# colmap/pycolmap

Hardware: AMD Instinct MI355X
Metric: descriptor-pair distances/sec (exhaustive SIFT match: dot + top-2 + ratio + cross-check) (higher is better)
Workload: dtype u8 descriptors, int8 MFMA / int32 accumulate; 1 GPU; 500 images x 4096 descriptors, exhaustive match + ratio test + cross-check (BASELINE.json configs[1] at N=1); pairs_total=124750, pairs_per_rank=124750, kernel=auto, matches_rank0=1865611

## Files before the change

### include/amc.h

```cpp
#ifndef AMC_H_
#define AMC_H_

#include <stddef.h>
#include <stdint.h>

#ifdef __cplusplus
extern "C" {
#endif

#define AMC_ABI_VERSION 5
#define AMC_DESC_DIM 128

enum {
    AMC_OK = 0,
    AMC_E_INVALID = -1,
    AMC_E_HIP = -2,
    AMC_E_NOMEM = -3,
    AMC_E_STATE = -4
};

enum { AMC_KERNEL_AUTO = 0, AMC_KERNEL_MFMA = 1, AMC_KERNEL_DOT4 = 2 };

typedef struct amc_ctx amc_ctx;

// ... 43 lines not shown

typedef struct amc_gathered_tables {
    size_t npairs;
    const uint64_t* offsets;
    const uint32_t* matches;
    const uint32_t* matches_device;
    uint64_t num_matches;
    uint64_t rows_sent, rows_received;
    int32_t world_size, rank;
    double sizes_ms, meta_ms, rows_ms, reorder_ms, download_ms, total_ms;
    void* _priv;
} amc_gathered_tables;

int amc_allgather_match_tables(amc_ctx* ctx, amc_comm* comm, const uint64_t* pair_index, size_t npairs_local,
                               const uint64_t* offsets, const uint32_t* matches, int download,
                               amc_gathered_tables* out);
void amc_gathered_tables_free(amc_gathered_tables* t);

typedef struct amc_gathered_records {
    size_t npairs;
    size_t record_bytes;
    const void* records;
    const void* records_device;
    uint64_t bytes_sent, bytes_received;
    int32_t world_size, rank;
    double total_ms;
    void* _priv;
} amc_gathered_records;
int amc_allgather_pair_records(amc_ctx* ctx, amc_comm* comm, const uint64_t* pair_index, size_t npairs_local,
                               const void* records, size_t record_bytes, int download, amc_gathered_records* out);
void amc_gathered_records_free(amc_gathered_records* r);
int amc_allgather_inlier_tables(amc_ctx* ctx, amc_comm* comm, const uint64_t* pair_index, size_t npairs_local,
                                int download, amc_gathered_tables* out);

int amc_ctx_reserve_slots(amc_ctx* ctx, uint32_t num_slots);
int amc_ctx_grow_slots(amc_ctx* ctx, uint32_t num_slots);

int amc_upload_descriptors(amc_ctx* ctx, uint32_t slot, const uint8_t* host_desc, uint32_t rows);

int amc_upload_descriptors_device(amc_ctx* ctx, uint32_t slot, const void* dev_desc,
                                  uint32_t rows);

int amc_match_pairs(amc_ctx* ctx, const uint32_t* slot1, const uint32_t* slot2, size_t npairs,
                    const amc_match_opts* opts, amc_match_result* out);
void amc_match_result_free(amc_match_result* r);

void amc_match_opts_default(amc_match_opts* opts);

int amc_get_acos_lut(amc_ctx* ctx, float* out);


typedef struct amc_ransac_opts {
    double max_error;
    double min_inlier_ratio;
    double confidence;
    double dyn_num_trials_multiplier;
    int64_t min_num_trials;
    int64_t max_num_trials;
} amc_ransac_opts;

typedef struct amc_tvg_opts {
    int32_t min_num_inliers;
    int32_t detect_watermark;
    int32_t multiple_ignore_watermark;
    int32_t force_H_use;
    int32_t compute_relative_pose;
    int32_t multiple_models;
    double min_E_F_inlier_ratio;
    double max_H_inlier_ratio;
    double watermark_min_inlier_ratio;
    double watermark_border_size;
    amc_ransac_opts ransac;
} amc_tvg_opts;

enum {
    AMC_TVG_UNDEFINED = 0, AMC_TVG_DEGENERATE = 1, AMC_TVG_CALIBRATED = 2, AMC_TVG_UNCALIBRATED = 3,
    AMC_TVG_PLANAR = 4, AMC_TVG_PANORAMIC = 5, AMC_TVG_PLANAR_OR_PANORAMIC = 6, AMC_TVG_WATERMARK = 7,
    AMC_TVG_MULTIPLE = 8
};

enum {
    AMC_CAM_SIMPLE_PINHOLE = 0,
    AMC_CAM_PINHOLE = 1,
    AMC_CAM_SIMPLE_RADIAL = 2,
    AMC_CAM_RADIAL = 3,
    AMC_CAM_OPENCV = 4,
    AMC_CAM_OPENCV_FISHEYE = 5,
    AMC_CAM_FULL_OPENCV = 6,
    AMC_CAM_FOV = 7,
    AMC_CAM_SIMPLE_RADIAL_FISHEYE = 8,
    AMC_CAM_RADIAL_FISHEYE = 9,
    AMC_CAM_THIN_PRISM_FISHEYE = 10
};

typedef struct amc_tvg {
    int32_t config;
    int32_t num_inliers;
    double E[9], F[9], H[9];
    int64_t num_trials[4];
    int64_t model_inliers[3];
} amc_tvg;

typedef struct amc_pose {
    int32_t ok;
    int32_t config;
    double qvec[4];
    double tvec[3];
    double R[9];
    double tri_angle;
    uint32_t num_points3D;
    uint32_t pad_;
} amc_pose;

typedef struct amc_verify_result {
    size_t npairs;
    amc_tvg* tvg;
    uint8_t* inlier_mask;
    double device_ms;
    double kernel_ms;
    uint32_t kernel_launches;
    amc_pose* pose;
    double pose_kernel_ms;
    uint64_t work[12];
    void* _priv;
} amc_verify_result;

void amc_tvg_opts_default(amc_tvg_opts* opts);

int amc_upload_keypoints(amc_ctx* ctx, uint32_t slot, const float* xy, uint32_t rows,
                         uint32_t stride_floats);

int amc_upload_points_f64(amc_ctx* ctx, uint32_t slot, const double* xy, uint32_t rows);

int amc_upload_camera(amc_ctx* ctx, uint32_t slot, int32_t model_id, uint64_t width,
                      uint64_t height, const double* params, int32_t num_params,
                      int32_t has_prior_focal_length);

int amc_cam_from_img(amc_ctx* ctx, int32_t model_id, const double* params, int32_t num_params,
                     const double* xy, size_t n, double* uv);
int amc_img_from_cam(amc_ctx* ctx, int32_t model_id, const double* params, int32_t num_params,
                     const double* uv, size_t n, double* xy);

int amc_verify_pairs(amc_ctx* ctx, const uint32_t* slot1, const uint32_t* slot2, size_t npairs,
                     const uint64_t* match_offsets, const uint32_t* matches,
                     const amc_tvg_opts* opts, uint32_t seed, amc_verify_result* out);
void amc_verify_result_free(amc_verify_result* r);

int amc_match_verify_pairs(amc_ctx* ctx, const uint32_t* slot1, const uint32_t* slot2, size_t npairs,
                           const amc_match_opts* match_opts, const amc_tvg_opts* tvg_opts, uint32_t seed,
                           amc_match_result* match_out, amc_verify_result* verify_out);

int amc_ctx_last_timeline(amc_ctx* ctx, double out_ms[8]);

int amc_pose_pairs(amc_ctx* ctx, const uint32_t* slot1, const uint32_t* slot2, size_t npairs,
                   const uint64_t* match_offsets, const uint32_t* inlier_matches, const amc_tvg* geoms,
                   amc_pose* out);

int amc_match_guided_pairs(amc_ctx* ctx, const uint32_t* slot1, const uint32_t* slot2, size_t npairs,
                           const amc_tvg* geoms, double max_error, const amc_match_opts* opts,
                           amc_match_result* out);

enum { AMC_RANSAC_F = 0, AMC_RANSAC_H = 1, AMC_RANSAC_E = 2 };
typedef struct amc_ransac_report {
    int32_t success;
    int32_t num_inliers;
    int64_t num_trials;
    double model[9];
} amc_ransac_report;
typedef struct amc_ransac_result {
    size_t npairs;
    amc_ransac_report* reports;
    uint8_t* inlier_mask;
    double device_ms;
    void* _priv;
} amc_ransac_result;
int amc_ransac_pairs(amc_ctx* ctx, int kind, const uint32_t* slot1, const uint32_t* slot2, size_t npairs,
                     const uint64_t* match_offsets, const uint32_t* matches,
                     const amc_ransac_opts* opts, uint32_t seed, amc_ransac_result* out);
void amc_ransac_result_free(amc_ransac_result* r);

int amc_squared_sampson_error(amc_ctx* ctx, const double* points1, const double* points2, size_t n,
                              const double E[9], double* out);

int amc_homography_decomposition(amc_ctx* ctx, const double H[9], const double K1[9], const double K2[9],
                                 const double* points1, const double* points2, size_t n, double R[9], double t[3],
                                 double normal[3], double* points3D, uint64_t* num_points3D);

#ifdef __cplusplus
}
#endif
#endif
```

### pycolmap_amd/_capi.py

```python
from __future__ import annotations

import ctypes as C
from pathlib import Path

import numpy as np

_PKG = Path(__file__).resolve().parent
LIB_PATH = _PKG / "libamc.so"

AMC_OK = 0
AMC_E_INVALID, AMC_E_HIP, AMC_E_NOMEM, AMC_E_STATE = -1, -2, -3, -4
KERNEL_AUTO, KERNEL_MFMA, KERNEL_DOT4 = 0, 1, 2
KERNELS = {"auto": KERNEL_AUTO, "mfma": KERNEL_MFMA, "dot4": KERNEL_DOT4}

EXPORTED_SYMBOLS = [
    "amc_last_error", "amc_abi_version", "amc_device_count", "amc_ctx_create", "amc_ctx_destroy",
    "amc_ctx_set_stream", "amc_ctx_reserve_slots", "amc_upload_descriptors",
    "amc_upload_descriptors_device", "amc_match_pairs", "amc_match_result_free",
    "amc_match_opts_default", "amc_get_acos_lut",
    "amc_tvg_opts_default", "amc_upload_keypoints", "amc_upload_camera", "amc_verify_pairs",
    "amc_verify_result_free", "amc_upload_points_f64", "amc_ransac_pairs", "amc_ransac_result_free",
    "amc_squared_sampson_error", "amc_match_guided_pairs", "amc_ctx_grow_slots", "amc_pose_pairs",
    "amc_cam_from_img", "amc_match_verify_pairs", "amc_ctx_trim", "amc_ctx_resident_matches",
    "amc_homography_decomposition", "amc_img_from_cam",
# ... 991 lines not shown
class UndistortOpts(C.Structure):
    _fields_ = [("blank_pixels", C.c_double), ("min_scale", C.c_double), ("max_scale", C.c_double),
                ("max_image_size", C.c_int32), ("_pad", C.c_int32), ("roi_min_x", C.c_double), ("roi_min_y", C.c_double),
                ("roi_max_x", C.c_double), ("roi_max_y", C.c_double)]


class UndistortCam(C.Structure):
    _fields_ = [("model", C.c_int32), ("_pad", C.c_int32), ("width", C.c_uint64), ("height", C.c_uint64),
                ("params", C.c_double * 12)]


class UndistortImage(C.Structure):
    _fields_ = [("src", C.c_void_p), ("src_stride", C.c_uint64), ("channels", C.c_int32), ("_pad", C.c_int32),
                ("src_camera", UndistortCam), ("dst_camera", UndistortCam), ("dst", C.c_void_p)]


class UndistortResult(C.Structure):
    _fields_ = [("device_ms", C.c_double), ("kernel_ms", C.c_double), ("num_batches", C.c_uint32),
                ("num_resized", C.c_uint32)]


CAMERA_MODEL_IDS = {"SIMPLE_PINHOLE": 0, "PINHOLE": 1, "SIMPLE_RADIAL": 2, "RADIAL": 3, "OPENCV": 4, "OPENCV_FISHEYE": 5,
                    "FULL_OPENCV": 6, "FOV": 7, "SIMPLE_RADIAL_FISHEYE": 8, "RADIAL_FISHEYE": 9, "THIN_PRISM_FISHEYE": 10}
CAMERA_NUM_PARAMS = [3, 4, 4, 5, 8, 8, 12, 5, 4, 5, 12]


def _undistort_cam(camera) -> UndistortCam:
    model, width, height, params = camera
    mid = CAMERA_MODEL_IDS[model] if isinstance(model, str) else int(model)
    p = [float(v) for v in params]
    if 0 <= mid < len(CAMERA_NUM_PARAMS) and len(p) != CAMERA_NUM_PARAMS[mid]:
        raise ValueError(f"camera model {model} takes {CAMERA_NUM_PARAMS[mid]} parameters, got {len(p)}")
    c = UndistortCam()
    c.model, c.width, c.height = mid, int(width), int(height)
    for i, v in enumerate(p[:12]):
        c.params[i] = v
    return c


def _undistort_cam_tuple(c: UndistortCam):
    n = CAMERA_NUM_PARAMS[c.model]
    return (c.model, int(c.width), int(c.height), np.array(c.params[:n], dtype=np.float64))


def undistort_options(**kw) -> UndistortOpts:
    o = UndistortOpts()
    load().amc_undistort_opts_default(C.byref(o))
    for k, v in kw.items():
        if k.startswith("_") or k not in dict(UndistortOpts._fields_):
            raise ValueError(f"undistort options: unknown option {k!r}")
        setattr(o, k, v)
    return o


def undistort_camera(camera, **opts):
    out = UndistortCam()
    _check(load().amc_undistort_camera(C.byref(undistort_options(**opts)), C.byref(_undistort_cam(camera)), C.byref(out)))
    return _undistort_cam_tuple(out)


def undistort_points(camera, undistorted, points) -> np.ndarray:
    xy = np.ascontiguousarray(points, dtype=np.float64).reshape(-1, 2)
    out = np.empty_like(xy)
    _check(load().amc_undistort_points(C.byref(_undistort_cam(camera)), C.byref(_undistort_cam(undistorted)), xy.shape[0],
                                       xy.ctypes.data_as(C.c_void_p), out.ctypes.data_as(C.c_void_p)))
    return out


class RansacOpts(C.Structure):
    _fields_ = [("max_error", C.c_double), ("min_inlier_ratio", C.c_double),
                ("confidence", C.c_double), ("dyn_num_trials_multiplier", C.c_double),
                ("min_num_trials", C.c_int64), ("max_num_trials", C.c_int64)]


class TvgOpts(C.Structure):
    _fields_ = [("min_num_inliers", C.c_int32), ("detect_watermark", C.c_int32),
                ("multiple_ignore_watermark", C.c_int32), ("force_H_use", C.c_int32),
                ("compute_relative_pose", C.c_int32), ("multiple_models", C.c_int32),
                ("min_E_F_inlier_ratio", C.c_double), ("max_H_inlier_ratio", C.c_double),
                ("watermark_min_inlier_ratio", C.c_double), ("watermark_border_size", C.c_double),
                ("ransac", RansacOpts)]


class Tvg(C.Structure):
    _fields_ = [("config", C.c_int32), ("num_inliers", C.c_int32), ("E", C.c_double * 9),
                ("F", C.c_double * 9), ("H", C.c_double * 9), ("num_trials", C.c_int64 * 4),
                ("model_inliers", C.c_int64 * 3)]


class Pose(C.Structure):
    _fields_ = [("ok", C.c_int32), ("config", C.c_int32), ("qvec", C.c_double * 4), ("tvec", C.c_double * 3),
                ("R", C.c_double * 9), ("tri_angle", C.c_double), ("num_points3D", C.c_uint32),
                ("pad_", C.c_uint32)]


class VerifyResult(C.Structure):
    _fields_ = [("npairs", C.c_size_t), ("tvg", C.POINTER(Tvg)), ("inlier_mask", C.POINTER(C.c_uint8)),
                ("device_ms", C.c_double), ("kernel_ms", C.c_double), ("kernel_launches", C.c_uint32),
                ("pose", C.POINTER(Pose)), ("pose_kernel_ms", C.c_double), ("work", C.c_uint64 * 12),
                ("_priv", C.c_void_p)]


class RansacReport(C.Structure):
    _fields_ = [("success", C.c_int32), ("num_inliers", C.c_int32), ("num_trials", C.c_int64),
                ("model", C.c_double * 9)]


class RansacResult(C.Structure):
    _fields_ = [("npairs", C.c_size_t), ("reports", C.POINTER(RansacReport)),
                ("inlier_mask", C.POINTER(C.c_uint8)), ("device_ms", C.c_double), ("_priv", C.c_void_p)]


RANSAC_DTYPE = np.dtype([("success", np.int32), ("num_inliers", np.int32), ("num_trials", np.int64),
                         ("model", np.float64, (3, 3))])
POSE_DTYPE = np.dtype([("ok", np.int32), ("config", np.int32), ("qvec", np.float64, (4,)),
                       ("tvec", np.float64, (3,)), ("R", np.float64, (3, 3)), ("tri_angle", np.float64),
                       ("num_points3D", np.uint32), ("pad_", np.uint32)])
TVG_DTYPE = np.dtype([("config", np.int32), ("num_inliers", np.int32), ("E", np.float64, (3, 3)),
                      ("F", np.float64, (3, 3)), ("H", np.float64, (3, 3)),
                      ("num_trials", np.int64, (4,)), ("model_inliers", np.int64, (3,))])
CAMERA_MODELS = {"SIMPLE_PINHOLE": 0, "PINHOLE": 1, "SIMPLE_RADIAL": 2, "RADIAL": 3, "OPENCV": 4, "OPENCV_FISHEYE": 5,
                 "FULL_OPENCV": 6, "FOV": 7, "SIMPLE_RADIAL_FISHEYE": 8, "RADIAL_FISHEYE": 9,
                 "THIN_PRISM_FISHEYE": 10}
CONFIG_NAMES = ["UNDEFINED", "DEGENERATE", "CALIBRATED", "UNCALIBRATED", "PLANAR", "PANORAMIC",
                "PLANAR_OR_PANORAMIC", "WATERMARK", "MULTIPLE"]

_lib = None


def load() -> C.CDLL:
    global _lib
    if _lib is not None:
        return _lib
    import os
    path = Path(os.environ.get("AMC_LIB_PATH", LIB_PATH))
    if not path.exists():
        raise ImportError(
            f"{path} not found — run `python -m pycolmap_amd.build` (hipcc, gfx950). "
            "pycolmap_amd has no CPU fallback.")
    lib = C.CDLL(str(path))
    lib.amc_last_error.restype = C.c_char_p
    lib.amc_abi_version.restype = C.c_int
    lib.amc_device_count.restype = C.c_int
    lib.amc_ctx_create.argtypes = [C.c_int, C.POINTER(C.c_void_p)]
    lib.amc_ctx_destroy.argtypes = [C.c_void_p]
    lib.amc_ctx_destroy.restype = None
    lib.amc_ctx_set_stream.argtypes = [C.c_void_p, C.c_void_p]
    lib.amc_ctx_trim.argtypes = [C.c_void_p]
    lib.amc_ctx_trim.restype = C.c_int
    lib.amc_ctx_resident_matches.argtypes = [C.c_void_p, C.c_void_p, C.c_void_p]
    lib.amc_ctx_resident_matches.restype = C.c_int
    lib.amc_upload_matches.argtypes = [C.c_void_p, C.c_void_p, C.c_uint64]
    lib.amc_upload_matches.restype = C.c_int
    if hasattr(lib, "amc_ctx_last_timeline"):
        lib.amc_ctx_last_timeline.argtypes = [C.c_void_p, C.c_void_p]
    lib.amc_ctx_reserve_slots.argtypes = [C.c_void_p, C.c_uint32]
    lib.amc_ctx_grow_slots.argtypes = [C.c_void_p, C.c_uint32]
    lib.amc_upload_descriptors.argtypes = [C.c_void_p, C.c_uint32, C.c_void_p, C.c_uint32]
    lib.amc_upload_descriptors_device.argtypes = [C.c_void_p, C.c_uint32, C.c_void_p, C.c_uint32]
    lib.amc_match_pairs.argtypes = [C.c_void_p, C.c_void_p, C.c_void_p, C.c_size_t,
                                    C.POINTER(MatchOpts), C.POINTER(MatchResult)]
    lib.amc_match_result_free.argtypes = [C.POINTER(MatchResult)]
    lib.amc_match_result_free.restype = None
    lib.amc_match_opts_default.argtypes = [C.POINTER(MatchOpts)]
    if hasattr(lib, "amc_sift_extract"):
        lib.amc_sift_opts_default.argtypes = [C.POINTER(SiftOpts)]
        lib.amc_sift_opts_default.restype = None
        lib.amc_sift_extract.argtypes = [C.c_void_p, C.POINTER(SiftImage), C.c_size_t, C.POINTER(SiftOpts),
                                         C.POINTER(SiftResult)]
        lib.amc_sift_extract.restype = C.c_int
        lib.amc_sift_result_free.argtypes = [C.POINTER(SiftResult)]
        lib.amc_sift_result_free.restype = None
    lib.amc_match_opts_default.restype = None
    if hasattr(lib, "amc_estimate_absolute_poses"):
        lib.amc_estimate_absolute_poses.argtypes = ([C.c_void_p, C.c_void_p, C.c_size_t] + [C.c_void_p] * 4 +
                                                    [C.POINTER(AbsPoseOpts), C.POINTER(AbsPoseRefineOpts), C.c_int,
                                                     C.POINTER(AbsPoseResult)])
        lib.amc_estimate_absolute_poses.restype = C.c_int
        lib.amc_refine_absolute_poses.argtypes = ([C.c_void_p, C.c_void_p, C.c_size_t] + [C.c_void_p] * 7 +
                                                  [C.POINTER(AbsPoseRefineOpts), C.c_int, C.POINTER(AbsPoseResult)])
        lib.amc_refine_absolute_poses.restype = C.c_int
        lib.amc_abspose_result_free.argtypes = [C.POINTER(AbsPoseResult)]
        lib.amc_abspose_result_free.restype = None
    if hasattr(lib, "amc_estimate_rig_absolute_poses"):
        lib.amc_estimate_rig_absolute_poses.argtypes = ([C.c_void_p, C.c_void_p, C.c_size_t] + [C.c_void_p] * 7 +
                                                        [C.POINTER(RansacOpts), C.POINTER(AbsPoseRefineOpts), C.c_int,
                                                         C.POINTER(RigPoseResult)])
        lib.amc_estimate_rig_absolute_poses.restype = C.c_int
        lib.amc_rigpose_result_free.argtypes = [C.POINTER(RigPoseResult)]
        lib.amc_rigpose_result_free.restype = None
    if hasattr(lib, "amc_bundle_adjust"):
        lib.amc_ba_opts_default.argtypes = [C.POINTER(BaOpts)]
        lib.amc_ba_opts_default.restype = None
        lib.amc_bundle_adjust.argtypes = [C.c_void_p, C.POINTER(BaProblem), C.POINTER(BaOpts), C.POINTER(BaResult)]
        lib.amc_bundle_adjust.restype = C.c_int
    if hasattr(lib, "amc_bundle_adjust_masked"):
        lib.amc_bundle_adjust_masked.argtypes = [C.c_void_p, C.POINTER(BaProblem), C.c_void_p, C.POINTER(BaOpts),
                                                 C.POINTER(BaResult)]
        lib.amc_bundle_adjust_masked.restype = C.c_int
    if hasattr(lib, "amc_filter_points3d"):
        lib.amc_filter_opts_default.argtypes = [C.POINTER(FilterOpts)]
        lib.amc_filter_opts_default.restype = None
        lib.amc_filter_points3d.argtypes = [C.c_void_p, C.POINTER(FilterProblem), C.POINTER(FilterOpts),
                                            C.POINTER(FilterResult)]
        lib.amc_filter_points3d.restype = C.c_int
        lib.amc_filter_result_free.argtypes = [C.POINTER(FilterResult)]
        lib.amc_filter_result_free.restype = None
    if hasattr(lib, "amc_triangulate_observations"):
        lib.amc_triobs_opts_default.argtypes = [C.POINTER(TriobsOpts)]
        lib.amc_triobs_opts_default.restype = None
        lib.amc_triangulate_observations.argtypes = [C.c_void_p, C.POINTER(TriobsProblem), C.POINTER(TriobsOpts),
                                                     C.POINTER(TriobsResult)]
        lib.amc_triangulate_observations.restype = C.c_int
        lib.amc_triobs_result_free.argtypes = [C.POINTER(TriobsResult)]
        lib.amc_triobs_result_free.restype = None
    if hasattr(lib, "amc_complete_tracks"):
        lib.amc_complete_opts_default.argtypes = [C.POINTER(CompleteOpts)]
        lib.amc_complete_opts_default.restype = None
        lib.amc_complete_tracks.argtypes = [C.c_void_p, C.POINTER(CompleteProblem), C.POINTER(CompleteOpts),
                                            C.POINTER(CompleteResult)]
        lib.amc_complete_tracks.restype = C.c_int
        lib.amc_complete_result_free.argtypes = [C.POINTER(CompleteResult)]
        lib.amc_complete_result_free.restype = None
    if hasattr(lib, "amc_merge_tracks"):
        lib.amc_merge_opts_default.argtypes = [C.POINTER(MergeOpts)]
        lib.amc_merge_opts_default.restype = None
        lib.amc_merge_tracks.argtypes = [C.c_void_p, C.POINTER(MergeProblem), C.POINTER(MergeOpts), C.POINTER(MergeResult)]
        lib.amc_merge_tracks.restype = C.c_int
        lib.amc_merge_result_free.argtypes = [C.POINTER(MergeResult)]
        lib.amc_merge_result_free.restype = None
    if hasattr(lib, "amc_retriangulate_pairs"):
        lib.amc_retri_opts_default.argtypes = [C.POINTER(RetriOpts)]
        lib.amc_retri_opts_default.restype = None
        lib.amc_retriangulate_pairs.argtypes = [C.c_void_p, C.POINTER(RetriProblem), C.POINTER(RetriOpts), C.POINTER(RetriResult)]
        lib.amc_retriangulate_pairs.restype = C.c_int
        lib.amc_retri_result_free.argtypes = [C.POINTER(RetriResult)]
        lib.amc_retri_result_free.restype = None
    if hasattr(lib, "amc_image_visibility"):
        lib.amc_image_visibility.argtypes = [C.c_void_p, C.POINTER(VisibilityProblem), C.POINTER(VisibilityResult)]
        lib.amc_image_visibility.restype = C.c_int
        lib.amc_visibility_result_free.argtypes = [C.POINTER(VisibilityResult)]
        lib.amc_visibility_result_free.restype = None
        lib.amc_pair_angle_opts_default.argtypes = [C.POINTER(PairAngleOpts)]
        lib.amc_pair_angle_opts_default.restype = None
        lib.amc_shared_point_angles.argtypes = [C.c_void_p, C.POINTER(PairAngleProblem), C.POINTER(PairAngleOpts),
                                                C.POINTER(PairAngleResult)]
        lib.amc_shared_point_angles.restype = C.c_int
        lib.amc_pair_angle_result_free.argtypes = [C.POINTER(PairAngleResult)]
        lib.amc_pair_angle_result_free.restype = None
    if hasattr(lib, "amc_patch_match"):
        lib.amc_patch_match_opts_default.argtypes = [C.POINTER(PatchMatchOpts)]
        lib.amc_patch_match_opts_default.restype = None
        lib.amc_patch_match.argtypes = [C.c_void_p, C.POINTER(PatchMatchOpts), C.POINTER(PatchMatchProblem), C.POINTER(PatchMatchResult)]
        lib.amc_patch_match.restype = C.c_int
        lib.amc_patch_match_result_free.argtypes = [C.POINTER(PatchMatchResult)]
        lib.amc_patch_match_result_free.restype = None
    if hasattr(lib, "amc_fuse_depth_maps"):
        lib.amc_fusion_opts_default.argtypes = [C.POINTER(FusionOpts)]
        lib.amc_fusion_opts_default.restype = None
        lib.amc_fuse_depth_maps.argtypes = [C.c_void_p, C.POINTER(FusionOpts), C.POINTER(FusionProblem), C.POINTER(FusionResult)]
        lib.amc_fuse_depth_maps.restype = C.c_int
        lib.amc_fusion_result_free.argtypes = [C.POINTER(FusionResult)]
        lib.amc_fusion_result_free.restype = None
    if hasattr(lib, "amc_triangulate_pairs"):
        lib.amc_pair_tri_opts_default.argtypes = [C.POINTER(PairTriOpts)]
        lib.amc_pair_tri_opts_default.restype = None
        lib.amc_triangulate_pairs.argtypes = [C.c_void_p, C.POINTER(PairTriProblem), C.POINTER(PairTriOpts), C.POINTER(PairTriResult)]
        lib.amc_triangulate_pairs.restype = C.c_int
        lib.amc_pair_tri_result_free.argtypes = [C.POINTER(PairTriResult)]
        lib.amc_pair_tri_result_free.restype = None
    if hasattr(lib, "amc_triangulate_tracks"):
        lib.amc_tri_opts_default.argtypes = [C.POINTER(TriOpts)]
        lib.amc_tri_opts_default.restype = None
        lib.amc_triangulate_tracks.argtypes = [C.c_void_p, C.c_void_p, C.c_size_t, C.c_void_p, C.c_size_t, C.c_void_p,
                                               C.c_void_p, C.POINTER(TriOpts), C.POINTER(TriResult)]
        lib.amc_triangulate_tracks.restype = C.c_int
        lib.amc_tri_result_free.argtypes = [C.POINTER(TriResult)]
        lib.amc_tri_result_free.restype = None
    if hasattr(lib, "amc_undistort_images"):
        lib.amc_undistort_opts_default.argtypes = [C.POINTER(UndistortOpts)]
        lib.amc_undistort_opts_default.restype = None
        lib.amc_undistort_camera.argtypes = [C.POINTER(UndistortOpts), C.POINTER(UndistortCam), C.POINTER(UndistortCam)]
        lib.amc_undistort_camera.restype = C.c_int
        lib.amc_undistort_points.argtypes = [C.POINTER(UndistortCam), C.POINTER(UndistortCam), C.c_size_t, C.c_void_p,
                                             C.c_void_p]
        lib.amc_undistort_points.restype = C.c_int
        lib.amc_undistort_images.argtypes = [C.c_void_p, C.c_size_t, C.c_void_p, C.POINTER(UndistortResult)]
        lib.amc_undistort_images.restype = C.c_int
    lib.amc_get_acos_lut.argtypes = [C.c_void_p, C.c_void_p]
    lib.amc_tvg_opts_default.argtypes = [C.POINTER(TvgOpts)]
    lib.amc_tvg_opts_default.restype = None
    lib.amc_upload_keypoints.argtypes = [C.c_void_p, C.c_uint32, C.c_void_p, C.c_uint32, C.c_uint32]
    lib.amc_upload_camera.argtypes = [C.c_void_p, C.c_uint32, C.c_int32, C.c_uint64, C.c_uint64,
                                      C.c_void_p, C.c_int32, C.c_int32]
    lib.amc_verify_pairs.argtypes = [C.c_void_p, C.c_void_p, C.c_void_p, C.c_size_t, C.c_void_p,
                                     C.c_void_p, C.POINTER(TvgOpts), C.c_uint32, C.POINTER(VerifyResult)]
    lib.amc_verify_result_free.argtypes = [C.POINTER(VerifyResult)]
    lib.amc_verify_result_free.restype = None
    lib.amc_match_guided_pairs.argtypes = [C.c_void_p, C.c_void_p, C.c_void_p, C.c_size_t, C.c_void_p, C.c_double,
                                           C.POINTER(MatchOpts), C.POINTER(MatchResult)]
    lib.amc_upload_points_f64.argtypes = [C.c_void_p, C.c_uint32, C.c_void_p, C.c_uint32]
    lib.amc_ransac_pairs.argtypes = [C.c_void_p, C.c_int, C.c_void_p, C.c_void_p, C.c_size_t, C.c_void_p,
                                     C.c_void_p, C.POINTER(RansacOpts), C.c_uint32, C.POINTER(RansacResult)]
    lib.amc_ransac_result_free.argtypes = [C.POINTER(RansacResult)]
    lib.amc_ransac_result_free.restype = None
    lib.amc_cam_from_img.argtypes = [C.c_void_p, C.c_int32, C.c_void_p, C.c_int32, C.c_void_p, C.c_size_t, C.c_void_p]
# ... 51 lines not shown
    return n


def comm_unique_id() -> bytes:
    buf = C.create_string_buffer(COMM_ID_BYTES)
    _check(load().amc_comm_unique_id(buf))
    return buf.raw


class Comm:

    def __init__(self, ctx: "Context", world_size: int, rank: int, unique_id: bytes):
        if len(unique_id) != COMM_ID_BYTES:
            raise ValueError(f"unique_id must be {COMM_ID_BYTES} bytes")
        self._lib, self._ctx = ctx._lib, ctx
        self.world_size, self.rank = int(world_size), int(rank)
        h = C.c_void_p()
        _check(self._lib.amc_comm_create(ctx._h, int(world_size), int(rank), unique_id, C.byref(h)))
        self._h = h

    def close(self) -> None:
        if getattr(self, "_h", None) and getattr(self._ctx, "_h", None):
            self._lib.amc_comm_destroy(self._h)
        self._h = None

    def __del__(self):
        try:
            self.close()
        except Exception:
            pass

    def _tables_out(self, res, download):
        try:
            g_off = np.ctypeslib.as_array(res.offsets, shape=(int(res.npairs) + 1,)).copy()
            total = int(res.num_matches)
            g_m = None
            if download:
                g_m = (np.ctypeslib.as_array(res.matches, shape=(total, 2)).copy() if total
                       else np.zeros((0, 2), dtype=np.uint32))
            stats = {k: float(getattr(res, k)) for k in ("sizes_ms", "meta_ms", "rows_ms", "reorder_ms", "download_ms", "total_ms")}
            stats.update(num_matches=total, rows_sent=int(res.rows_sent), rows_received=int(res.rows_received),
                         world_size=int(res.world_size), rank=int(res.rank), device_ptr=int(res.matches_device or 0),
                         gather_path="C ABI: ncclAllGather (sizes) + grouped ncclSend/ncclRecv (records, rows) from device memory")
        finally:
            self._lib.amc_gathered_tables_free(C.byref(res))
        return g_off, g_m, stats

    def allgather_match_tables(self, pair_index, offsets, matches=None, download: bool = True):
        off = np.ascontiguousarray(offsets, dtype=np.uint64).reshape(-1)
        n = off.size - 1
        idx = None if pair_index is None else np.ascontiguousarray(pair_index, dtype=np.uint64)
        m = None if matches is None else np.ascontiguousarray(matches, dtype=np.uint32).reshape(-1, 2)
        local = None
        if n < 0:
            local = "offsets must have npairs + 1 entries"
        elif idx is not None and idx.shape != (n,):
            local = "one global position per local pair"
        elif m is not None and m.shape[0] != int(off[-1]) - int(off[0]):
            local = "offsets and matches disagree (%d rows for offsets[-1] = %d)" % (m.shape[0], int(off[-1]))
        if local is not None:
            off, n, idx, m = np.array([1, 0], dtype=np.uint64), 1, None, np.zeros((1, 2), dtype=np.uint32)
        res = GatheredTables()
        rc = self._lib.amc_allgather_match_tables(
            self._ctx._h, self._h, None if idx is None else idx.ctypes.data_as(C.c_void_p), n,
            off.ctypes.data_as(C.c_void_p), None if m is None else m.ctypes.data_as(C.c_void_p), 1 if download else 0,
            C.byref(res))
        if local is not None:
            raise AmcError(rc if rc != AMC_OK else AMC_E_INVALID, "amc_allgather_match_tables: " + local)
        _check(rc)
        return self._tables_out(res, download)

    def allgather_pair_records(self, pair_index, records=None, download: bool = True, dtype=None):
        idx = None if pair_index is None else np.ascontiguousarray(pair_index, dtype=np.uint64).reshape(-1)
        rec = None if records is None else np.ascontiguousarray(records).reshape(-1)
        rdt = TVG_DTYPE if rec is None else rec.dtype
        if dtype is not None:
            rdt = np.dtype(dtype)
        n = len(rec) if rec is not None else (len(idx) if idx is not None else 0)
        width = rdt.itemsize
        if rec is not None and idx is not None and len(idx) != n:
            width, bad = 4, "one global position per local record"
        else:
            bad = None
        res = GatheredRecords()
        rc = self._lib.amc_allgather_pair_records(
            self._ctx._h, self._h, None if idx is None else idx.ctypes.data_as(C.c_void_p), n,
            None if rec is None else rec.ctypes.data_as(C.c_void_p), width, 1 if download else 0, C.byref(res))
        if bad is not None:
            raise AmcError(rc if rc != AMC_OK else AMC_E_INVALID, "amc_allgather_pair_records: " + bad)
        _check(rc)
        try:
            total = int(res.npairs)
            out = None
            if download:
                out = (np.frombuffer(C.string_at(res.records, total * width), dtype=rdt).copy() if total
                       else np.zeros(0, dtype=rdt))
            stats = dict(npairs=total, record_bytes=int(res.record_bytes), bytes_sent=int(res.bytes_sent),
                         bytes_received=int(res.bytes_received), world_size=int(res.world_size), rank=int(res.rank),
                         total_ms=float(res.total_ms), device_ptr=int(res.records_device or 0))
        finally:
            self._lib.amc_gathered_records_free(C.byref(res))
        return out, stats

    def allgather_inlier_tables(self, pair_index, npairs_local: int | None = None, download: bool = True):
        idx = None if pair_index is None else np.ascontiguousarray(pair_index, dtype=np.uint64).reshape(-1)
        n = len(idx) if idx is not None else int(npairs_local or 0)
        res = GatheredTables()
        _check(self._lib.amc_allgather_inlier_tables(self._ctx._h, self._h, None if idx is None else idx.ctypes.data_as(C.c_void_p),
                                                     n, 1 if download else 0, C.byref(res)))
        return self._tables_out(res, download)


class Context:

    def comm_create(self, world_size: int, rank: int, unique_id: bytes) -> Comm:
        import weakref
        comm = Comm(self, world_size, rank, unique_id)
        self.__dict__.setdefault("_comms", []).append(weakref.ref(comm))
        return comm

    def __init__(self, device_id: int = 0):
        self._lib = load()
        h = C.c_void_p()
        _check(self._lib.amc_ctx_create(device_id, C.byref(h)))
        self._h = h
        self.device_id = device_id
        self.resident_generation = 0

    def close(self) -> None:
        self.resident_generation = getattr(self, "resident_generation", 0) + 1
        for ref in self.__dict__.pop("_comms", []):
            comm = ref()
            if comm is not None:
                comm.close()
        if getattr(self, "_h", None):
            self._lib.amc_ctx_destroy(self._h)
            self._h = None

    def __del__(self):
        try:
            self.close()
        except Exception:
            pass

    def __enter__(self):
        return self

    def __exit__(self, *exc):
        self.close()

    def set_stream(self, hip_stream: int | None) -> None:
        _check(self._lib.amc_ctx_set_stream(self._h, C.c_void_p(hip_stream or 0)))

    def last_timeline(self) -> dict:
        buf = (C.c_double * 8)()
        _check(self._lib.amc_ctx_last_timeline(self._h, buf))
        return dict(verify_setup_done=buf[0], match_returned=buf[1], verify_launched=buf[2], verify_results_on_host=buf[3],
                    call_returned=buf[4], batch_handover_host_ms_hidden=buf[5])

    def resident_matches(self):
        ptr, n = C.c_void_p(), C.c_uint64()
        _check(self._lib.amc_ctx_resident_matches(self._h, C.byref(ptr), C.byref(n)))
        return int(ptr.value or 0), int(n.value)

    def upload_matches(self, matches) -> int:
        m = np.ascontiguousarray(matches, dtype=np.uint32).reshape(-1, 2)
        self.resident_generation += 1
        _check(self._lib.amc_upload_matches(self._h, m.ctypes.data_as(C.c_void_p), C.c_uint64(m.shape[0])))
        return int(m.shape[0])

    def resident_view_valid(self, generation: int) -> bool:
        return generation == self.resident_generation and bool(getattr(self, "_h", None))

    def resident_matches_tensor(self, device_index: int = 0, copy: bool = False):
        import torch
        ptr, n = self.resident_matches()
        if n == 0:
            return torch.zeros((0, 2), dtype=torch.int32, device=torch.device("cuda", device_index))
        if copy:
            return self.resident_matches_tensor(device_index, copy=False).clone()

        class _View:
            __cuda_array_interface__ = {"shape": (n, 2), "typestr": "<i4", "data": (ptr, False), "version": 3, "strides": None}
        return torch.as_tensor(_View(), device=torch.device("cuda", device_index))

    def trim(self) -> None:
        self.resident_generation += 1
        _check(self._lib.amc_ctx_trim(self._h))

    def reserve_slots(self, n: int) -> None:
        _check(self._lib.amc_ctx_reserve_slots(self._h, n))

    def grow_slots(self, n: int) -> None:
        _check(self._lib.amc_ctx_grow_slots(self._h, n))

    def upload_descriptors(self, slot: int, desc: np.ndarray) -> None:
        d = np.ascontiguousarray(desc, dtype=np.uint8)
        if d.size and (d.ndim != 2 or d.shape[1] != 128):
            raise ValueError(f"descriptors must be N x 128 uint8, got {d.shape}")
        rows = d.shape[0] if d.ndim == 2 else 0
        _check(self._lib.amc_upload_descriptors(self._h, slot, d.ctypes.data_as(C.c_void_p), rows))

    def upload_descriptors_device(self, slot: int, dev_ptr: int, rows: int) -> None:
        _check(self._lib.amc_upload_descriptors_device(self._h, slot, C.c_void_p(dev_ptr), rows))

    def sift_extract(self, images, **opts):
        single = isinstance(images, np.ndarray)
        imgs = [im if isinstance(im, np.ndarray) and im.ndim == 2 and im.strides[1] == 1 and im.strides[0] >= im.shape[1]
                else np.ascontiguousarray(im) for im in ([images] if single else images)]
        for im in imgs:
            if im.dtype != np.uint8 or im.ndim != 2:
                raise ValueError(f"sift_extract: images must be 2-D uint8, got {im.dtype} {im.shape}")
        o = SiftOpts()
        self._lib.amc_sift_opts_default(C.byref(o))
        for k, v in opts.items():
            if k == "normalization" and isinstance(v, str):
                v = SIFT_NORMALIZATIONS[v]
            if k not in dict(SiftOpts._fields_):
                raise ValueError(f"sift_extract: unknown option {k!r}")
            setattr(o, k, type(getattr(o, k))(v) if not isinstance(v, bool) else int(v))
        arr = (SiftImage * max(1, len(imgs)))()
        for i, im in enumerate(imgs):
            arr[i] = SiftImage(im.ctypes.data, im.shape[1], im.shape[0], im.strides[0])
        res = SiftResult()
        _check(self._lib.amc_sift_extract(self._h, arr, len(imgs), C.byref(o), C.byref(res)))
        try:
            off = np.ctypeslib.as_array(res.offsets, (len(imgs) + 1,)).copy()
            n = int(off[-1])
            kp = np.ctypeslib.as_array(res.keypoints, (max(n, 1), 4))[:n].copy()
            desc = np.ctypeslib.as_array(res.descriptors, (max(n, 1), 128))[:n].copy()
            stats = {"device_ms": res.device_ms, "stage_ms": dict(zip(SIFT_STAGES, list(res.stage_ms)))}
        finally:
            self._lib.amc_sift_result_free(C.byref(res))
        out = [(kp[off[i]:off[i + 1]], desc[off[i]:off[i + 1]]) for i in range(len(imgs))]
        return (out[0] if single else out), stats

    def estimate_absolute_poses(self, offsets, camera_models, camera_params, points2D, points3D, estimation=None,
                                refinement=None, return_covariance=False):
        off, models, prm, p2, p3 = abspose_inputs(offsets, camera_models, camera_params, points2D, points3D)
        eo, ro = abspose_options(estimation, refinement)
        res = AbsPoseResult()
        ptr = lambda a: a.ctypes.data_as(C.c_void_p)
        _check(self._lib.amc_estimate_absolute_poses(self._h, ptr(off), off.size - 1, ptr(models), ptr(prm), ptr(p2),
                                                      ptr(p3), C.byref(eo), C.byref(ro), int(bool(return_covariance)),
                                                      C.byref(res)))
        return self._abspose_out(res, off.size - 1, int(off[-1]), return_covariance)

    def refine_absolute_poses(self, offsets, camera_models, camera_params, points2D, points3D, qvec, tvec, inlier_mask,
                              refinement=None, return_covariance=False):
        off, models, prm, p2, p3 = abspose_inputs(offsets, camera_models, camera_params, points2D, points3D)
        nq, n = off.size - 1, int(off[-1])
        q = np.ascontiguousarray(qvec, dtype=np.float64).reshape(-1, 4)
        t = np.ascontiguousarray(tvec, dtype=np.float64).reshape(-1, 3)
        m = np.ascontiguousarray(inlier_mask, dtype=bool).reshape(-1).astype(np.uint8)
        if q.shape[0] != nq or t.shape[0] != nq or m.size != n:
            raise ValueError(f"refine_absolute_poses: {nq} queries and {n} correspondences by offsets, {q.shape[0]} "
                             f"rotations, {t.shape[0]} translations, {m.size} mask entries")
        _, ro = abspose_options(None, refinement)
        res = AbsPoseResult()
        ptr = lambda a: a.ctypes.data_as(C.c_void_p)
        _check(self._lib.amc_refine_absolute_poses(self._h, ptr(off), nq, ptr(models), ptr(prm), ptr(p2), ptr(p3),
                                                    ptr(q), ptr(t), ptr(m), C.byref(ro), int(bool(return_covariance)),
                                                    C.byref(res)))
        return self._abspose_out(res, nq, n, return_covariance)

    def _abspose_out(self, res, nq, n, cov):
        try:
            a = lambda p, shape: np.ctypeslib.as_array(p, (max(shape[0], 1),) + shape[1:])[:shape[0]].copy()
            out = {"success": a(res.success, (nq,)).astype(bool), "qvec": a(res.qvec, (nq, 4)),
                   "tvec": a(res.tvec, (nq, 3)), "num_inliers": a(res.num_inliers, (nq,)),
                   "num_trials": a(res.num_trials, (nq,)), "focal_factor": a(res.focal_factor, (nq,)),
                   "inlier_mask": a(res.inlier_mask, (n,)).astype(bool), "device_ms": res.device_ms,
                   "kernel_ms": res.kernel_ms, "num_batches": int(res.num_batches)}
            if cov:
                out["covariance"] = a(res.covariance, (nq, 36)).reshape(nq, 6, 6)
        finally:
            self._lib.amc_abspose_result_free(C.byref(res))
        return out

    def bundle_adjust(self, camera_models, camera_params, camera_const, image_cameras, qvec, tvec, pose_const, xyz,
                      obs_image, obs_point, obs_xy, options=None, point_const=None):
        models, prm, cc, icam, q, t, pc, X, oi, op, xy = ba_inputs(camera_models, camera_params, camera_const,
                                                                   image_cameras, qvec, tvec, pose_const, xyz,
                                                                   obs_image, obs_point, obs_xy)
        o = ba_options(options)
        ptr = lambda a: a.ctypes.data_as(C.c_void_p)
        pb = BaProblem(models.size, ptr(models), ptr(prm), ptr(cc), icam.size, ptr(icam), ptr(q), ptr(t), ptr(pc),
                       X.shape[0], ptr(X), oi.size, ptr(oi), ptr(op), ptr(xy))
        res = BaResult()
        if point_const is None:
            _check(self._lib.amc_bundle_adjust(self._h, C.byref(pb), C.byref(o), C.byref(res)))
        else:
            mask = np.ascontiguousarray(np.asarray(point_const).reshape(-1) != 0, dtype=np.uint8)
            if mask.size != X.shape[0]:
                raise ValueError(f"bundle adjustment: {X.shape[0]} points, {mask.size} point_const flags")
            _check(self._lib.amc_bundle_adjust_masked(self._h, C.byref(pb), ptr(mask), C.byref(o), C.byref(res)))
        out = {k: getattr(res, k) for k, _ in BaResult._fields_}
        out["termination"] = BA_TERMINATIONS[res.termination]
        out.update(camera_params=prm, qvec=q, tvec=t, xyz=X)
        return out

    def filter_points3d(self, camera_models, camera_params, image_cameras, qvec, tvec, xyz, track_offsets, obs_image,
                        obs_xy, selected=None, max_reproj_error=4.0, min_tri_angle=1.5, errors_only=False):
        models, prm, icam, q, t, X, off, oi, xy, sel = filter_inputs(camera_models, camera_params, image_cameras, qvec,
                                                                     tvec, xyz, track_offsets, obs_image, obs_xy,
                                                                     selected)
# ... 563 lines not shown
```

### pycolmap_amd/csrc/amc_api.hip

```cpp
#include <algorithm>
#include <chrono>
#include <cmath>
#include <cstdarg>
#include <cstdio>
#include <cstring>
#include <new>
#include <string>
#include <thread>
#include <vector>

#include "amc_ctx.h"
#include "camera_math.h"

using namespace amc;

namespace {
thread_local std::string g_err;
}

namespace amc {
int api_fail(int code, const char* fmt, ...) {
    char buf[512];
    va_list ap;
    va_start(ap, fmt);
    vsnprintf(buf, sizeof buf, fmt, ap);
    va_end(ap);
    g_err = buf;
    return code;
}
CtxView ctx_view(amc_ctx* c) {
    return CtxView{c->device, c->stream, c->resident_matches ? c->d_keep.p : nullptr, c->resident_matches};
}
VerifyResident verify_resident(amc_ctx* c) { return c->vres; }
}

extern "C" {

const char* amc_last_error(void) { return g_err.c_str(); }
int amc_abi_version(void) { return AMC_ABI_VERSION; }

int amc_device_count(void) {
    int n = 0;
    hipError_t e = hipGetDeviceCount(&n);
    if (e != hipSuccess) {
        if (e == hipErrorNoDevice) return 0;
        return api_fail(AMC_E_HIP, "hipGetDeviceCount: %s", hipGetErrorString(e));
    }
    return n;
}

void amc_match_opts_default(amc_match_opts* o) {
    if (!o) return;
    o->max_ratio = 0.8;
    o->max_distance = 0.7;
    o->cross_check = 1;
    o->kernel = AMC_KERNEL_AUTO;
}

int amc_ctx_create(int device_id, amc_ctx** out) {
    if (!out) return api_fail(AMC_E_INVALID, "amc_ctx_create: out is NULL");
    *out = nullptr;
    int n = 0;
    HIPCHK(hipGetDeviceCount(&n));
    if (device_id < 0 || device_id >= n)
        return api_fail(AMC_E_INVALID, "amc_ctx_create: device %d out of range (%d devices)",
                        device_id, n);
    HIPCHK(hipSetDevice(device_id));
    hipDeviceProp_t prop;
    HIPCHK(hipGetDeviceProperties(&prop, device_id));
    if (std::strncmp(prop.gcnArchName, "gfx950", 6) != 0)
        return api_fail(AMC_E_HIP, "amc_ctx_create: device %d is %s; this library is gfx950-only",
                        device_id, prop.gcnArchName);
    amc_ctx* c = new (std::nothrow) amc_ctx();
    if (!c) return api_fail(AMC_E_NOMEM, "amc_ctx_create: out of host memory");
    c->device = device_id;
    hipError_t e = hipStreamCreateWithFlags(&c->own_stream, hipStreamNonBlocking);
    if (e != hipSuccess) {
        delete c;
        return api_fail(AMC_E_HIP, "hipStreamCreate: %s", hipGetErrorString(e));
    }
    c->stream = c->own_stream;
    e = hipStreamCreateWithFlags(&c->copy_stream, hipStreamNonBlocking);
    if (e != hipSuccess) {
        (void)hipStreamDestroy(c->own_stream);
        delete c;
        return api_fail(AMC_E_HIP, "hipStreamCreate: %s", hipGetErrorString(e));
    }
    bool ev_ok = true;
    for (auto& ev : c->cev) ev_ok &= hipEventCreateWithFlags(&ev, hipEventDisableTiming) == hipSuccess;
    {
        int lo = 0, hi = 0;
        (void)hipDeviceGetStreamPriorityRange(&lo, &hi);
        if (hipStreamCreateWithPriority(&c->aux_stream, hipStreamNonBlocking, lo) != hipSuccess) c->aux_stream = nullptr;
        for (auto& ev : c->aev) ev_ok &= hipEventCreateWithFlags(&ev, hipEventDisableTiming) == hipSuccess;
    }
    if (hipStreamCreateWithFlags(&c->vstream, hipStreamNonBlocking) != hipSuccess) c->vstream = nullptr;
    ev_ok &= hipEventCreateWithFlags(&c->vev_setup, hipEventDisableTiming) == hipSuccess;
    ev_ok &= hipEventCreateWithFlags(&c->vev_matches, hipEventDisableTiming) == hipSuccess;
    for (auto& ev : c->ev) ev_ok &= hipEventCreate(&ev) == hipSuccess;
    for (auto& set : c->bev)
        for (auto& ev : set) ev_ok &= hipEventCreate(&ev) == hipSuccess;
    if (!ev_ok) {
        amc_ctx_destroy(c);
        return api_fail(AMC_E_HIP, "amc_ctx_create: hipEventCreate failed");
    }
    c->h_lut.resize(kAcosLutSize);
    const float kDistNorm = 1.0f / (512.0f * 512.0f);
    for (int d = 0; d < kAcosLutSize; ++d)
        c->h_lut[d] = acosf(std::fmin(kDistNorm * (float)d, 1.0f));
    if (hipMalloc(reinterpret_cast<void**>(&c->d_lut), kAcosLutSize * sizeof(float)) !=
            hipSuccess ||
        hipMalloc(reinterpret_cast<void**>(&c->d_scalars), 16 * sizeof(uint32_t)) !=
            hipSuccess ||
        hipMalloc(reinterpret_cast<void**>(&c->d_vscalars), kVScalarWords * sizeof(uint32_t)) != hipSuccess ||
        hipMemcpy(c->d_lut, c->h_lut.data(), kAcosLutSize * sizeof(float),
                  hipMemcpyHostToDevice) != hipSuccess ||
        c->h_scalars.ensure(16) != hipSuccess) {
        amc_ctx_destroy(c);
        return api_fail(AMC_E_HIP, "amc_ctx_create: device allocation failed");
    }
    *out = c;
    return AMC_OK;
}

void amc_ctx_destroy(amc_ctx* c) {
    if (!c) return;
    (void)hipSetDevice(c->device);
    const bool dprof = env_flag("AMC_DESTROY_PROFILE");
    auto tp0 = std::chrono::steady_clock::now();
    auto dlap = [&](const char* what) {
        if (!dprof) return;
        const auto now = std::chrono::steady_clock::now();
        std::fprintf(stderr, "[amc destroy] %s %.1f ms\n", what, std::chrono::duration<double, std::milli>(now - tp0).count());
        tp0 = now;
    };
    (void)hipDeviceSynchronize();
    dlap("sync");
    c->slots.clear();
    c->arena.release_all();
    dlap("slots");
    c->d_imgs.release();
    c->d_grids.release();
    if (c->d_lut) (void)hipFree(c->d_lut);
    if (c->d_accept) (void)hipFree(c->d_accept);
    if (c->d_scalars) (void)hipFree(c->d_scalars);
    c->ms.release_all();
    c->d_keep.release(); c->d_csr.release();
    dlap("match device buffers");
    c->h_csr[0].release(); c->h_csr[1].release();
    c->h_tout.release(); c->h_tmask.release();
    for (int k = 0; k < 2; ++k) {
        c->h_pairs[k].release(); c->h_work[k].release(); c->h_order[k].release(); c->h_order2[k].release();
        c->h_grp[k].release(); c->h_grp2[k].release();
        c->h_pair_off[k].release(); c->h_pair_cnt[k].release(); c->h_matches[k].release();
        c->h_bscalars[k].release();
    }
    c->h_scalars.release();
    dlap("pinned host buffers");
    c->d_timgs.release(); c->d_tmatches.release();
    c->d_estate.release(); c->d_stream.release(); c->d_wmcut.release();
    c->d_tout.release();
    c->vslices.clear();
    c->h_timgs.release(); c->h_tp.release(); c->h_moff.release();
    if (c->d_vscalars) (void)hipFree(c->d_vscalars);
    c->d_tvg_packed.release(); c->d_mask_packed.release(); c->d_moff.release(); c->d_tp_all.release(); c->d_worksum.release();
    c->d_ppairs.release(); c->d_pmatches.release(); c->d_pcos.release(); c->d_pout.release();
    c->h_ppairs.release(); c->h_pout.release();
    dlap("verify device buffers");
    for (auto& ev : c->ev)
        if (ev) (void)hipEventDestroy(ev);
    for (auto& set : c->bev)
        for (auto& ev : set)
            if (ev) (void)hipEventDestroy(ev);
    for (auto& ev : c->cev)
        if (ev) (void)hipEventDestroy(ev);
    if (c->copy_stream) (void)hipStreamDestroy(c->copy_stream);
    if (c->aux_stream) (void)hipStreamDestroy(c->aux_stream);
    for (auto& ev : c->aev)
        if (ev) (void)hipEventDestroy(ev);
    if (c->vstream) (void)hipStreamDestroy(c->vstream);
    if (c->vev_setup) (void)hipEventDestroy(c->vev_setup);
    if (c->vev_matches) (void)hipEventDestroy(c->vev_matches);
    if (c->own_stream) (void)hipStreamDestroy(c->own_stream);
    dlap("events and streams");
    delete c;
    dlap("delete (pools)");
}

int amc_ctx_set_stream(amc_ctx* c, void* hip_stream) {
    if (!c) return api_fail(AMC_E_INVALID, "amc_ctx_set_stream: ctx is NULL");
    c->stream = hip_stream ? reinterpret_cast<hipStream_t>(hip_stream) : c->own_stream;
    return AMC_OK;
}

int amc_ctx_trim(amc_ctx* c) {
    if (!c) return api_fail(AMC_E_INVALID, "amc_ctx_trim: NULL ctx");
    HIPCHK(hipSetDevice(c->device));
    HIPCHK(hipStreamSynchronize(c->stream));
    if (c->copy_stream) HIPCHK(hipStreamSynchronize(c->copy_stream));
    c->result_pool->trim();
    c->d_keep.release(); c->d_csr.release();
    c->resident_matches = 0;
    c->vres = amc::VerifyResident{};
    c->ms.release_large();
    if (c->d_stream.cap * sizeof(uint32_t) > ((size_t)16 << 20)) {
        c->d_stream.release();
        c->stream_len = 0;
    }
    if (c->aux_stream) HIPCHK(hipStreamSynchronize(c->aux_stream));
    if (c->vstream) HIPCHK(hipStreamSynchronize(c->vstream));
    for (auto& sl : c->vslices)
        if (sl) sl->release();
    c->h_tp.release(); c->h_moff.release(); c->h_ppairs.release(); c->h_pout.release();
    c->d_estate.release();
    c->d_tout.release(); c->d_tmatches.release(); c->d_pmatches.release(); c->d_pcos.release();
    c->d_tvg_packed.release(); c->d_mask_packed.release(); c->d_moff.release(); c->d_tp_all.release();
    c->verify_pool->trim();
    c->arena.release_idle_slabs();
    c->h_tout.release(); c->h_tmask.release();
    for (int k = 0; k < 2; ++k) {
        c->h_matches[k].release();
        c->h_csr[k].release();
    }
    return AMC_OK;
}

int amc_ctx_resident_matches(amc_ctx* c, const uint32_t** dev_matches, uint64_t* num_matches) {
    if (!c || !dev_matches || !num_matches) return api_fail(AMC_E_INVALID, "amc_ctx_resident_matches: NULL argument");
    *dev_matches = c->resident_matches ? c->d_keep.p : nullptr;
    *num_matches = c->resident_matches;
    return AMC_OK;
}

int amc_upload_matches(amc_ctx* c, const uint32_t* matches, uint64_t num_matches) {
    if (!c) return api_fail(AMC_E_INVALID, "amc_upload_matches: ctx is NULL");
    if (num_matches > 0 && !matches) return api_fail(AMC_E_INVALID, "amc_upload_matches: NULL rows");
    HIPCHK(hipSetDevice(c->device));
    HIPCHK(hipStreamSynchronize(c->stream));
    c->resident_matches = 0;
    c->vres = amc::VerifyResident{};
    if (num_matches == 0) return AMC_OK;
    HIPCHK(c->d_keep.ensure((size_t)(2 * num_matches)));
    HIPCHK(hipMemcpyAsync(c->d_keep.p, matches, (size_t)(2 * num_matches) * sizeof(uint32_t), hipMemcpyHostToDevice, c->stream));
    HIPCHK(hipStreamSynchronize(c->stream));
    c->resident_matches = num_matches;
    return AMC_OK;
}

int amc_ctx_reserve_slots(amc_ctx* c, uint32_t num_slots) {
    if (!c) return api_fail(AMC_E_INVALID, "amc_ctx_reserve_slots: ctx is NULL");
    HIPCHK(hipSetDevice(c->device));
    HIPCHK(hipStreamSynchronize(c->stream));
    c->slots.assign(num_slots, Slot());
    c->arena.release_all();
    c->table_dirty = true;
    return AMC_OK;
}

int amc_ctx_grow_slots(amc_ctx* c, uint32_t num_slots) {
    if (!c) return api_fail(AMC_E_INVALID, "amc_ctx_grow_slots: ctx is NULL");
    if (num_slots < c->slots.size())
        return api_fail(AMC_E_INVALID, "amc_ctx_grow_slots: %u < current %zu slots (use amc_ctx_reserve_slots to reset)",
                        num_slots, c->slots.size());
    c->slots.resize(num_slots);
    c->table_dirty = true;
    return AMC_OK;
}

static int upload_common(amc_ctx* c, uint32_t slot, const void* src, uint32_t rows,
                         hipMemcpyKind kind) {
    if (!c) return api_fail(AMC_E_INVALID, "upload_descriptors: ctx is NULL");
    if (slot >= c->slots.size())
        return api_fail(AMC_E_INVALID, "upload_descriptors: slot %u >= reserved %zu", slot,
                        c->slots.size());
    if (rows > 0 && !src) return api_fail(AMC_E_INVALID, "upload_descriptors: NULL data, rows=%u", rows);
    if (rows > (1u << 30)) return api_fail(AMC_E_INVALID, "upload_descriptors: rows=%u too large", rows);
    HIPCHK(hipSetDevice(c->device));
    Slot& s = c->slots[slot];
    if (s.base) {
        HIPCHK(hipStreamSynchronize(c->stream));
        c->arena.free(s.base);
        s.base = nullptr;
    }
    c->table_dirty = true;
    s.valid = true;
    s.dev.rows = rows;
    s.dev.rows_pad = round_up(rows, kRowPad);
    s.maxsq = 0;
    if (rows == 0) return AMC_OK;
    const size_t rp = s.dev.rows_pad;
    const size_t bytes = rp * kDim * 2 + rp * sizeof(int32_t);
    hipError_t e = c->arena.alloc(&s.base, bytes);
    if (e != hipSuccess) {
        s.valid = false;
        s.dev = ImageDev{};
        return api_fail(AMC_E_NOMEM, "upload_descriptors: hipMalloc(%zu): %s", bytes,
                        hipGetErrorString(e));
    }
    uint8_t* raw = static_cast<uint8_t*>(s.base);
    uint8_t* prep = raw + rp * kDim;
    int32_t* rs = reinterpret_cast<int32_t*>(prep + rp * kDim);
    s.dev.raw = raw;
    s.dev.prep = prep;
    s.dev.rs128 = rs;
    HIPCHK(hipMemcpyAsync(raw, src, (size_t)rows * kDim, kind, c->stream));
    if (rp > rows)
        HIPCHK(memset_async(raw + (size_t)rows * kDim, 0, (rp - rows) * kDim, c->stream));
    HIPCHK(memset_async(c->d_scalars + 2, 0, sizeof(uint32_t), c->stream));
    HIPCHK(launch_prep(raw, prep, rs, s.dev.rows_pad, c->d_scalars + 2, c->stream));
    HIPCHK(hipMemcpyAsync(c->h_scalars.p + 2, c->d_scalars + 2, sizeof(uint32_t),
                          hipMemcpyDeviceToHost, c->stream));
    HIPCHK(hipStreamSynchronize(c->stream));
    s.maxsq = c->h_scalars.p[2];
    return AMC_OK;
}

int amc_upload_descriptors(amc_ctx* c, uint32_t slot, const uint8_t* host_desc, uint32_t rows) {
    return upload_common(c, slot, host_desc, rows, hipMemcpyHostToDevice);
}
int amc_upload_descriptors_device(amc_ctx* c, uint32_t slot, const void* dev_desc,
                                  uint32_t rows) {
    return upload_common(c, slot, dev_desc, rows, hipMemcpyDeviceToDevice);
}

int amc_get_acos_lut(amc_ctx* c, float* out) {
    if (!c || !out) return api_fail(AMC_E_INVALID, "amc_get_acos_lut: NULL argument");
    HIPCHK(hipSetDevice(c->device));
    HIPCHK(hipMemcpy(out, c->d_lut, kAcosLutSize * sizeof(float), hipMemcpyDeviceToHost));
    return AMC_OK;
}

void amc_tvg_opts_default(amc_tvg_opts* o) {
    if (!o) return;
    o->min_num_inliers = 15;
    o->detect_watermark = 1;
    o->multiple_ignore_watermark = 1;
    o->force_H_use = 0;
    o->compute_relative_pose = 0;
    o->multiple_models = 0;
    o->min_E_F_inlier_ratio = 0.95;
    o->max_H_inlier_ratio = 0.8;
    o->watermark_min_inlier_ratio = 0.7;
    o->watermark_border_size = 0.1;
    o->ransac.max_error = 4.0;
    o->ransac.min_inlier_ratio = 0.25;
    o->ransac.confidence = 0.999;
    o->ransac.dyn_num_trials_multiplier = 3.0;
    o->ransac.min_num_trials = 100;
    o->ransac.max_num_trials = 10000;
}

static int build_keypoint_grid(amc_ctx* c, Slot& s, const float* xy, uint32_t rows) {
    guided::GridGeom gg;
    std::vector<uint32_t> sidx, start;
    if (!guided::build_grid(xy, rows, gg, sidx, start)) return AMC_OK;
    GridDev g{};
    g.x0 = gg.x0; g.y0 = gg.y0; g.cw = gg.cw; g.ch = gg.ch; g.inv_cw = gg.inv_cw; g.inv_ch = gg.inv_ch;
    g.bx1 = gg.bx1; g.by1 = gg.by1;
    g.n = rows;
    std::vector<float> sxy((size_t)rows * 2);
    for (uint32_t k = 0; k < rows; ++k) {
        sxy[2 * (size_t)k] = xy[2 * (size_t)sidx[k]];
        sxy[2 * (size_t)k + 1] = xy[2 * (size_t)sidx[k] + 1];
    }
    const size_t b_xy = sxy.size() * sizeof(float), b_idx = sidx.size() * sizeof(uint32_t), b_st = start.size() * sizeof(uint32_t);
    hipError_t e = c->arena.alloc(&s.grid_base, b_xy + b_idx + b_st);
    if (e != hipSuccess) return api_fail(AMC_E_NOMEM, "amc_upload_keypoints: hipMalloc (grid): %s", hipGetErrorString(e));
    char* base = static_cast<char*>(s.grid_base);
    HIPCHK(hipMemcpy(base, sxy.data(), b_xy, hipMemcpyHostToDevice));
    HIPCHK(hipMemcpy(base + b_xy, sidx.data(), b_idx, hipMemcpyHostToDevice));
    HIPCHK(hipMemcpy(base + b_xy + b_idx, start.data(), b_st, hipMemcpyHostToDevice));
    g.sxy = reinterpret_cast<const float*>(base);
    g.sidx = reinterpret_cast<const uint32_t*>(base + b_xy);
    g.cell_start = reinterpret_cast<const uint32_t*>(base + b_xy + b_idx);
    s.grid = g;
    return AMC_OK;
// ... 238 lines not shown
```

### pycolmap_amd/csrc/amc_ctx.h

```cpp
#pragma once

#include <functional>
#include <map>
#include <memory>
#include <mutex>
#include <vector>

#include "amc_internal.h"
#include "slot_arena.h"
#include "scan_accept.h"

namespace amc {

inline uint32_t round_up(uint32_t x, uint32_t m) { return (x + m - 1) / m * m; }

struct Slot {
    void* base = nullptr;
    ImageDev dev{};
    uint32_t maxsq = 0;
    bool valid = false;
    float* kp = nullptr;
    double* kp64 = nullptr;
    double* kpn = nullptr;
    bool kpn_valid = false;
    uint32_t kp_rows = 0;
    bool has_kp = false, has_cam = false;
    CameraDev cam{};
    void* grid_base = nullptr;
    GridDev grid{};
};

struct HipRaw {
    static int alloc(void** p, size_t bytes) { return (int)hipMalloc(p, bytes); }
    static void free(void* p) { (void)hipFree(p); }
    static void clear_error() { (void)hipGetLastError(); }
};
struct SlotArena : amc::SlotArenaT<HipRaw> {
    template <class T>
    hipError_t alloc(T** out, size_t bytes) {
        return (hipError_t)amc::SlotArenaT<HipRaw>::alloc(out, bytes);
    }
};

struct PinnedPool {
    static constexpr size_t kMaxIdleBytes = (size_t)3 << 29;
    std::mutex mu;
    std::vector<PinBuf<uint32_t>> idle;
    PinBuf<uint32_t> acquire(size_t want = 0) {
        std::lock_guard<std::mutex> lock(mu);
        if (idle.empty()) return PinBuf<uint32_t>();
        auto better = [&](const PinBuf<uint32_t>& a, const PinBuf<uint32_t>& b) {
            const bool fa = a.cap >= want, fb = b.cap >= want;
            if (want && fa != fb) return fa;
            if (want && fa) return a.cap < b.cap;
            return a.cap > b.cap;
        };
        size_t best = 0;
        for (size_t i = 1; i < idle.size(); ++i)
            if (better(idle[i], idle[best])) best = i;
        PinBuf<uint32_t> b = std::move(idle[best]);
        idle.erase(idle.begin() + best);
        return b;
    }
    void give_back(PinBuf<uint32_t> b) {
        if (!b.p) return;
        std::lock_guard<std::mutex> lock(mu);
        idle.push_back(std::move(b));
        auto total = [&] {
            size_t t = 0;
            for (auto& x : idle) t += x.cap * sizeof(uint32_t);
            return t;
        };
        while (!idle.empty() && (idle.size() > 3 || total() > kMaxIdleBytes)) {
            size_t small = 0;
            for (size_t i = 1; i < idle.size(); ++i)
                if (idle[i].cap < idle[small].cap) small = i;
            idle.erase(idle.begin() + small);
        }
    }
    void trim() {
        std::lock_guard<std::mutex> lock(mu);
        idle.clear();
    }
};

struct VerifyClassSlot {
    PinBuf<TvgPair> h_pairs, h_pairs_e;
    DevBuf<TvgPair> pairs, pairs_e;
    DevBuf<double> ws, ws_e;
    DevBuf<uint8_t> maskws;
    void release() { pairs.release(); pairs_e.release(); ws.release(); ws_e.release(); maskws.release(); h_pairs.release(); h_pairs_e.release(); }
};
struct VerifySliceBufs {
    PinBuf<uint32_t> h_tabs;
    DevBuf<uint32_t> tabs;
    DevBuf<uint8_t> outmask, emask;
    VerifyClassSlot cls[4];
    hipEvent_t ev[4] = {nullptr, nullptr, nullptr, nullptr};
    hipEvent_t ev_e_done = nullptr, ev_aux_done = nullptr;
    bool aux_pending = false;
    void release() {
        tabs.release(); outmask.release(); emask.release(); h_tabs.release();
        for (auto& k : cls) k.release();
    }
    ~VerifySliceBufs() {
        for (auto& e : ev)
            if (e) (void)hipEventDestroy(e);
        if (ev_e_done) (void)hipEventDestroy(ev_e_done);
        if (ev_aux_done) (void)hipEventDestroy(ev_aux_done);
    }
};
constexpr size_t kVScalarWords = 128;
constexpr size_t kMaxStreamWords = (size_t)1 << 28;

struct TrialTabKey {
    uint32_t M;
    double confidence, multiplier;
    bool operator<(const TrialTabKey& o) const {
        if (M != o.M) return M < o.M;
        if (confidence != o.confidence) return confidence < o.confidence;
        return multiplier < o.multiplier;
    }
};
constexpr size_t kTrialTabCacheWords = size_t(64) << 20;

}

using namespace amc;

struct amc_ctx {
    int device = 0;
    hipStream_t own_stream = nullptr;
    hipStream_t stream = nullptr;
    hipStream_t copy_stream = nullptr;
    hipEvent_t cev[2] = {nullptr, nullptr};
    hipStream_t aux_stream = nullptr;
    hipEvent_t aev[2] = {nullptr, nullptr};
    std::vector<Slot> slots;
    bool table_dirty = true;
    DevBuf<ImageDev> d_imgs;
    DevBuf<GridDev> d_grids;
    float* d_lut = nullptr;
    std::vector<float> h_lut;
    ScanAccept* d_accept = nullptr;
    ScanAccept h_accept{};
    float accept_ratio = 0.f, accept_distance = 0.f;
    bool accept_valid = false;
    uint32_t* d_scalars = nullptr;
    struct MatchScratch {
        DevBuf<PairDev> d_pairs;
        DevBuf<Dot4Work> d_work;
        DevBuf<uint32_t> d_order, d_order2;
        DevBuf<uint32_t> d_grp, d_grp2, d_seg_base, d_grp_segs, d_grp_item_base;
        DevBuf<SegDesc> d_segs;
        DevBuf<Top2> d_rowbuf, d_colbuf;
        DevBuf<uint32_t> d_accmask;
        DevBuf<GuidedDev> d_guided;
        DevBuf<uint32_t> d_pair_off, d_pair_cnt, d_matches, d_cand_cnt, d_candbuf;
        DevBuf<uint32_t> d_live, d_live_fwd, d_live_all, d_live_rev, d_live_scan;
        void release_all() {
            d_pairs.release(); d_work.release(); d_order.release(); d_order2.release();
            d_grp.release(); d_grp2.release(); d_seg_base.release(); d_grp_segs.release();
            d_grp_item_base.release(); d_segs.release();
            d_rowbuf.release(); d_colbuf.release(); d_accmask.release(); d_guided.release();
            d_pair_off.release(); d_pair_cnt.release(); d_matches.release();
            d_cand_cnt.release(); d_candbuf.release();
            d_live.release(); d_live_fwd.release(); d_live_all.release(); d_live_rev.release();
            d_live_scan.release();
        }
        void release_large() {
            d_rowbuf.release(); d_colbuf.release(); d_accmask.release(); d_matches.release(); d_candbuf.release();
            d_segs.release(); d_seg_base.release();
        }
    };
    MatchScratch ms;
    DevBuf<uint32_t> d_keep;
    DevBuf<uint64_t> d_csr;
    uint64_t resident_matches = 0;
    PinBuf<uint64_t> h_csr[2];
    std::shared_ptr<PinnedPool> result_pool = std::make_shared<PinnedPool>();
    SlotArena arena;
    PinBuf<PairDev> h_pairs[2];
    PinBuf<Dot4Work> h_work[2];
    PinBuf<uint32_t> h_order[2], h_order2[2], h_pair_off[2], h_pair_cnt[2], h_matches[2], h_bscalars[2];
    PinBuf<uint32_t> h_grp[2], h_grp2[2];
    PinBuf<uint32_t> h_scalars;
    hipEvent_t ev[6] = {nullptr, nullptr, nullptr, nullptr, nullptr, nullptr};
    hipEvent_t bev[2][5] = {{nullptr, nullptr, nullptr, nullptr, nullptr},
                            {nullptr, nullptr, nullptr, nullptr, nullptr}};
    DevBuf<TvgImage> d_timgs;
    DevBuf<uint32_t> d_tmatches;
    DevBuf<TvgEState> d_estate;
    std::vector<std::unique_ptr<VerifySliceBufs>> vslices;
    hipStream_t vstream = nullptr;
    hipEvent_t vev_setup = nullptr, vev_matches = nullptr;
    uint32_t* d_vscalars = nullptr;
    std::vector<double> wm_cut_cache;
    double wm_cut_conf = 0.0, wm_cut_mult = 0.0;
    bool wm_cut_on_device = false;
    PinBuf<TvgImage> h_timgs;
    std::vector<TvgImage> timgs_on_device;
    PinBuf<TvgPair> h_tp;
    PinBuf<uint64_t> h_moff;
    DevBuf<uint32_t> d_stream;
    uint32_t stream_seed = 0;
    size_t stream_len = 0;
    DevBuf<double> d_wmcut;
    DevBuf<TvgOut> d_tout;
    DevBuf<amc_tvg> d_tvg_packed;
    DevBuf<uint8_t> d_mask_packed;
    DevBuf<uint64_t> d_moff;
    DevBuf<TvgPair> d_tp_all;
    DevBuf<unsigned long long> d_worksum;
    amc::VerifyResident vres;
    double timeline[8] = {0, 0, 0, 0, 0, 0, 0, 0};
    double last_hook_ms = 0.0;
    std::shared_ptr<PinnedPool> verify_pool = std::make_shared<PinnedPool>();
    PinBuf<TvgOut> h_tout;
    PinBuf<uint8_t> h_tmask;
    std::map<TrialTabKey, std::vector<uint32_t>> trial_tabs;
    size_t trial_tab_words = 0;
    DevBuf<PosePair> d_ppairs;
    DevBuf<uint32_t> d_pmatches;
    DevBuf<double> d_pcos;
    DevBuf<PoseOut> d_pout;
    PinBuf<PosePair> h_ppairs;
    PinBuf<PoseOut> h_pout;
};

namespace amc {

using BatchHook = std::function<int(size_t begin, size_t end, const uint64_t* offsets, const uint64_t* keep_off)>;
int match_impl(amc_ctx* c, const uint32_t* slot1, const uint32_t* slot2, size_t npairs, const amc_match_opts* opts_in,
               const amc_tvg* geoms, double max_error, amc_match_result* out, std::vector<uint64_t>* keep_off = nullptr,
               const BatchHook* batch_hook = nullptr);

int ensure_normalized(amc_ctx* c, uint32_t slot);
void fill_tvg_images(const amc_ctx* c, std::vector<TvgImage>& timgs);

}
```

### pycolmap_amd/csrc/amc_internal.h

```cpp
#pragma once

#include <hip/hip_runtime.h>
#include <stdint.h>

#include <algorithm>
#include <cstdlib>
#include <type_traits>
#include <vector>

#include "../../include/amc.h"
#include "guided_region.h"

namespace amc {

constexpr int kDim = AMC_DESC_DIM;
constexpr int kRowPad = 256;
constexpr int kAcosLutSize = 262145;

__host__ __device__ __forceinline__ constexpr uint32_t arena_swizzle(uint32_t row) {
    return ((row >> 1) & 1u) | (((row >> 5) & 3u) << 1);
}

struct ImageDev {
    const uint8_t* raw;
// ... 172 lines not shown
};

inline hipError_t create_events(hipEvent_t* ev, int n, const unsigned* flags = nullptr) {
    for (int i = 0; i < n; ++i) {
        const hipError_t e = hipEventCreateWithFlags(&ev[i], flags ? flags[i] : hipEventDefault);
        if (e != hipSuccess) {
            for (int j = 0; j < i; ++j) (void)hipEventDestroy(ev[j]);
            std::fill(ev, ev + n, nullptr);
            return e;
        }
    }
    return hipSuccess;
}

class StreamTimer {
  public:
    explicit StreamTimer(hipStream_t s) : s_(s), made_(create_events(ab_, 2)) {}
    StreamTimer(const StreamTimer&) = delete;
    StreamTimer& operator=(const StreamTimer&) = delete;
    ~StreamTimer() {
        for (hipEvent_t e : ab_)
            if (e) (void)hipEventDestroy(e);
        for (hipEvent_t e : spans_) (void)hipEventDestroy(e);
    }

    hipError_t start() { return made_ != hipSuccess ? made_ : hipEventRecord(ab_[0], s_); }
    hipError_t stop(double& ms) {
        hipError_t e = hipEventRecord(ab_[1], s_);
        if (e == hipSuccess) e = hipEventSynchronize(ab_[1]);
        return e == hipSuccess ? add_elapsed(ab_[0], ab_[1], ms) : e;
    }
    hipError_t span_begin() {
        hipEvent_t two[2];
        if (const hipError_t e = create_events(two, 2)) return e;
        spans_.insert(spans_.end(), two, two + 2);
        return hipEventRecord(two[0], s_);
    }
    hipError_t span_end() { return hipEventRecord(spans_.back(), s_); }
    hipError_t spans(double& ms) const {
        for (size_t i = 0; i + 1 < spans_.size(); i += 2)
            if (const hipError_t e = add_elapsed(spans_[i], spans_[i + 1], ms)) return e;
        return hipSuccess;
    }

  private:
    static hipError_t add_elapsed(hipEvent_t a, hipEvent_t b, double& ms) {
        float f = 0.f;
        const hipError_t e = hipEventElapsedTime(&f, a, b);
        if (e == hipSuccess) ms += f;
        return e;
    }
    hipStream_t s_;
    hipEvent_t ab_[2] = {nullptr, nullptr};
    hipError_t made_;
    std::vector<hipEvent_t> spans_;
};

struct Batches {
    std::vector<size_t> start{0};
    uint64_t most_items = 0, most_elems = 0;
    size_t count() const { return start.size() - 1; }
};
inline Batches split_batches(const uint64_t* offsets, size_t n, uint64_t max_items, uint64_t max_elems,
                             uint64_t factor = 1) {
    Batches b;
    for (size_t i = 0; i < n;) {
        size_t j = i + 1;
        while (j < n && j - i < max_items && (offsets[j + 1] - offsets[i]) * factor <= max_elems) ++j;
        b.most_items = std::max<uint64_t>(b.most_items, j - i);
        b.most_elems = std::max<uint64_t>(b.most_elems, offsets[j] - offsets[i]);
        b.start.push_back(j);
        i = j;
    }
    return b;
}

struct CtxView {
    int device;
    hipStream_t stream;
    const uint32_t* resident;
    uint64_t resident_rows;
};
CtxView ctx_view(amc_ctx* c);
struct TvgPair;
struct VerifyResident {
    size_t npairs = 0;
    uint64_t total = 0;
    const amc_tvg* tvg = nullptr;
    const uint8_t* mask = nullptr;
    const uint64_t* moff = nullptr;
    const TvgPair* tp = nullptr;
    const uint32_t* matches = nullptr;
};
VerifyResident verify_resident(amc_ctx* c);

hipError_t memset_async(void* p, int value, size_t bytes, hipStream_t s);
hipError_t memcpy_async(void* dst, const void* src, size_t bytes, hipMemcpyKind kind, hipStream_t s);

hipError_t launch_prep(const uint8_t* raw, uint8_t* prep, int32_t* rs128, uint32_t rows_pad,
                 uint32_t* maxsq_out, hipStream_t s);

hipError_t launch_match_dot4(const ImageDev* imgs, const PairDev* pairs, const Dot4Work* work,
                       uint32_t nwork, Top2* rowbuf, Top2* colbuf, const GuidedDev* guided, hipStream_t s);
hipError_t launch_match_guided_grid(const ImageDev* imgs, const GridDev* grids, const PairDev* pairs, const Dot4Work* work,
                              uint32_t nwork, Top2* rowbuf, Top2* colbuf, const GuidedDev* guided, hipStream_t s);

constexpr int kSegRows = 128;
constexpr int kSegsPerItem = 4;
struct alignas(64) SegDesc {
    const uint8_t* xprep;
    const int32_t* xrs;
    Top2* out;
    const uint32_t* list;
    const uint8_t* yprep;
    const int32_t* yrs;
    uint32_t cnt;
    uint32_t accword;
    uint32_t yrows;
    uint32_t pad_;
};
__device__ __forceinline__ bool one_way_accepts(const Top2 t, const float* __restrict__ lut,
                                                float max_ratio, float max_distance) {
    if (t.best_v == 0u) return false;
    const float a_best = lut[min(t.best_v, 262144u)];
    if (a_best > max_distance) return false;
    const float a_second = lut[min(t.second_v, 262144u)];
    if (a_best >= max_ratio * a_second) return false;
    return true;
}

hipError_t launch_build_segments(int mode, const ImageDev* imgs, const PairDev* pairs, const uint32_t* order,
                           const uint32_t* grp_start, uint32_t ngroups, const uint32_t* cand_cnt,
                           const uint32_t* candbuf, Top2* outbuf, uint32_t* seg_base, uint32_t* grp_segs,
                           uint32_t* grp_item_base, SegDesc* segs, uint32_t* nitems_dev, hipStream_t s);
struct ScanAccept;
struct CopyJob {
    const void* src = nullptr;
    void* dst = nullptr;
    unsigned long long n16 = 0;
    uint32_t parts = 0, pad_ = 0;
};
hipError_t launch_match_mfma(int mode, const SegDesc* segs, const uint32_t* nitems_dev, uint32_t max_items,
                       uint32_t* queue_head, uint32_t* accmask, const ScanAccept* accept_dev, hipStream_t s,
                       const CopyJob& job = CopyJob(), uint32_t* copy_head = nullptr);

size_t live_scratch_words(size_t npairs);
hipError_t launch_live_pairs(const ImageDev* imgs, const PairDev* pairs, uint32_t npairs, const uint32_t* accmask,
                             const uint32_t* order, uint32_t norder, uint32_t* live, uint32_t* live_fwd,
                             uint32_t* live_all, uint32_t* nlive, uint32_t* cand_cnt, uint32_t* pair_cnt,
                             uint32_t* pair_off, uint32_t* scratch, hipStream_t s);
hipError_t launch_compact_order(const uint32_t* order, uint32_t norder, uint32_t npairs, const uint32_t* key, uint32_t* list,
                                uint32_t* nlist, uint32_t* scratch, hipStream_t s);

hipError_t launch_resolve_index(int side, const ImageDev* imgs, const PairDev* pairs,
                          Top2* table, uint32_t* accmask, const float* acos_lut, FinalizeParams fp,
                          const uint32_t* cand_cnt, const uint32_t* candbuf, uint32_t* err_count,
                          bool grouped, const uint32_t* order, const uint32_t* nlist, uint32_t max_list, hipStream_t s);
uint32_t resolve_grouped_max_rows();
constexpr uint32_t kSelectMaxCols = 1u << 20;

hipError_t launch_select_candidates(const ImageDev* imgs, const PairDev* pairs, uint32_t npairs, uint32_t max_cols,
                              const Top2* rowbuf, const uint32_t* accmask, const float* acos_lut,
                              FinalizeParams fp, uint32_t* cand_cnt, uint32_t* candbuf, const uint32_t* list,
                              const uint32_t* nlist, hipStream_t s);

hipError_t launch_finalize(const ImageDev* imgs, const PairDev* pairs, uint32_t npairs, const uint32_t* list,
                     const uint32_t* nlist, const Top2* rowbuf, const Top2* colbuf, uint32_t* accmask,
                     const float* acos_lut, FinalizeParams fp, uint32_t* cursor, uint32_t capacity,
                     uint32_t* pair_off, uint32_t* pair_cnt, uint32_t* matches, hipStream_t s);

hipError_t launch_host_copy(void* dst_pinned, const void* src_dev, size_t bytes, hipStream_t s);
hipError_t launch_reorder_matches(const uint32_t* src_off, const uint32_t* cnt, const uint64_t* dst_off, uint32_t npairs,
                            const uint32_t* src, uint32_t* dst, hipStream_t s);

struct CameraDev {
    int32_t model_id;
    int32_t has_prior;
    uint64_t width, height;
    double params[12];
};
struct TvgImage {
    const float* kp;
    const double* kp64;
    const double* kpn;
    uint32_t rows;
    uint32_t pad;
    CameraDev cam;
};
hipError_t launch_undistort(const float* kp, const double* kp64, uint32_t rows, const CameraDev& cam, double* kpn,
                            hipStream_t s);
hipError_t launch_project(const double* uv, uint32_t n, const CameraDev& cam, double* xy, hipStream_t s);
struct TvgPair {
    uint32_t slot1, slot2;
    uint64_t match_off;
    uint64_t mask_off;
    uint32_t M;
    uint32_t tab_off[3];
    uint32_t orig;
};
struct PosePair {
    uint32_t slot1, slot2;
    uint64_t match_off;
    uint64_t mask_off;
    uint64_t ws_off;
    uint32_t M;
    int32_t config;
    double E[9], H[9];
};
struct alignas(128) PoseOut {
    int32_t ok;
    int32_t t_is_zero;
    uint32_t num_points3D;
    uint32_t pad;
    double R[9], t[3], q[4], cmed[2];
};
hipError_t launch_pose(const TvgImage* imgs, const PosePair* pairs, uint32_t npairs, const uint32_t* matches,
                       const uint8_t* mask, double* cosine_ws, PoseOut* out, hipStream_t s);

struct alignas(128) TvgOut {
    amc_tvg g;
    unsigned long long prof[8];
    unsigned long long work[12];
};
struct TvgParams {
    int32_t min_num_inliers, detect_watermark, force_H_use, min_num_trials;
    int32_t max_trials[4];
    double min_E_F_inlier_ratio, max_H_inlier_ratio, watermark_min_inlier_ratio,
        watermark_border_size, max_error;
    int32_t force_slow_sampler;
    int32_t no_fast_count;
    int32_t no_fast32;
    int32_t mode;
    uint32_t* bad_index_count;
    const double* wm_cut;
    const uint32_t* stream;
    uint32_t stream_len;
    uint32_t* stream_err;
};
struct alignas(64) TvgEState {
    double model[9];
    double sum;
    int32_t cnt, success, num_trials;
    uint32_t soff;
};
void tvg_diag_report();
void tvg_diag_report_e();
size_t tvg_ws_doubles_host(uint32_t mcap);
size_t tvg_ws_doubles_e_host(uint32_t mcap);
size_t tvg_ws_mask_bytes_host(uint32_t mcap);
constexpr int kTvgEWavesPerSimd = 2;
constexpr int kTvgFhWavesPerSimd = 4;
size_t tvg_lds_bytes(uint32_t mcap, int waves);
size_t tvg_lds_bytes_e(uint32_t mcap, int waves);
hipError_t launch_pack_verify(const TvgOut* out, const TvgPair* tp, uint32_t npairs, const uint8_t* mask_src,
                              const uint64_t* moff, amc_tvg* tvg_dst, uint8_t* mask_dst, unsigned long long* work,
                              int32_t trivial_below, hipStream_t s);
hipError_t launch_homography_decomposition(const double* in27, const double* p1, const double* p2, uint32_t n, double* out16,
                                           double* points3D, hipStream_t s);
hipError_t launch_sampson(const double* p1, const double* p2, size_t n, const double* E9, double* out,
                          hipStream_t s);
hipError_t launch_tvg_e(const TvgImage* imgs, const TvgPair* pairs, uint32_t npairs, const uint32_t* matches,
                        const uint32_t* trial_tabs, const TvgParams& P, double* ws, uint32_t mcap, uint32_t num_waves,
                        int waves_per_block, uint32_t* queue_head, TvgEState* estate, uint8_t* emask, TvgOut* out,
                        uint8_t* out_mask, hipStream_t s);
hipError_t launch_tvg_fh(const TvgImage* imgs, const TvgPair* pairs, uint32_t npairs, const uint32_t* matches,
                         const uint32_t* trial_tabs, const TvgParams& P, double* ws, uint8_t* mask_ws, uint32_t mcap,
                         uint32_t num_waves, int waves_per_block, uint32_t* queue_head, const TvgEState* estate,
                         const uint8_t* emask, TvgOut* out, uint8_t* out_mask, hipStream_t s);

size_t tvg_big_lds_bytes(int waves);
size_t tvg_big_lds_bytes_e(int waves);
size_t tvg_big_idx_doubles_host(uint32_t mcap);
hipError_t launch_tvg_e_big(const TvgImage* imgs, const TvgPair* pairs, uint32_t npairs, const uint32_t* matches,
                            const uint32_t* trial_tabs, const TvgParams& P, double* ws, uint32_t mcap, uint32_t num_waves,
                            int waves_per_block, uint32_t* queue_head, TvgEState* estate, uint8_t* emask, TvgOut* out,
                            uint8_t* out_mask, hipStream_t s);
hipError_t launch_tvg_fh_big(const TvgImage* imgs, const TvgPair* pairs, uint32_t npairs, const uint32_t* matches,
                             const uint32_t* trial_tabs, const TvgParams& P, double* ws, uint8_t* mask_ws, uint32_t mcap,
                             uint32_t num_waves, int waves_per_block, uint32_t* queue_head, const TvgEState* estate,
                             const uint8_t* emask, TvgOut* out, uint8_t* out_mask, hipStream_t s);

}
```

### pycolmap_amd/csrc/amc_match.hip

```cpp
#include <algorithm>
#include <chrono>
#include <cstdio>
#include <cstdlib>
#include <cstring>
#include <limits>
#include <memory>
#include <new>
#include <vector>

#include "amc_ctx.h"

using namespace amc;

namespace {

struct ResultPriv {
    std::vector<uint64_t> offsets;
    PinBuf<uint32_t> matches;
    std::shared_ptr<PinnedPool> pool;
    ~ResultPriv() {
        if (pool) pool->give_back(std::move(matches));
    }
};

constexpr size_t kMaxTop2Entries = (size_t)256 << 20;
constexpr size_t kMaxMatchCap = (size_t)256 << 20;

}

static void guided_grid_setup(GuidedDev& g, const GridDev& g1, const GridDev& g2, bool dense_only) {
    g.grid_ok = 0;
    g.bound[0] = g.bound[1] = 0.0;
    for (int k = 0; k < 9; ++k) g.minv[k] = 0.0;
    if (dense_only || g1.n == 0 || g2.n == 0) return;
    const float box1[4] = {g1.x0, g1.y0, g1.bx1, g1.by1}, box2[4] = {g2.x0, g2.y0, g2.bx1, g2.by1};
    g.grid_ok = guided::guided_pair_setup(g.kind, g.m, g.max_residual, box1, box2, g.bound, g.minv) ? 1 : 0;
}

int amc::match_impl(amc_ctx* c, const uint32_t* slot1, const uint32_t* slot2, size_t npairs,
                    const amc_match_opts* opts_in, const amc_tvg* geoms, double max_error,
                    amc_match_result* out, std::vector<uint64_t>* keep_off, const BatchHook* batch_hook) {
    if (!c || !out) return api_fail(AMC_E_INVALID, "amc_match_pairs: NULL ctx/out");
    std::memset(out, 0, sizeof *out);
    if (npairs > 0 && (!slot1 || !slot2))
        return api_fail(AMC_E_INVALID, "amc_match_pairs: NULL pair arrays");
    const bool prof = env_flag("AMC_MATCH_PROFILE");
    const bool guided_dense_only = env_flag("AMC_GUIDED_DENSE");
    const bool accept_trivial = env_flag("AMC_SCAN_ACCEPT_TRIVIAL");
    const bool resolve_ungrouped = env_flag("AMC_RESOLVE_UNGROUPED");
    const size_t batch_entries = (size_t)env_int("AMC_MATCH_BATCH_ENTRIES", 0, 0, (long long)kMaxTop2Entries);
    const char* const d2h_env = std::getenv("AMC_D2H");
    const size_t fuse_min_bytes = (size_t)env_int("AMC_D2H_FUSE_MIN_BYTES", 1 << 20, 0, std::numeric_limits<long long>::max());
    const int hook_split_mode = (int)env_int("AMC_HOOK_SPLIT", 1, 0, 2);
    const auto wall0 = std::chrono::steady_clock::now();
    double t_prepare = 0.0, t_collect = 0.0, t_enqueue = 0.0, t_scatter = 0.0;
    auto since = [](std::chrono::steady_clock::time_point t) {
        return std::chrono::duration<double, std::milli>(std::chrono::steady_clock::now() - t).count();
    };
    amc_match_opts o;
    if (opts_in) o = *opts_in; else amc_match_opts_default(&o);
    if (o.kernel != AMC_KERNEL_AUTO && o.kernel != AMC_KERNEL_MFMA && o.kernel != AMC_KERNEL_DOT4)
        return api_fail(AMC_E_INVALID, "amc_match_pairs: unknown kernel %d", o.kernel);
    uint64_t rows_total = 0;
    for (size_t i = 0; i < npairs; ++i) {
        if (slot1[i] >= c->slots.size() || slot2[i] >= c->slots.size())
            return api_fail(AMC_E_INVALID, "amc_match_pairs: pair %zu references slot out of range", i);
        if (!c->slots[slot1[i]].valid || !c->slots[slot2[i]].valid)
            return api_fail(AMC_E_STATE, "amc_match_pairs: pair %zu references a slot with no "
                            "descriptors uploaded", i);
        rows_total += c->slots[slot1[i]].dev.rows_pad;
    }
    std::vector<GuidedDev> h_guided;
    if (geoms) {
        h_guided.resize(npairs);
        for (size_t i = 0; i < npairs; ++i) {
            const int cfg = geoms[i].config;
            GuidedDev& g = h_guided[i];
            g.kind = (cfg == AMC_TVG_CALIBRATED || cfg == AMC_TVG_UNCALIBRATED) ? kGuidedF
                     : (cfg == AMC_TVG_PLANAR || cfg == AMC_TVG_PANORAMIC || cfg == AMC_TVG_PLANAR_OR_PANORAMIC)
                         ? kGuidedH : kGuidedNone;
            if (g.kind == kGuidedNone)
                return api_fail(AMC_E_INVALID, "amc_match_guided_pairs: pair %zu: configuration %d has no guided "
                                "matching (COLMAP keeps the inlier matches it has)", i, cfg);
            const double* m = g.kind == kGuidedF ? geoms[i].F : geoms[i].H;
            for (int k = 0; k < 9; ++k) g.m[k] = (float)m[k];
            g.max_residual = (float)(max_error * max_error);
            const Slot& a = c->slots[slot1[i]];
            const Slot& b = c->slots[slot2[i]];
            if (!a.kp || !b.kp || a.kp_rows < a.dev.rows || b.kp_rows < b.dev.rows)
                return api_fail(AMC_E_STATE, "amc_match_guided_pairs: pair %zu: float32 keypoints (one per descriptor) "
                                "must be uploaded for both images", i);
            guided_grid_setup(g, a.grid, b.grid, guided_dense_only);
        }
    }
    HIPCHK(hipSetDevice(c->device));
    hipStream_t st = c->stream;

    if (c->table_dirty) {
        HIPCHK(c->d_imgs.ensure(c->slots.size()));
        std::vector<ImageDev> t(c->slots.size());
        for (size_t i = 0; i < t.size(); ++i) t[i] = c->slots[i].dev;
        if (!t.empty())
            HIPCHK(hipMemcpy(c->d_imgs.p, t.data(), t.size() * sizeof(ImageDev),
                             hipMemcpyHostToDevice));
        HIPCHK(c->d_grids.ensure(c->slots.size()));
        std::vector<GridDev> gt(c->slots.size());
        for (size_t i = 0; i < gt.size(); ++i) gt[i] = c->slots[i].grid;
        if (!gt.empty())
            HIPCHK(hipMemcpy(c->d_grids.p, gt.data(), gt.size() * sizeof(GridDev), hipMemcpyHostToDevice));
        c->table_dirty = false;
    }

    const float max_ratio_f = (float)o.max_ratio;
    FinalizeParams fp;
    fp.max_ratio = max_ratio_f;
    fp.max_distance = (float)o.max_distance;
    fp.cross_check = o.cross_check ? 1 : 0;
    fp.reserved = 0;

    if (!c->accept_valid || std::memcmp(&c->accept_ratio, &fp.max_ratio, sizeof(float)) != 0 ||
        std::memcmp(&c->accept_distance, &fp.max_distance, sizeof(float)) != 0) {
        c->h_accept = build_scan_accept(c->h_lut.data(), (uint32_t)c->h_lut.size(), fp.max_ratio, fp.max_distance);
        if (accept_trivial) c->h_accept.trivial = 1;
        if (!c->d_accept) HIPCHK(hipMalloc(reinterpret_cast<void**>(&c->d_accept), sizeof(ScanAccept)));
        HIPCHK(hipStreamSynchronize(st));
        HIPCHK(hipMemcpy(c->d_accept, &c->h_accept, sizeof(ScanAccept), hipMemcpyHostToDevice));
        c->accept_ratio = fp.max_ratio;
        c->accept_distance = fp.max_distance;
        c->accept_valid = true;
    }
    HIPCHK(hipEventRecord(c->ev[0], st));
    ResultPriv* priv = new (std::nothrow) ResultPriv();
    if (!priv) return api_fail(AMC_E_NOMEM, "amc_match_pairs: out of host memory");
    priv->offsets.assign(npairs + 1, 0);
    priv->pool = c->result_pool;
    priv->matches = c->result_pool->acquire();
    size_t keep_used = 0;
    c->resident_matches = 0;
    c->vres = amc::VerifyResident{};
    if (keep_off) keep_off->assign(npairs, 0);

    const size_t mfma_max_cols = kSelectMaxCols;

    uint64_t num_dist = 0, n_mfma = 0, n_dot4 = 0, n_grid = 0;
    double kernel_ms = 0.0, cross_ms = 0.0;
    uint32_t kernel_launches = 0;

    int rc = AMC_OK;
    auto hc = [&](hipError_t e, const char* what) {
        if (e != hipSuccess && rc == AMC_OK)
            rc = api_fail(AMC_E_HIP, "amc_match_pairs: %s: %s", what, hipGetErrorString(e));
        return e == hipSuccess;
    };
    const size_t max_entries = batch_entries ? batch_entries : kMaxTop2Entries;

    struct Batch {
        size_t begin = 0, end = 0, nb = 0, top_rows = 0, top_cols = 0, cap = 0;
        size_t row_off = 0, nwork = 0, nord = 0, nwork_grid = 0;
        uint32_t max_cols = 0;
        size_t ngrp = 0, ngrp2 = 0, seg_cap = 0;
        int set = 0;
        uint32_t total = 0;
        bool grouped_resolve = true;
    };
    uint64_t rows_carved = 0, rows_collected = 0;
    const int d2h_mode = !d2h_env ? 0 : (std::strcmp(d2h_env, "memcpy") == 0 ? 2 : (std::strcmp(d2h_env, "stream") == 0 ? 1 : 0));
    struct PendingCopy {
        void* dst = nullptr;
        const void* src = nullptr;
        size_t bytes = 0;
        int set = -1;
    } pending;
    constexpr uint32_t kCopyParts = 64 / kSegsPerItem;
    auto sync_batch_streams = [&](const char* what) { return hc(hipStreamSynchronize(st), what); };
    const bool hook_split = batch_hook && hook_split_mode != 0;
    const size_t hook_split_min_pairs = hook_split_mode == 2 ? 2 : 4096;
    auto carve = [&](size_t begin, int set) {
        Batch b;
        b.begin = b.end = begin;
        b.set = set;
        size_t limit = max_entries;
        const uint64_t rows_left = rows_total - rows_carved;
        if (begin > 0 && rows_left <= max_entries && rows_left > max_entries / 4)
            limit = (size_t)(rows_left - max_entries / 4);
        if (begin == 0 && hook_split && rows_total <= max_entries && npairs >= hook_split_min_pairs)
            limit = (size_t)(rows_total * 6 / 10);
        while (b.end < npairs) {
            const Slot& x = c->slots[slot1[b.end]];
            const Slot& y = c->slots[slot2[b.end]];
            const size_t nr = x.dev.rows_pad, nc = y.dev.rows_pad;
            const size_t mc = o.cross_check ? std::min(x.dev.rows, y.dev.rows) : x.dev.rows;
            if (b.end > b.begin && (b.top_rows + nr > limit || b.top_cols + nc > max_entries ||
                                    b.cap + mc > kMaxMatchCap || b.end - b.begin >= (1u << 24)))
                break;
            b.top_rows += nr; b.top_cols += nc; b.cap += mc; ++b.end;
        }
        b.nb = b.end - b.begin;
        rows_carved += b.top_rows;
        return b;
    };
    auto build_reverse_order = [&](Batch& b) {
        const int k = b.set;
        const size_t nord = b.nord;
        if (!nord || !o.cross_check) return;
        const PairDev* hp = c->h_pairs[k].p;
        const size_t nslots = c->slots.size();
        std::vector<uint32_t> cnt(nslots + 1), tmp(nord);
        auto by_slot = [&](const uint32_t* src, uint32_t* dst, bool key_is_slot2) {
            std::fill(cnt.begin(), cnt.end(), 0u);
            for (size_t q = 0; q < nord; ++q) ++cnt[(key_is_slot2 ? hp[src[q]].slot2 : hp[src[q]].slot1) + 1];
            for (size_t v = 0; v < nslots; ++v) cnt[v + 1] += cnt[v];
            for (size_t q = 0; q < nord; ++q) dst[cnt[key_is_slot2 ? hp[src[q]].slot2 : hp[src[q]].slot1]++] = src[q];
        };
        uint32_t* ord2 = c->h_order2[k].p;
        by_slot(c->h_order[k].p, tmp.data(), true);
        by_slot(tmp.data(), ord2, false);
        size_t ngrp2 = 0;
        for (size_t q = 0; q < nord; ++q)
            if (q == 0 || hp[ord2[q]].slot1 != hp[ord2[q - 1]].slot1) c->h_grp2[k].p[ngrp2++] = (uint32_t)q;
        c->h_grp2[k].p[ngrp2] = (uint32_t)nord;
    };
    auto prepare = [&](Batch& b, bool defer_reverse) {
        const int k = b.set;
        const size_t nb = b.nb, begin = b.begin;
        if (!hc(c->h_pairs[k].ensure(nb), "pinned pairs") || !hc(c->h_order[k].ensure(nb), "pinned order") ||
            !hc(c->h_order2[k].ensure(nb), "pinned order2") || !hc(c->h_pair_off[k].ensure(nb), "pinned pair_off") ||
            !hc(c->h_pair_cnt[k].ensure(nb), "pinned pair_cnt") || !hc(c->h_bscalars[k].ensure(16), "pinned scalars"))
            return false;
        std::vector<uint8_t> want_mfma(nb, 0);
        for (size_t i = 0; i < nb; ++i) {
            const Slot& x = c->slots[slot1[begin + i]];
            const Slot& y = c->slots[slot2[begin + i]];
            const bool nonempty = x.dev.rows > 0 && y.dev.rows > 0;
            want_mfma[i] = nonempty && o.kernel != AMC_KERNEL_DOT4 && !geoms &&
                           (!o.cross_check || y.dev.rows_pad <= mfma_max_cols);
        }
        PairDev* hp = c->h_pairs[k].p;
        size_t row_off = 0, col_off = 0, nwork = 0, nord = 0, nimg1 = 0;
        std::vector<uint8_t> seen1(c->slots.size(), 0);
        b.grouped_resolve = !resolve_ungrouped;
        for (size_t i = 0; i < nb; ++i) {
            const Slot& x = c->slots[slot1[begin + i]];
            const Slot& y = c->slots[slot2[begin + i]];
            const bool nonempty = x.dev.rows > 0 && y.dev.rows > 0;
            if (o.kernel == AMC_KERNEL_MFMA && nonempty && !want_mfma[i]) {
                rc = api_fail(AMC_E_INVALID,
                              "amc_match_pairs: kernel=MFMA forced but pair %zu is not eligible "
                              "(rows_pad=%u, cols_pad=%u > %zu)", begin + i, x.dev.rows_pad,
                              y.dev.rows_pad, mfma_max_cols);
                return false;
            }
            PairDev& pd = hp[i];
            pd.slot1 = slot1[begin + i];
            pd.slot2 = slot2[begin + i];
            pd.mode = want_mfma[i] ? 1u : 0u;
            pd.pad = 0;
            pd.row_off = row_off;
            pd.col_off = col_off;
            row_off += x.dev.rows_pad;
            col_off += y.dev.rows_pad;
            num_dist += (uint64_t)x.dev.rows * y.dev.rows;
            if (!nonempty) continue;
            if (want_mfma[i]) {
                c->h_order[k].p[nord++] = (uint32_t)i;
                if (!seen1[pd.slot1]) { seen1[pd.slot1] = 1; ++nimg1; }
                ++n_mfma;
                b.max_cols = std::max(b.max_cols, y.dev.rows);
                if (std::max(x.dev.rows_pad, y.dev.rows_pad) > resolve_grouped_max_rows()) b.grouped_resolve = false;
            } else {
                nwork += (x.dev.rows + 63) / 64;
                if (o.cross_check) nwork += (y.dev.rows + 63) / 64;
                if (geoms && h_guided[begin + i].grid_ok) ++n_grid; else ++n_dot4;
            }
        }
        if (nord) {
            const size_t nslots = c->slots.size();
            std::vector<uint32_t> cnt(nslots + 1), tmp(nord);
            auto by_slot = [&](const uint32_t* src, uint32_t* dst, bool key_is_slot2) {
                std::fill(cnt.begin(), cnt.end(), 0u);
                for (size_t q = 0; q < nord; ++q) ++cnt[(key_is_slot2 ? hp[src[q]].slot2 : hp[src[q]].slot1) + 1];
                for (size_t v = 0; v < nslots; ++v) cnt[v + 1] += cnt[v];
                for (size_t q = 0; q < nord; ++q) dst[cnt[key_is_slot2 ? hp[src[q]].slot2 : hp[src[q]].slot1]++] = src[q];
            };
            uint32_t* ord = c->h_order[k].p;
            by_slot(ord, tmp.data(), false);
            by_slot(tmp.data(), ord, true);
        }
        b.ngrp = b.ngrp2 = 0;
        b.seg_cap = 0;
        if (nord) {
            if (!hc(c->h_grp[k].ensure(nord + 1), "pinned group cuts") ||
                (o.cross_check && !hc(c->h_grp2[k].ensure(nord + 1), "pinned group cuts")))
                return false;
            size_t seg1 = 0, seg2 = 0;
            for (size_t q = 0; q < nord; ++q) {
                const PairDev& pq = hp[c->h_order[k].p[q]];
                if (q == 0 || pq.slot2 != hp[c->h_order[k].p[q - 1]].slot2) c->h_grp[k].p[b.ngrp++] = (uint32_t)q;
                seg1 += (c->slots[pq.slot1].dev.rows + kSegRows - 1) / kSegRows;
                seg2 += (c->slots[pq.slot2].dev.rows + kSegRows - 1) / kSegRows;
            }
            c->h_grp[k].p[b.ngrp] = (uint32_t)nord;
            if (o.cross_check) b.ngrp2 = nimg1;
            b.seg_cap = std::max(seg1 + kSegsPerItem * b.ngrp, o.cross_check ? seg2 + kSegsPerItem * b.ngrp2 : 0);
        }
        b.nwork_grid = 0;
        if (nwork) {
            if (!hc(c->h_work[k].ensure(nwork), "pinned work")) return false;
            size_t w = 0;
            for (int pass = geoms ? 0 : 1; pass < 2; ++pass) {
                for (size_t i = 0; i < nb; ++i) {
                    if (hp[i].mode) continue;
                    if (geoms && (h_guided[begin + i].grid_ok != 0) != (pass == 0)) continue;
                    const Slot& x = c->slots[slot1[begin + i]];
                    const Slot& y = c->slots[slot2[begin + i]];
                    if (x.dev.rows == 0 || y.dev.rows == 0) continue;
                    for (uint32_t rb = 0; rb < (x.dev.rows + 63) / 64; ++rb)
                        c->h_work[k].p[w++] = Dot4Work{(uint32_t)i, 0u, rb};
                    if (o.cross_check)
                        for (uint32_t rb = 0; rb < (y.dev.rows + 63) / 64; ++rb)
                            c->h_work[k].p[w++] = Dot4Work{(uint32_t)i, 1u, rb};
                }
                if (pass == 0) b.nwork_grid = w;
            }
        }
        b.row_off = row_off;
        b.nwork = nwork;
        b.nord = nord;
        if (!defer_reverse) build_reverse_order(b);
        return true;
    };
    auto enqueue_scan = [&](Batch& b) {
        const int k = b.set;
        amc_ctx::MatchScratch& S = c->ms;
        const size_t nb = b.nb, nord = b.nord, nwork = b.nwork;
        const bool grow = S.d_pairs.cap < nb || S.d_order.cap < nb || S.d_order2.cap < nb ||
                          S.d_rowbuf.cap < b.top_rows || S.d_colbuf.cap < b.top_cols ||
                          S.d_accmask.cap < b.top_rows / 32 + 8 || S.d_pair_off.cap < nb || S.d_pair_cnt.cap < nb ||
                          S.d_matches.cap < 2 * b.cap || S.d_cand_cnt.cap < nb || S.d_candbuf.cap < b.top_cols ||
                          S.d_live.cap < nb || S.d_live_fwd.cap < nb || S.d_live_all.cap < nb || S.d_live_rev.cap < nb ||
                          S.d_live_scan.cap < live_scratch_words(nb) ||
                          S.d_work.cap < nwork || (geoms && S.d_guided.cap < nb) || S.d_segs.cap < b.seg_cap ||
                          S.d_seg_base.cap < nord || S.d_grp.cap < b.ngrp + 1 || S.d_grp2.cap < b.ngrp2 + 1 ||
                          S.d_grp_segs.cap < std::max(b.ngrp, b.ngrp2) || S.d_grp_item_base.cap < std::max(b.ngrp, b.ngrp2);
        if (grow && !sync_batch_streams("sync before growing device scratch")) return false;
        if (!hc(S.d_pairs.ensure(nb), "dev pairs") || !hc(S.d_order.ensure(nb), "dev order") ||
            !hc(S.d_order2.ensure(nb), "dev order2") ||
            !hc(S.d_rowbuf.ensure(b.top_rows), "row top2") || !hc(S.d_colbuf.ensure(b.top_cols), "col top2") ||
            !hc(S.d_accmask.ensure(b.top_rows / 32 + 8), "accept mask") ||
            !hc(S.d_pair_off.ensure(nb), "pair_off") || !hc(S.d_pair_cnt.ensure(nb), "pair_cnt") ||
            !hc(S.d_matches.ensure(2 * b.cap), "dev matches") ||
            !hc(S.d_cand_cnt.ensure(nb), "cand_cnt") || !hc(S.d_candbuf.ensure(b.top_cols), "candbuf") ||
            !hc(S.d_live.ensure(nb), "live flags") || !hc(S.d_live_fwd.ensure(nb), "live list (forward)") ||
            !hc(S.d_live_all.ensure(nb), "live list") || !hc(S.d_live_rev.ensure(nb), "live list (reverse)") ||
            !hc(S.d_live_scan.ensure(live_scratch_words(nb)), "live list scratch") ||
            (nwork && !hc(S.d_work.ensure(nwork), "dev work")) || (geoms && !hc(S.d_guided.ensure(nb), "dev guided")) ||
            !hc(S.d_segs.ensure(b.seg_cap), "segment descriptors") || !hc(S.d_seg_base.ensure(nord), "segment bases") ||
            !hc(S.d_grp.ensure(b.ngrp + 1), "group cuts") || !hc(S.d_grp2.ensure(b.ngrp2 + 1), "group cuts") ||
            !hc(S.d_grp_segs.ensure(std::max(b.ngrp, b.ngrp2)), "group segments") ||
            !hc(S.d_grp_item_base.ensure(std::max(b.ngrp, b.ngrp2)), "group items"))
            return false;
        bool okq = hc(hipMemcpyAsync(S.d_pairs.p, c->h_pairs[k].p, nb * sizeof(PairDev),
                                     hipMemcpyHostToDevice, st), "H2D pairs") &&
                   hc(memset_async(c->d_scalars, 0, 2 * sizeof(uint32_t), st), "memset cursor") &&
                   hc(memset_async(c->d_scalars + 3, 0, sizeof(uint32_t), st), "memset errcount");
        if (okq && nord)
            okq = hc(hipMemcpyAsync(S.d_order.p, c->h_order[k].p, nord * sizeof(uint32_t),
                                    hipMemcpyHostToDevice, st), "H2D order") &&
                  hc(hipMemcpyAsync(S.d_grp.p, c->h_grp[k].p, (b.ngrp + 1) * sizeof(uint32_t),
                                    hipMemcpyHostToDevice, st), "H2D group cuts") &&
                  hc(memset_async(S.d_accmask.p, 0, (b.row_off / 32 + 8) * sizeof(uint32_t), st), "memset accmask");
        if (okq && nwork)
            okq = hc(hipMemcpyAsync(S.d_work.p, c->h_work[k].p, nwork * sizeof(Dot4Work),
                                    hipMemcpyHostToDevice, st), "H2D work");
        if (okq && geoms)
            okq = hc(hipMemcpyAsync(S.d_guided.p, h_guided.data() + b.begin, nb * sizeof(GuidedDev),
                                    hipMemcpyHostToDevice, st), "H2D guided");
        if (!okq) return false;
        if (nord &&
            !hc(launch_build_segments(0, c->d_imgs.p, S.d_pairs.p, S.d_order.p, S.d_grp.p, (uint32_t)b.ngrp,
                                      S.d_cand_cnt.p, S.d_candbuf.p, S.d_rowbuf.p, S.d_seg_base.p, S.d_grp_segs.p,
                                      S.d_grp_item_base.p, S.d_segs.p, c->d_scalars + 5, st), "segment packing"))
            return false;
        if (!hc(hipEventRecord(c->bev[k][0], st), "event record")) return false;
        if (nord) {
            CopyJob job;
            const uintptr_t ps = reinterpret_cast<uintptr_t>(pending.src), pd = reinterpret_cast<uintptr_t>(pending.dst);
            const bool take = pending.set >= 0 && d2h_mode == 0 && b.seg_cap > 0 && pending.bytes >= fuse_min_bytes &&
                              (ps & 15) == (pd & 15);
            int done_set = -1;
            if (take) {
                const size_t head = (ps & 15) ? 16 - (ps & 15) : 0, n16 = (pending.bytes - head) / 16;
                const size_t tail = pending.bytes - head - n16 * 16;
                if (head && !hc(memcpy_async(pending.dst, pending.src, head, hipMemcpyDeviceToHost, st), "D2H matches (head)"))
                    return false;
                if (tail && !hc(memcpy_async(static_cast<char*>(pending.dst) + head + n16 * 16,
                                             static_cast<const char*>(pending.src) + head + n16 * 16, tail,
                                             hipMemcpyDeviceToHost, st), "D2H matches (tail)"))
                    return false;
                job.src = static_cast<const char*>(pending.src) + head;
                job.dst = static_cast<char*>(pending.dst) + head;
                job.n16 = n16;
                job.parts = kCopyParts;
                done_set = pending.set;
                pending.set = -1;
            }
            if (!hc(launch_match_mfma(0, S.d_segs.p, c->d_scalars + 5, (uint32_t)std::min<size_t>(b.seg_cap, 0xFFFFFFFFu),
                                      c->d_scalars + 1, S.d_accmask.p, c->d_accept, st, job, c->d_scalars + 7), "forward scan"))
                return false;
            if (done_set >= 0 && !hc(hipEventRecord(c->bev[done_set][4], st), "event record")) return false;
        }
        if (b.nwork_grid &&
            !hc(launch_match_guided_grid(c->d_imgs.p, c->d_grids.p, S.d_pairs.p, S.d_work.p, (uint32_t)b.nwork_grid,
                                         S.d_rowbuf.p, S.d_colbuf.p, S.d_guided.p, st), "guided scan"))
            return false;
        if (nwork > b.nwork_grid &&
            !hc(launch_match_dot4(c->d_imgs.p, S.d_pairs.p, S.d_work.p + b.nwork_grid, (uint32_t)(nwork - b.nwork_grid),
                                  S.d_rowbuf.p, S.d_colbuf.p, geoms ? S.d_guided.p : nullptr, st), "dot4 scan"))
            return false;
        kernel_launches += (nord ? 1 : 0) + (b.nwork_grid ? 1 : 0) + (nwork > b.nwork_grid ? 1 : 0);
        return hc(hipEventRecord(c->bev[k][1], st), "event record");
    };
    auto enqueue_chain = [&](Batch& b) {
        const int k = b.set;
        amc_ctx::MatchScratch& S = c->ms;
        const size_t nb = b.nb, nord = b.nord;
        uint32_t* const nlive = c->d_scalars + 8;
        if (!hc(launch_live_pairs(c->d_imgs.p, S.d_pairs.p, (uint32_t)nb, S.d_accmask.p, S.d_order.p, (uint32_t)nord,
                                  S.d_live.p, S.d_live_fwd.p, S.d_live_all.p, nlive, S.d_cand_cnt.p, S.d_pair_cnt.p,
                                  S.d_pair_off.p, S.d_live_scan.p, st), "live pairs"))
            return false;
        if (nord &&
            !hc(launch_resolve_index(0, c->d_imgs.p, S.d_pairs.p, S.d_rowbuf.p, S.d_accmask.p, c->d_lut,
                                     fp, S.d_cand_cnt.p, S.d_candbuf.p, c->d_scalars + 3, b.grouped_resolve,
                                     S.d_live_fwd.p, nlive, (uint32_t)nord, st), "resolve (rows)"))
            return false;
        if (nord && o.cross_check) {
            if (!hc(launch_select_candidates(c->d_imgs.p, S.d_pairs.p, (uint32_t)nb, b.max_cols, S.d_rowbuf.p,
                                             S.d_accmask.p, c->d_lut, fp, S.d_cand_cnt.p, S.d_candbuf.p,
                                             S.d_live_all.p, nlive + 1, st),
                    "candidate selection"))
                return false;
            if (!hc(hipMemcpyAsync(S.d_order2.p, c->h_order2[k].p, nord * sizeof(uint32_t),
                                   hipMemcpyHostToDevice, st), "H2D order2") ||
                !hc(hipMemcpyAsync(S.d_grp2.p, c->h_grp2[k].p, (b.ngrp2 + 1) * sizeof(uint32_t),
                                   hipMemcpyHostToDevice, st), "H2D group cuts"))
                return false;
            if (!hc(launch_compact_order(S.d_order2.p, (uint32_t)nord, (uint32_t)nb, S.d_cand_cnt.p, S.d_live_rev.p, nlive + 2,
                                         S.d_live_scan.p, st),
                    "live pairs (reverse)") ||
                !hc(launch_build_segments(1, c->d_imgs.p, S.d_pairs.p, S.d_order2.p, S.d_grp2.p, (uint32_t)b.ngrp2,
                                          S.d_cand_cnt.p, S.d_candbuf.p, S.d_colbuf.p, S.d_seg_base.p, S.d_grp_segs.p,
                                          S.d_grp_item_base.p, S.d_segs.p, c->d_scalars + 5, st), "segment packing (reverse)") ||
                !hc(launch_match_mfma(1, S.d_segs.p, c->d_scalars + 5, (uint32_t)std::min<size_t>(b.seg_cap, 0xFFFFFFFFu),
                                      c->d_scalars + 1, S.d_accmask.p, c->d_accept, st), "reverse scan") ||
                !hc(launch_resolve_index(1, c->d_imgs.p, S.d_pairs.p, S.d_colbuf.p, S.d_accmask.p, c->d_lut,
                                         fp, S.d_cand_cnt.p, S.d_candbuf.p, c->d_scalars + 3, b.grouped_resolve,
                                         S.d_live_rev.p, nlive + 2, (uint32_t)nord, st), "resolve (columns)"))
                return false;
        }
        if (!hc(hipEventRecord(c->bev[k][2], st), "event record") ||
            !hc(launch_finalize(c->d_imgs.p, S.d_pairs.p, (uint32_t)nb, S.d_live_all.p, nlive + 1, S.d_rowbuf.p, S.d_colbuf.p,
                                S.d_accmask.p, c->d_lut, fp, c->d_scalars, (uint32_t)std::min(b.cap, (size_t)0xFFFFFFFFu),
                                S.d_pair_off.p, S.d_pair_cnt.p, S.d_matches.p, st), "finalize"))
            return false;
        return hc(hipMemcpyAsync(c->h_bscalars[k].p, c->d_scalars, 4 * sizeof(uint32_t),
                                 hipMemcpyDeviceToHost, st), "D2H cursor") &&
               hc(hipMemcpyAsync(c->h_pair_off[k].p, S.d_pair_off.p, nb * sizeof(uint32_t),
                                 hipMemcpyDeviceToHost, st), "D2H pair_off") &&
               hc(hipMemcpyAsync(c->h_pair_cnt[k].p, S.d_pair_cnt.p, nb * sizeof(uint32_t),
                                 hipMemcpyDeviceToHost, st), "D2H pair_cnt") &&
               hc(hipEventRecord(c->bev[k][3], st), "event record");
    };
    auto collect = [&](Batch& b) {
        const int k = b.set;
        amc_ctx::MatchScratch& S = c->ms;
        if (!hc(hipEventSynchronize(c->bev[k][3]), "wait for the batch")) return false;
        b.total = c->h_bscalars[k].p[0];
        if (c->h_bscalars[k].p[3] != 0) {
            rc = api_fail(AMC_E_HIP, "amc_match_pairs: internal: %u accepted rows could not be resolved "
                          "to an index (scan/recompute mismatch)", c->h_bscalars[k].p[3]);
            return false;
        }
        if (b.total > b.cap) {
            rc = api_fail(AMC_E_HIP, "amc_match_pairs: internal: %u matches exceed capacity %zu", b.total, b.cap);
            return false;
        }
        if (!hc(c->h_csr[k].ensure(b.nb), "pinned csr")) return false;
        uint64_t run = keep_used;
        for (size_t i = 0; i < b.nb; ++i) {
            c->h_csr[k].p[i] = run;
            if (keep_off) (*keep_off)[b.begin + i] = run;
            run += c->h_pair_cnt[k].p[i];
            priv->offsets[b.begin + i + 1] = run;
        }
        if (run - keep_used != b.total) {
            rc = api_fail(AMC_E_HIP, "amc_match_pairs: internal: pair counts (%llu) disagree with the cursor (%u)",
                          (unsigned long long)(run - keep_used), b.total);
            return false;
        }
        rows_collected += b.top_rows;
        if (b.total) {
            const auto tgrow = std::chrono::steady_clock::now();
            const size_t need = 2 * (keep_used + (size_t)b.total);
            size_t want = need;
            if (rows_collected > 0 && rows_collected < rows_total) {
                const double est = std::min((double)need * ((double)rows_total / (double)rows_collected) * 1.1, 4.0 * (double)need);
                want = std::max(need, (size_t)est / 2 * 2);
            }
            if (need > c->d_keep.cap) {
                DevBuf<uint32_t> bigger;
                if (bigger.ensure(std::max(want, 2 * c->d_keep.cap)) != hipSuccess) {
                    (void)hipGetLastError();
                    if (!hc(bigger.ensure(need), "resident match table")) return false;
                }
                if (keep_used &&
                    !hc(hipMemcpyAsync(bigger.p, c->d_keep.p, 2 * keep_used * sizeof(uint32_t), hipMemcpyDeviceToDevice, st),
                        "move resident match table"))
                    return false;
                if (!sync_batch_streams("sync before freeing the old resident table") ||
                    !hc(hipStreamSynchronize(c->copy_stream), "sync before freeing the old resident table"))
                    return false;
                c->d_keep = std::move(bigger);
            }
            if (need > priv->matches.cap) {
                if (!sync_batch_streams("sync before growing the result buffer") ||
                    !hc(hipStreamSynchronize(c->copy_stream), "sync before growing the result buffer"))
                    return false;
                PinBuf<uint32_t> bigger;
                if (bigger.ensure(std::max(want, 2 * priv->matches.cap)) != hipSuccess) {
                    (void)hipGetLastError();
                    if (prof) std::fprintf(stderr, "[amc match profile] pinned result: %zu words refused, asking for %zu\n", want, need);
                    if (!hc(bigger.ensure(need), "pinned result")) return false;
                }
                if (keep_used) std::memcpy(bigger.p, priv->matches.p, 2 * keep_used * sizeof(uint32_t));
                priv->matches = std::move(bigger);
            }
            if (prof && since(tgrow) > 5.0)
                std::fprintf(stderr, "[amc match profile] batch of %zu pairs: %.1f ms growing the result tables to %zu words\n", b.nb,
                             since(tgrow), priv->matches.cap);
            if (!hc(c->d_csr.ensure(b.nb), "dev csr") ||
                !hc(hipMemcpyAsync(c->d_csr.p, c->h_csr[k].p, b.nb * sizeof(uint64_t), hipMemcpyHostToDevice, st), "H2D csr"))
                return false;
            if (!hc(launch_reorder_matches(S.d_pair_off.p, S.d_pair_cnt.p, c->d_csr.p, (uint32_t)b.nb, S.d_matches.p,
                                           c->d_keep.p, st), "reorder launch"))
                return false;
            pending.dst = priv->matches.p + 2 * keep_used;
            pending.src = c->d_keep.p + 2 * keep_used;
            pending.bytes = (size_t)b.total * 2 * sizeof(uint32_t);
            pending.set = k;
            keep_used += b.total;
            return true;
        }
        return hc(hipEventRecord(c->bev[k][4], st), "event record");
    };
    double t_hook = 0.0;
    auto run_hook = [&](const Batch& b) {
        if (!batch_hook) return true;
        const auto th = std::chrono::steady_clock::now();
        const int hrc = (*batch_hook)(b.begin, b.end, priv->offsets.data(), keep_off ? keep_off->data() : nullptr);
        t_hook += since(th);
        if (hrc != AMC_OK && rc == AMC_OK) rc = hrc;
        return hrc == AMC_OK;
    };
    auto flush_copy = [&]() {
        if (pending.set < 0) return true;
        const int k = pending.set;
        pending.set = -1;
        if (!hc(hipEventRecord(c->cev[k], st), "event record") || !hc(hipStreamWaitEvent(c->copy_stream, c->cev[k], 0), "stream wait"))
            return false;
        if (d2h_mode == 2) {
            if (!hc(hipMemcpyAsync(pending.dst, pending.src, pending.bytes, hipMemcpyDeviceToHost, c->copy_stream), "D2H matches"))
                return false;
        } else {
            if (!hc(launch_host_copy(pending.dst, pending.src, pending.bytes, c->copy_stream), "D2H matches")) return false;
        }
        return hc(hipEventRecord(c->bev[k][4], c->copy_stream), "event record");
    };
    auto scatter = [&](Batch& b) {
        const int k = b.set;
        if (!hc(hipEventSynchronize(c->bev[k][4]), "wait for the matches")) return false;
        float ms = 0.f;
        if (hipEventElapsedTime(&ms, c->bev[k][0], c->bev[k][1]) == hipSuccess) kernel_ms += ms;
        if (hipEventElapsedTime(&ms, c->bev[k][1], c->bev[k][2]) == hipSuccess) cross_ms += ms;
        return true;
    };

    if (npairs > 0) {
        Batch cur = carve(0, 0);
        auto tp = std::chrono::steady_clock::now();
        bool ok = prepare(cur, true);
        t_prepare += since(tp);
        tp = std::chrono::steady_clock::now();
        ok = ok && enqueue_scan(cur);
        if (ok) build_reverse_order(cur);
        ok = ok && enqueue_chain(cur);
        t_enqueue += since(tp);
        Batch prev;
        bool have_prev = false;
        while (ok) {
            Batch next;
            const bool have_next = cur.end < npairs;
            if (have_next) {
                tp = std::chrono::steady_clock::now();
                next = carve(cur.end, cur.set ^ 1);
                ok = prepare(next, false);
                t_prepare += since(tp);
            }
            tp = std::chrono::steady_clock::now();
            if (ok && have_prev) ok = scatter(prev);
            t_scatter += since(tp);
            tp = std::chrono::steady_clock::now();
            ok = ok && collect(cur);
            t_collect += since(tp);
            tp = std::chrono::steady_clock::now();
            if (ok && have_next) ok = enqueue_scan(next) && enqueue_chain(next);
            ok = ok && flush_copy();
            t_enqueue += since(tp);
            ok = ok && run_hook(cur);
            if (!have_next) {
                tp = std::chrono::steady_clock::now();
                ok = ok && scatter(cur);
                t_scatter += since(tp);
                break;
            }
            prev = cur;
            have_prev = true;
            cur = next;
        }
        if (!ok && rc == AMC_OK) rc = api_fail(AMC_E_HIP, "amc_match_pairs: batch failed");
        if (rc != AMC_OK) {
            (void)hipStreamSynchronize(st);
            (void)hipStreamSynchronize(c->copy_stream);
        }
    }
    if (rc == AMC_OK && npairs > 0 &&
        hc(hipEventRecord(c->cev[0], c->copy_stream), "event record"))
        hc(hipStreamWaitEvent(st, c->cev[0], 0), "stream wait");
    if (rc == AMC_OK && hc(hipEventRecord(c->ev[1], st), "event record")) hc(hipEventSynchronize(c->ev[1]), "wait for the call");
    if (rc != AMC_OK) {
        delete priv;
        return rc;
    }
    float total_ms = 0.f;
    (void)hipEventElapsedTime(&total_ms, c->ev[0], c->ev[1]);

    out->npairs = npairs;
    c->resident_matches = keep_used;
    out->offsets = priv->offsets.data();
    out->matches = priv->offsets[npairs] ? priv->matches.p : nullptr;
    out->num_distances = num_dist;
    out->pairs_mfma = n_mfma;
    out->pairs_dot4 = n_dot4;
    out->pairs_guided_grid = n_grid;
    out->device_ms = total_ms;
    out->match_kernel_ms = kernel_ms;
    out->match_kernel_launches = kernel_launches;
    out->cross_kernel_ms = cross_ms;
    out->_priv = priv;
    c->last_hook_ms = t_hook;
    if (prof)
        std::fprintf(stderr, "[amc match profile] pairs=%zu wall=%.1f ms: prepare %.1f, enqueue %.1f, collect(wait+reorder+D2H enqueue) %.1f, "
                     "scatter(wait) %.1f, batch hook %.1f; device events %.1f ms (scan %.1f, cross %.1f)\n", npairs, since(wall0), t_prepare,
                     t_enqueue, t_collect, t_scatter, t_hook, (double)total_ms, kernel_ms, cross_ms);
    return AMC_OK;
}

extern "C" {

int amc_match_pairs(amc_ctx* c, const uint32_t* slot1, const uint32_t* slot2, size_t npairs,
                    const amc_match_opts* opts_in, amc_match_result* out) {
    return match_impl(c, slot1, slot2, npairs, opts_in, nullptr, 0.0, out);
}

int amc_match_guided_pairs(amc_ctx* c, const uint32_t* slot1, const uint32_t* slot2, size_t npairs,
                           const amc_tvg* geoms, double max_error, const amc_match_opts* opts_in,
                           amc_match_result* out) {
    if (npairs > 0 && !geoms) {
        if (out) std::memset(out, 0, sizeof *out);
        return api_fail(AMC_E_INVALID, "amc_match_guided_pairs: NULL geometries");
    }
    if (!(max_error >= 0.0)) {
        if (out) std::memset(out, 0, sizeof *out);
        return api_fail(AMC_E_INVALID, "amc_match_guided_pairs: max_error must be >= 0");
    }
    static const amc_tvg kNone{};
    return match_impl(c, slot1, slot2, npairs, opts_in, npairs ? geoms : &kNone, max_error, out);
}

void amc_match_result_free(amc_match_result* r) {
    if (!r) return;
    delete static_cast<ResultPriv*>(r->_priv);
    std::memset(r, 0, sizeof *r);
}

}
```

### pycolmap_amd/csrc/match_common.hip

```cpp
#include <algorithm>
#include <atomic>
#include <climits>
#include <cstdlib>

#include "amc_internal.h"

namespace amc {

__global__ __launch_bounds__(256) void prep_kernel(const uint8_t* __restrict__ raw,
                                                   uint8_t* __restrict__ prep,
                                                   int32_t* __restrict__ rs128,
                                                   uint32_t rows_pad,
                                                   uint32_t* __restrict__ maxsq_out) {
    const uint32_t gid = blockIdx.x * 256u + threadIdx.x;
    const uint32_t r = gid >> 3, q = gid & 7;
    uint32_t sum = 0, sq = 0;
    if (r < rows_pad) {
        const uint4 v = *reinterpret_cast<const uint4*>(raw + (size_t)r * kDim + q * 16);
        const uint32_t w[4] = {v.x, v.y, v.z, v.w};
#pragma unroll
        for (int i = 0; i < 4; ++i) {
            sum = __builtin_amdgcn_udot4(w[i], 0x01010101u, sum, false);
            sq = __builtin_amdgcn_udot4(w[i], w[i], sq, false);
        }
// ... 716 lines not shown
    const uint32_t per = ((max_cols + 31) / 32 + 255) / 256;
    const size_t shmem = (size_t)std::max(per, 1u) * 256 * sizeof(uint32_t);
    if (shmem > 48 * 1024) {
        const hipError_t e = hipFuncSetAttribute(reinterpret_cast<const void*>(select_candidates_kernel),
                                                 hipFuncAttributeMaxDynamicSharedMemorySize, (int)(kSelectMaxCols / 8));
        if (e != hipSuccess) return e;
    }
    hipLaunchKernelGGL(select_candidates_kernel, dim3(npairs), dim3(256), shmem, s, imgs, pairs,
                       rowbuf, accmask, acos_lut, fp, cand_cnt, candbuf, list, nlist);
    return hipGetLastError();
}

static_assert(kRowPad % 128 == 0, "live_flag_kernel reads a pair's accept words 16 bytes (128 rows) at a time");
__global__ __launch_bounds__(256) void live_flag_kernel(const ImageDev* __restrict__ imgs, const PairDev* __restrict__ pairs,
                                                        uint32_t npairs, const uint32_t* __restrict__ accmask,
                                                        uint32_t* __restrict__ live, uint32_t* __restrict__ cand_cnt,
                                                        uint32_t* __restrict__ pair_cnt, uint32_t* __restrict__ pair_off) {
    const uint32_t pi = blockIdx.x * 4 + (threadIdx.x >> 6), lane = threadIdx.x & 63;
    if (pi >= npairs) return;
    const PairDev p = pairs[pi];
    uint32_t flag;
    if (p.mode) {
        const uint4* w = reinterpret_cast<const uint4*>(accmask + (p.row_off >> 5));
        const uint32_t n16 = imgs[p.slot1].rows_pad / 128;
        uint32_t any = 0;
        for (uint32_t k = lane; k < n16; k += 64) {
            const uint4 v = w[k];
            any |= v.x | v.y | v.z | v.w;
        }
        flag = __ballot(any != 0) ? 3u : 0u;
    } else {
        flag = (imgs[p.slot1].rows != 0 && imgs[p.slot2].rows != 0) ? 1u : 0u;
    }
    if (lane == 0) {
        live[pi] = flag;
        if (flag != 3u) cand_cnt[pi] = 0;
        if (flag == 0u) {
            pair_cnt[pi] = 0;
            pair_off[pi] = 0;
        }
    }
}

constexpr uint32_t kCompactPer = 8, kCompactThreads = 256, kCompactSeg = kCompactPer * kCompactThreads;
static_assert(kCompactPer == 8, "a thread's entries are read as two uint4");
struct CompactJob {
    const uint32_t* order;
    const uint32_t* key;
    uint32_t* list;
    uint32_t* nlist;
    uint32_t* keep;
    uint32_t* segcnt;
    uint32_t n, mask, nseg;
};
static uint32_t compact_segments(uint32_t n) { return std::max(1u, (n + kCompactSeg - 1) / kCompactSeg); }
size_t live_scratch_words(size_t npairs) { return 3 * (size_t)compact_segments((uint32_t)npairs) * (kCompactThreads + 1); }
static CompactJob compact_job(const uint32_t* order, uint32_t n, const uint32_t* key, uint32_t mask, uint32_t* list,
                              uint32_t* nlist, uint32_t* scratch) {
    const uint32_t nseg = compact_segments(n);
    return CompactJob{order, key, list, nlist, scratch, scratch + (size_t)nseg * kCompactThreads, n, mask, nseg};
}
__global__ __launch_bounds__(kCompactThreads) void compact_count_kernel(CompactJob j0, CompactJob j1) {
    __shared__ uint32_t wsum[4];
    const bool first = blockIdx.x < j0.nseg;
    const CompactJob j = first ? j0 : j1;
    const uint32_t seg = first ? blockIdx.x : blockIdx.x - j0.nseg;
    const uint32_t tid = threadIdx.x, lane = tid & 63, wid = tid >> 6;
    const uint32_t i0 = seg * kCompactSeg + tid * kCompactPer;
    uint32_t keep = 0;
    if (i0 < j.n) {
        uint32_t pi[kCompactPer], kv[kCompactPer];
        if (j.order && i0 + kCompactPer <= j.n) {
            const uint4 a = *reinterpret_cast<const uint4*>(j.order + i0), b = *reinterpret_cast<const uint4*>(j.order + i0 + 4);
            pi[0] = a.x; pi[1] = a.y; pi[2] = a.z; pi[3] = a.w; pi[4] = b.x; pi[5] = b.y; pi[6] = b.z; pi[7] = b.w;
        } else {
#pragma unroll
            for (uint32_t u = 0; u < kCompactPer; ++u) {
                const uint32_t i = min(i0 + u, j.n - 1);
                pi[u] = j.order ? j.order[i] : i;
            }
        }
#pragma unroll
        for (uint32_t u = 0; u < kCompactPer; ++u) kv[u] = j.key[pi[u]];
#pragma unroll
        for (uint32_t u = 0; u < kCompactPer; ++u)
            if (i0 + u < j.n && (kv[u] & j.mask) != 0) keep |= 1u << u;
    }
    j.keep[seg * kCompactThreads + tid] = keep;
    uint32_t c = __popc(keep);
#pragma unroll
    for (int m = 1; m < 64; m <<= 1) c += __shfl_xor(c, m);
    if (lane == 0) wsum[wid] = c;
    __syncthreads();
    if (tid == 0) j.segcnt[seg] = wsum[0] + wsum[1] + wsum[2] + wsum[3];
}
__global__ __launch_bounds__(kCompactThreads) void compact_scatter_kernel(CompactJob j0, CompactJob j1) {
    __shared__ uint32_t wsum[4], psum[4];
    const bool first = blockIdx.x < j0.nseg;
    const CompactJob j = first ? j0 : j1;
    const uint32_t seg = first ? blockIdx.x : blockIdx.x - j0.nseg;
    const uint32_t tid = threadIdx.x, lane = tid & 63, wid = tid >> 6;
    const uint32_t i0 = seg * kCompactSeg + tid * kCompactPer;
    uint32_t part = 0;
    for (uint32_t k = tid; k < seg; k += kCompactThreads) part += j.segcnt[k];
    uint32_t keep = j.keep[seg * kCompactThreads + tid];
    const uint32_t c = __popc(keep);
    uint32_t inc = c;
#pragma unroll
    for (int m = 1; m < 64; m <<= 1) {
        const uint32_t o = __shfl_up(inc, m);
        if (lane >= (uint32_t)m) inc += o;
        part += __shfl_xor(part, m);
    }
    if (lane == 63) wsum[wid] = inc;
    if (lane == 0) psum[wid] = part;
    __syncthreads();
    const uint32_t base = psum[0] + psum[1] + psum[2] + psum[3];
    uint32_t wbase = 0;
    for (uint32_t k = 0; k < wid; ++k) wbase += wsum[k];
    uint32_t dst = base + wbase + inc - c;
    while (keep) {
        const uint32_t i = i0 + (uint32_t)(__ffs(keep) - 1);
        keep &= keep - 1;
        j.list[dst++] = j.order ? j.order[i] : i;
    }
    if (seg == j.nseg - 1 && tid == 0) *j.nlist = base + wsum[0] + wsum[1] + wsum[2] + wsum[3];
}
static hipError_t launch_compact(const CompactJob& a, const CompactJob* b, hipStream_t s) {
    const CompactJob second = b ? *b : a;
    const uint32_t grid = a.nseg + (b ? b->nseg : 0u);
    hipLaunchKernelGGL(compact_count_kernel, dim3(grid), dim3(kCompactThreads), 0, s, a, second);
    hipLaunchKernelGGL(compact_scatter_kernel, dim3(grid), dim3(kCompactThreads), 0, s, a, second);
    return hipGetLastError();
}

hipError_t launch_live_pairs(const ImageDev* imgs, const PairDev* pairs, uint32_t npairs, const uint32_t* accmask,
                             const uint32_t* order, uint32_t norder, uint32_t* live, uint32_t* live_fwd,
                             uint32_t* live_all, uint32_t* nlive, uint32_t* cand_cnt, uint32_t* pair_cnt,
                             uint32_t* pair_off, uint32_t* scratch, hipStream_t s) {
    if (npairs == 0) return memset_async(nlive, 0, 2 * sizeof(uint32_t), s);
    hipLaunchKernelGGL(live_flag_kernel, dim3((npairs + 3) / 4), dim3(256), 0, s, imgs, pairs, npairs, accmask, live,
                       cand_cnt, pair_cnt, pair_off);
    const size_t third = live_scratch_words(npairs) / 3;
    const CompactJob fwd = compact_job(order, norder, live, 2u, live_fwd, nlive, scratch);
    const CompactJob all = compact_job(nullptr, npairs, live, 1u, live_all, nlive + 1, scratch + third);
    return launch_compact(fwd, &all, s);
}
hipError_t launch_compact_order(const uint32_t* order, uint32_t norder, uint32_t npairs, const uint32_t* key, uint32_t* list,
                                uint32_t* nlist, uint32_t* scratch, hipStream_t s) {
    const CompactJob job = compact_job(order, norder, key, 0xFFFFFFFFu, list, nlist, scratch + 2 * (live_scratch_words(npairs) / 3));
    return launch_compact(job, nullptr, s);
}

__global__ __launch_bounds__(256) void reorder_matches_kernel(const uint32_t* __restrict__ src_off,
                                                              const uint32_t* __restrict__ cnt,
                                                              const uint64_t* __restrict__ dst_off, uint32_t npairs,
                                                              const uint2* __restrict__ src, uint2* __restrict__ dst) {
    const uint32_t p = blockIdx.x * 4 + (threadIdx.x >> 6);
    if (p >= npairs) return;
    const uint32_t n = cnt[p];
    const uint2* s = src + src_off[p];
    uint2* d = dst + dst_off[p];
    for (uint32_t i = threadIdx.x & 63; i < n; i += 64) d[i] = s[i];
}
hipError_t launch_reorder_matches(const uint32_t* src_off, const uint32_t* cnt, const uint64_t* dst_off, uint32_t npairs,
                                  const uint32_t* src, uint32_t* dst, hipStream_t s) {
    if (npairs == 0) return hipSuccess;
    hipLaunchKernelGGL(reorder_matches_kernel, dim3((npairs + 3) / 4), dim3(256), 0, s, src_off, cnt, dst_off, npairs,
                       reinterpret_cast<const uint2*>(src), reinterpret_cast<uint2*>(dst));
    return hipGetLastError();
}

constexpr int kHostCopyBlocks = 64;
__global__ __launch_bounds__(256) void host_copy_kernel(uint4* __restrict__ dst, const uint4* __restrict__ src, size_t n16,
                                                        uint2* __restrict__ dst_tail, const uint2* __restrict__ src_tail,
                                                        uint32_t tail8) {
    const size_t stride = (size_t)gridDim.x * blockDim.x;
    size_t i = (size_t)blockIdx.x * blockDim.x + threadIdx.x;
    for (; i + 3 * stride < n16; i += 4 * stride) {
        const uint4 a = src[i], b = src[i + stride], c = src[i + 2 * stride], d = src[i + 3 * stride];
        dst[i] = a; dst[i + stride] = b; dst[i + 2 * stride] = c; dst[i + 3 * stride] = d;
    }
    for (; i < n16; i += stride) dst[i] = src[i];
    if (blockIdx.x == 0 && threadIdx.x < tail8) dst_tail[threadIdx.x] = src_tail[threadIdx.x];
}
hipError_t launch_host_copy(void* dst_pinned, const void* src_dev, size_t bytes, hipStream_t s) {
    if (bytes == 0) return hipSuccess;
    const uintptr_t a = reinterpret_cast<uintptr_t>(src_dev);
    const size_t head = (a & 15) && ((reinterpret_cast<uintptr_t>(dst_pinned) & 15) == (a & 15)) ? 16 - (a & 15) : 0;
    const bool same_phase = (reinterpret_cast<uintptr_t>(dst_pinned) & 15) == (a & 15);
    if (!same_phase || bytes < ((size_t)1 << 20)) {
        return memcpy_async(dst_pinned, src_dev, bytes, hipMemcpyDeviceToHost, s);
    }
    const char* sp = static_cast<const char*>(src_dev);
    char* dp = static_cast<char*>(dst_pinned);
    if (head) {
        const hipError_t e = memcpy_async(dp, sp, head, hipMemcpyDeviceToHost, s);
        if (e != hipSuccess) return e;
    }
    const size_t body = bytes - head, n16 = body / 16, tail = body - n16 * 16;
    hipLaunchKernelGGL(host_copy_kernel, dim3(kHostCopyBlocks), dim3(256), 0, s, reinterpret_cast<uint4*>(dp + head),
                       reinterpret_cast<const uint4*>(sp + head), n16, reinterpret_cast<uint2*>(dp + head + n16 * 16),
                       reinterpret_cast<const uint2*>(sp + head + n16 * 16), (uint32_t)(tail / 8));
    return hipGetLastError();
}

hipError_t launch_finalize(const ImageDev* imgs, const PairDev* pairs, uint32_t npairs, const uint32_t* list,
                           const uint32_t* nlist, const Top2* rowbuf, const Top2* colbuf, uint32_t* accmask,
                           const float* acos_lut, FinalizeParams fp, uint32_t* cursor, uint32_t capacity,
                           uint32_t* pair_off, uint32_t* pair_cnt, uint32_t* matches, hipStream_t s) {
    if (npairs == 0) return hipSuccess;
    hipLaunchKernelGGL(finalize_kernel, dim3(npairs), dim3(kFinalizeThreads), 0, s, imgs, pairs, list, nlist,
                       rowbuf, colbuf, accmask, acos_lut, fp, cursor, capacity, pair_off, pair_cnt, matches);
    return hipGetLastError();
}

}
```

Before: 14480 billion distances/s.

## Move batch queue building to GPU and adapt batch carving to predicted match volume

```diff
diff --git a/include/amc.h b/include/amc.h
--- a/include/amc.h
+++ b/include/amc.h
@@ -219,6 +219,9 @@
 
 int amc_ctx_last_timeline(amc_ctx* ctx, double out_ms[8]);
 
+int amc_ctx_debug_match_queues(amc_ctx* ctx, uint64_t sizes[5], uint32_t* order, uint32_t* grp, uint32_t* order2,
+                               uint32_t* grp2);
+
 int amc_pose_pairs(amc_ctx* ctx, const uint32_t* slot1, const uint32_t* slot2, size_t npairs,
                    const uint64_t* match_offsets, const uint32_t* inlier_matches, const amc_tvg* geoms,
                    amc_pose* out);
diff --git a/profiles/carve/recipes/parts_summary.py b/profiles/carve/recipes/parts_summary.py
--- /dev/null
+++ b/profiles/carve/recipes/parts_summary.py
@@ -0,0 +1,23 @@
+import json, sys, os, statistics
+d, names = sys.argv[1], sys.argv[2:]
+def last_json(p):
+    for line in reversed(open(p).read().strip().split("\n")):
+        if line.strip().startswith("{"):
+            try: return json.loads(line)
+            except Exception: pass
+res = {}
+for v in names:
+    ms, scan, launches = [], [], []
+    i = 1
+    while os.path.exists(f"{d}/head_{v}{i}.json"):
+        j = last_json(f"{d}/head_{v}{i}.json"); i += 1
+        ms.append(round(j["ms_per_step"], 3)); r = j.get("roofline") or {}
+        scan.append(round(r.get("avg_kernel_ms", 0), 3)); launches.append(r.get("kernel_launches", r.get("launches")))
+    res[v] = {"ms_per_step": ms, "median": statistics.median(ms), "spread": round(max(ms) - min(ms), 3), "scan_ms_per_launch": scan,
+              "scan_median": statistics.median(scan), "launches": launches}
+base = res[names[0]]
+for v in names[1:]:
+    res[v]["gain_vs_" + names[0]] = round(base["median"] - res[v]["median"], 3)
+    res[v]["three_spreads_of_" + names[0]] = round(3 * base["spread"], 3)
+json.dump(res, open(f"{d}/summary_multi.json", "w"), indent=1)
+print(json.dumps(res, indent=1))
diff --git a/profiles/carve/recipes/threshold_inputs.py b/profiles/carve/recipes/threshold_inputs.py
--- /dev/null
+++ b/profiles/carve/recipes/threshold_inputs.py
@@ -0,0 +1,49 @@
+import json, os, sys, time
+sys.path.insert(0, os.getcwd())
+import numpy as np
+import torch
+import bench
+from pycolmap_amd import _capi, synth
+
+which = sys.argv[1]
+out = {}
+dev = torch.device("cuda:0")
+arena = bench.make_arena_torch(500, 4096, seed=0 if which == "batches" else 1, device=dev, **({} if which == "batches" else {"overlap": "all"}))
+ctx = _capi.Context(0)
+ctx.set_stream(torch.cuda.current_stream().cuda_stream)
+ctx.reserve_slots(500)
+for i in range(500):
+    ctx.upload_descriptors_device(i, arena[i].data_ptr(), 4096)
+torch.cuda.synchronize()
+s1, s2 = synth.exhaustive_pairs(500)
+if which == "batches":
+    res = {}
+    for rnd in range(2):
+        for ent in (0, 192 << 20, 128 << 20, 96 << 20, 64 << 20):
+            if ent:
+                os.environ["AMC_MATCH_BATCH_ENTRIES"] = str(ent)
+            else:
+                os.environ.pop("AMC_MATCH_BATCH_ENTRIES", None)
+            for _ in range(3):
+                w = ctx.match_pairs(s1, s2, copy=False); w = None
+            d, wall = [], []
+            for _ in range(10):
+                t0 = time.perf_counter()
+                off, m, st = ctx.match_pairs(s1, s2, copy=False)
+                wall.append(1e3 * (time.perf_counter() - t0))
+                d.append(st["device_ms"])
+                off = m = None
+            res.setdefault(str(ent), []).append({"batches": st["match_kernel_launches"], "device_ms_median": float(np.median(d)),
+                                                 "wall_ms_median": float(np.median(wall)), "scan_ms_last": st["match_kernel_ms"]})
+            print(ent, res[str(ent)][-1], flush=True)
+    out["headline"] = res
+else:
+    for _ in range(3):
+        off = m = None
+        off, m, st = ctx.match_pairs(s1, s2, copy=False)
+    off = np.asarray(off)
+    out["dense"] = {"batches": st["match_kernel_launches"], "device_ms": st["device_ms"], "matches": int(off[-1]),
+                    "bytes_after_pair": {str(p): int((off[-1] - off[p]) * 8) for p in (65536, 108366)}}
+    print(out["dense"], flush=True)
+ctx.close()
+json.dump(out, open(f"profiles/carve/threshold_{which}.json", "w"), indent=1)
diff --git a/pycolmap_amd/_capi.py b/pycolmap_amd/_capi.py
--- a/pycolmap_amd/_capi.py
+++ b/pycolmap_amd/_capi.py
@@ -1167,6 +1167,8 @@
     lib.amc_ctx_resident_matches.restype = C.c_int
     lib.amc_upload_matches.argtypes = [C.c_void_p, C.c_void_p, C.c_uint64]
     lib.amc_upload_matches.restype = C.c_int
+    if hasattr(lib, "amc_ctx_debug_match_queues"):
+        lib.amc_ctx_debug_match_queues.argtypes = [C.c_void_p] * 6
     if hasattr(lib, "amc_ctx_last_timeline"):
         lib.amc_ctx_last_timeline.argtypes = [C.c_void_p, C.c_void_p]
     lib.amc_ctx_reserve_slots.argtypes = [C.c_void_p, C.c_uint32]
@@ -1524,6 +1526,16 @@
     def set_stream(self, hip_stream: int | None) -> None:
         _check(self._lib.amc_ctx_set_stream(self._h, C.c_void_p(hip_stream or 0)))
 
+    def debug_match_queues(self) -> dict:
+        sizes = np.zeros(5, dtype=np.uint64)
+        _check(self._lib.amc_ctx_debug_match_queues(self._h, sizes.ctypes.data, None, None, None, None))
+        begin, npairs, norder, ngrp, ngrp2 = (int(v) for v in sizes)
+        order, order2 = np.zeros(norder, dtype=np.uint32), np.zeros(norder, dtype=np.uint32)
+        grp, grp2 = np.zeros(ngrp + 1, dtype=np.uint32), np.zeros(ngrp2 + 1, dtype=np.uint32)
+        _check(self._lib.amc_ctx_debug_match_queues(self._h, sizes.ctypes.data, order.ctypes.data, grp.ctypes.data,
+                                                    order2.ctypes.data, grp2.ctypes.data))
+        return dict(begin=begin, npairs=npairs, order=order, grp=grp, order2=order2, grp2=grp2)
+
     def last_timeline(self) -> dict:
         buf = (C.c_double * 8)()
         _check(self._lib.amc_ctx_last_timeline(self._h, buf))
diff --git a/pycolmap_amd/csrc/amc_api.hip b/pycolmap_amd/csrc/amc_api.hip
--- a/pycolmap_amd/csrc/amc_api.hip
+++ b/pycolmap_amd/csrc/amc_api.hip
@@ -147,12 +147,12 @@
     c->ms.release_all();
     c->d_keep.release(); c->d_csr.release();
     dlap("match device buffers");
-    c->h_csr[0].release(); c->h_csr[1].release();
     c->h_tout.release(); c->h_tmask.release();
+    for (int k = 0; k < amc_ctx::kMatchStages; ++k) {
+        c->h_pairs[k].release(); c->h_work[k].release();
+    }
     for (int k = 0; k < 2; ++k) {
-        c->h_pairs[k].release(); c->h_work[k].release(); c->h_order[k].release(); c->h_order2[k].release();
-        c->h_grp[k].release(); c->h_grp2[k].release();
-        c->h_pair_off[k].release(); c->h_pair_cnt[k].release(); c->h_matches[k].release();
+        c->h_pair_cnt[k].release(); c->h_matches[k].release();
         c->h_bscalars[k].release();
     }
     c->h_scalars.release();
@@ -218,10 +218,27 @@
     c->verify_pool->trim();
     c->arena.release_idle_slabs();
     c->h_tout.release(); c->h_tmask.release();
-    for (int k = 0; k < 2; ++k) {
-        c->h_matches[k].release();
-        c->h_csr[k].release();
-    }
+    for (int k = 0; k < 2; ++k) c->h_matches[k].release();
+    return AMC_OK;
+}
+
+int amc_ctx_debug_match_queues(amc_ctx* c, uint64_t sizes[5], uint32_t* order, uint32_t* grp, uint32_t* order2,
+                               uint32_t* grp2) {
+    if (!c || !sizes) return api_fail(AMC_E_INVALID, "amc_ctx_debug_match_queues: NULL argument");
+    const amc_ctx::LastQueues& q = c->last_queues;
+    sizes[0] = q.begin; sizes[1] = q.npairs; sizes[2] = q.norder; sizes[3] = q.ngrp; sizes[4] = q.ngrp2;
+    if (!order && !grp && !order2 && !grp2) return AMC_OK;
+    HIPCHK(hipSetDevice(c->device));
+    HIPCHK(hipStreamSynchronize(c->stream));
+    const amc_ctx::MatchScratch& S = c->ms;
+    if (q.norder > S.d_order.cap || q.ngrp + 1 > S.d_grp.cap || (order2 && q.norder > S.d_order2.cap) ||
+        (grp2 && q.ngrp2 + 1 > S.d_grp2.cap))
+        return api_fail(AMC_E_STATE, "amc_ctx_debug_match_queues: the scratch of the last match call is gone");
+    if (q.norder == 0) return AMC_OK;
+    if (order) HIPCHK(hipMemcpy(order, S.d_order.p, q.norder * sizeof(uint32_t), hipMemcpyDeviceToHost));
+    if (grp) HIPCHK(hipMemcpy(grp, S.d_grp.p, (q.ngrp + 1) * sizeof(uint32_t), hipMemcpyDeviceToHost));
+    if (order2) HIPCHK(hipMemcpy(order2, S.d_order2.p, q.norder * sizeof(uint32_t), hipMemcpyDeviceToHost));
+    if (grp2) HIPCHK(hipMemcpy(grp2, S.d_grp2.p, (q.ngrp2 + 1) * sizeof(uint32_t), hipMemcpyDeviceToHost));
     return AMC_OK;
 }
 
diff --git a/pycolmap_amd/csrc/amc_ctx.h b/pycolmap_amd/csrc/amc_ctx.h
--- a/pycolmap_amd/csrc/amc_ctx.h
+++ b/pycolmap_amd/csrc/amc_ctx.h
@@ -151,6 +151,7 @@
         DevBuf<PairDev> d_pairs;
         DevBuf<Dot4Work> d_work;
         DevBuf<uint32_t> d_order, d_order2;
+        DevBuf<uint32_t> d_queue_tmp, d_queue_tab;
         DevBuf<uint32_t> d_grp, d_grp2, d_seg_base, d_grp_segs, d_grp_item_base;
         DevBuf<SegDesc> d_segs;
         DevBuf<Top2> d_rowbuf, d_colbuf;
@@ -160,6 +161,7 @@
         DevBuf<uint32_t> d_live, d_live_fwd, d_live_all, d_live_rev, d_live_scan;
         void release_all() {
             d_pairs.release(); d_work.release(); d_order.release(); d_order2.release();
+            d_queue_tmp.release(); d_queue_tab.release();
             d_grp.release(); d_grp2.release(); d_seg_base.release(); d_grp_segs.release();
             d_grp_item_base.release(); d_segs.release();
             d_rowbuf.release(); d_colbuf.release(); d_accmask.release(); d_guided.release();
@@ -175,15 +177,18 @@
     };
     MatchScratch ms;
     DevBuf<uint32_t> d_keep;
-    DevBuf<uint64_t> d_csr;
+    DevBuf<uint32_t> d_csr;
     uint64_t resident_matches = 0;
-    PinBuf<uint64_t> h_csr[2];
     std::shared_ptr<PinnedPool> result_pool = std::make_shared<PinnedPool>();
     SlotArena arena;
-    PinBuf<PairDev> h_pairs[2];
-    PinBuf<Dot4Work> h_work[2];
-    PinBuf<uint32_t> h_order[2], h_order2[2], h_pair_off[2], h_pair_cnt[2], h_matches[2], h_bscalars[2];
-    PinBuf<uint32_t> h_grp[2], h_grp2[2];
+    static constexpr int kMatchStages = 3;
+    PinBuf<PairDev> h_pairs[kMatchStages];
+    PinBuf<Dot4Work> h_work[kMatchStages];
+    struct LastQueues {
+        size_t begin = 0, npairs = 0, norder = 0, ngrp = 0, ngrp2 = 0;
+    };
+    LastQueues last_queues;
+    PinBuf<uint32_t> h_pair_cnt[2], h_matches[2], h_bscalars[2];
     PinBuf<uint32_t> h_scalars;
     hipEvent_t ev[6] = {nullptr, nullptr, nullptr, nullptr, nullptr, nullptr};
     hipEvent_t bev[2][5] = {{nullptr, nullptr, nullptr, nullptr, nullptr},
diff --git a/pycolmap_amd/csrc/amc_internal.h b/pycolmap_amd/csrc/amc_internal.h
--- a/pycolmap_amd/csrc/amc_internal.h
+++ b/pycolmap_amd/csrc/amc_internal.h
@@ -348,6 +348,10 @@
 hipError_t launch_compact_order(const uint32_t* order, uint32_t norder, uint32_t npairs, const uint32_t* key, uint32_t* list,
                                 uint32_t* nlist, uint32_t* scratch, hipStream_t s);
 
+size_t queue_scratch_words(size_t npairs, size_t nslots);
+hipError_t launch_build_queues(const PairDev* pairs, uint32_t npairs, uint32_t norder, uint32_t nslots, uint32_t* order,
+                               uint32_t* grp, uint32_t* order2, uint32_t* grp2, uint32_t* tmp, uint32_t* tab, hipStream_t s);
+
 hipError_t launch_resolve_index(int side, const ImageDev* imgs, const PairDev* pairs,
                           Top2* table, uint32_t* accmask, const float* acos_lut, FinalizeParams fp,
                           const uint32_t* cand_cnt, const uint32_t* candbuf, uint32_t* err_count,
@@ -366,7 +370,8 @@
                      uint32_t* pair_off, uint32_t* pair_cnt, uint32_t* matches, hipStream_t s);
 
 hipError_t launch_host_copy(void* dst_pinned, const void* src_dev, size_t bytes, hipStream_t s);
-hipError_t launch_reorder_matches(const uint32_t* src_off, const uint32_t* cnt, const uint64_t* dst_off, uint32_t npairs,
+hipError_t launch_pair_csr(const uint32_t* cnt, uint32_t npairs, uint32_t* off, uint32_t* segsum, hipStream_t s);
+hipError_t launch_reorder_matches(const uint32_t* src_off, const uint32_t* cnt, const uint32_t* dst_off, uint32_t npairs,
                             const uint32_t* src, uint32_t* dst, hipStream_t s);
 
 struct CameraDev {
diff --git a/pycolmap_amd/csrc/amc_match.hip b/pycolmap_amd/csrc/amc_match.hip
--- a/pycolmap_amd/csrc/amc_match.hip
+++ b/pycolmap_amd/csrc/amc_match.hip
@@ -9,6 +9,7 @@
 #include <vector>
 
 #include "amc_ctx.h"
+#include "match_plan.h"
 
 using namespace amc;
 
@@ -61,14 +62,30 @@
     if (opts_in) o = *opts_in; else amc_match_opts_default(&o);
     if (o.kernel != AMC_KERNEL_AUTO && o.kernel != AMC_KERNEL_MFMA && o.kernel != AMC_KERNEL_DOT4)
         return api_fail(AMC_E_INVALID, "amc_match_pairs: unknown kernel %d", o.kernel);
+    struct SlotSize {
+        uint32_t rows, rows_pad, valid;
+    };
+    std::vector<SlotSize> packed_sizes;
+    if (npairs >= c->slots.size()) {
+        packed_sizes.resize(c->slots.size());
+        for (size_t k = 0; k < packed_sizes.size(); ++k)
+            packed_sizes[k] = SlotSize{c->slots[k].dev.rows, c->slots[k].dev.rows_pad, c->slots[k].valid ? 1u : 0u};
+    }
+    const SlotSize* const packed = packed_sizes.empty() ? nullptr : packed_sizes.data();
+    auto size_of = [&](uint32_t slot) {
+        if (packed) return packed[slot];
+        const Slot& t = c->slots[slot];
+        return SlotSize{t.dev.rows, t.dev.rows_pad, t.valid ? 1u : 0u};
+    };
     uint64_t rows_total = 0;
     for (size_t i = 0; i < npairs; ++i) {
         if (slot1[i] >= c->slots.size() || slot2[i] >= c->slots.size())
             return api_fail(AMC_E_INVALID, "amc_match_pairs: pair %zu references slot out of range", i);
-        if (!c->slots[slot1[i]].valid || !c->slots[slot2[i]].valid)
+        const SlotSize x = size_of(slot1[i]);
+        if (!x.valid || !size_of(slot2[i]).valid)
             return api_fail(AMC_E_STATE, "amc_match_pairs: pair %zu references a slot with no "
                             "descriptors uploaded", i);
-        rows_total += c->slots[slot1[i]].dev.rows_pad;
+        rows_total += x.rows_pad;
     }
     std::vector<GuidedDev> h_guided;
     if (geoms) {
@@ -160,10 +177,16 @@
         uint32_t max_cols = 0;
         size_t ngrp = 0, ngrp2 = 0, seg_cap = 0;
         int set = 0;
+        int stage = 0;
         uint32_t total = 0;
         bool grouped_resolve = true;
-    };
-    uint64_t rows_carved = 0, rows_collected = 0;
+        bool quarter_short = false;
+        uint64_t rows_before = 0;
+        uint64_t keep_base = 0;
+        uint64_t num_dist = 0, n_mfma = 0, n_dot4 = 0, n_grid = 0;
+    };
+    uint64_t rows_collected = 0;
+    match_plan::History collected;
     const int d2h_mode = !d2h_env ? 0 : (std::strcmp(d2h_env, "memcpy") == 0 ? 2 : (std::strcmp(d2h_env, "stream") == 0 ? 1 : 0));
     struct PendingCopy {
         void* dst = nullptr;
@@ -175,134 +198,86 @@
     auto sync_batch_streams = [&](const char* what) { return hc(hipStreamSynchronize(st), what); };
     const bool hook_split = batch_hook && hook_split_mode != 0;
     const size_t hook_split_min_pairs = hook_split_mode == 2 ? 2 : 4096;
-    auto carve = [&](size_t begin, int set) {
+    match_plan::Limits plan_limits;
+    plan_limits.max_entries = max_entries;
+    plan_limits.max_match_cap = kMaxMatchCap;
+    const uint64_t few_bytes = (uint64_t)env_int("AMC_MATCH_FEW_BYTES", batch_entries ? 0 : (long long)match_plan::kExposedCopyBytes,
+                                                 0, std::numeric_limits<long long>::max());
+    auto carve = [&](const Batch* before, int set, int stage, bool at_limits) {
         Batch b;
-        b.begin = b.end = begin;
+        b.begin = b.end = before ? before->end : 0;
         b.set = set;
-        size_t limit = max_entries;
-        const uint64_t rows_left = rows_total - rows_carved;
-        if (begin > 0 && rows_left <= max_entries && rows_left > max_entries / 4)
-            limit = (size_t)(rows_left - max_entries / 4);
-        if (begin == 0 && hook_split && rows_total <= max_entries && npairs >= hook_split_min_pairs)
-            limit = (size_t)(rows_total * 6 / 10);
-        while (b.end < npairs) {
-            const Slot& x = c->slots[slot1[b.end]];
-            const Slot& y = c->slots[slot2[b.end]];
-            const size_t nr = x.dev.rows_pad, nc = y.dev.rows_pad;
-            const size_t mc = o.cross_check ? std::min(x.dev.rows, y.dev.rows) : x.dev.rows;
-            if (b.end > b.begin && (b.top_rows + nr > limit || b.top_cols + nc > max_entries ||
-                                    b.cap + mc > kMaxMatchCap || b.end - b.begin >= (1u << 24)))
-                break;
-            b.top_rows += nr; b.top_cols += nc; b.cap += mc; ++b.end;
-        }
+        b.stage = stage;
+        b.rows_before = before ? before->rows_before + before->top_rows : 0;
+        const uint64_t first_row_limit =
+            hook_split && rows_total <= max_entries && npairs >= hook_split_min_pairs ? rows_total * 6 / 10 : 0;
+        const match_plan::Cut cut = match_plan::carve(
+            b.begin, npairs, rows_total - b.rows_before, plan_limits, collected,
+            [&](size_t i) {
+                const SlotSize x = size_of(slot1[i]), y = size_of(slot2[i]);
+                return match_plan::PairSize{x.rows_pad, y.rows_pad, o.cross_check ? std::min(x.rows, y.rows) : x.rows};
+            },
+            first_row_limit, at_limits, few_bytes);
+        b.end = cut.end;
+        b.top_rows = (size_t)cut.top_rows; b.top_cols = (size_t)cut.top_cols; b.cap = (size_t)cut.cap;
+        b.quarter_short = cut.quarter_short;
         b.nb = b.end - b.begin;
-        rows_carved += b.top_rows;
         return b;
     };
-    auto build_reverse_order = [&](Batch& b) {
-        const int k = b.set;
-        const size_t nord = b.nord;
-        if (!nord || !o.cross_check) return;
-        const PairDev* hp = c->h_pairs[k].p;
-        const size_t nslots = c->slots.size();
-        std::vector<uint32_t> cnt(nslots + 1), tmp(nord);
-        auto by_slot = [&](const uint32_t* src, uint32_t* dst, bool key_is_slot2) {
-            std::fill(cnt.begin(), cnt.end(), 0u);
-            for (size_t q = 0; q < nord; ++q) ++cnt[(key_is_slot2 ? hp[src[q]].slot2 : hp[src[q]].slot1) + 1];
-            for (size_t v = 0; v < nslots; ++v) cnt[v + 1] += cnt[v];
-            for (size_t q = 0; q < nord; ++q) dst[cnt[key_is_slot2 ? hp[src[q]].slot2 : hp[src[q]].slot1]++] = src[q];
+    auto prepare = [&](Batch& b) {
+        const int k = b.stage;
+        const size_t nb = b.nb, begin = b.begin;
+        if (!hc(c->h_pairs[k].ensure(nb), "pinned pairs") ||
+            !hc(c->h_pair_cnt[b.set].ensure(nb), "pinned pair_cnt") || !hc(c->h_bscalars[b.set].ensure(16), "pinned scalars"))
+            return false;
+        auto want_mfma = [&](const SlotSize& x, const SlotSize& y) {
+            return x.rows > 0 && y.rows > 0 && o.kernel != AMC_KERNEL_DOT4 && !geoms &&
+                   (!o.cross_check || y.rows_pad <= mfma_max_cols);
         };
-        uint32_t* ord2 = c->h_order2[k].p;
-        by_slot(c->h_order[k].p, tmp.data(), true);
-        by_slot(tmp.data(), ord2, false);
-        size_t ngrp2 = 0;
-        for (size_t q = 0; q < nord; ++q)
-            if (q == 0 || hp[ord2[q]].slot1 != hp[ord2[q - 1]].slot1) c->h_grp2[k].p[ngrp2++] = (uint32_t)q;
-        c->h_grp2[k].p[ngrp2] = (uint32_t)nord;
-    };
-    auto prepare = [&](Batch& b, bool defer_reverse) {
-        const int k = b.set;
-        const size_t nb = b.nb, begin = b.begin;
-        if (!hc(c->h_pairs[k].ensure(nb), "pinned pairs") || !hc(c->h_order[k].ensure(nb), "pinned order") ||
-            !hc(c->h_order2[k].ensure(nb), "pinned order2") || !hc(c->h_pair_off[k].ensure(nb), "pinned pair_off") ||
-            !hc(c->h_pair_cnt[k].ensure(nb), "pinned pair_cnt") || !hc(c->h_bscalars[k].ensure(16), "pinned scalars"))
-            return false;
-        std::vector<uint8_t> want_mfma(nb, 0);
-        for (size_t i = 0; i < nb; ++i) {
-            const Slot& x = c->slots[slot1[begin + i]];
-            const Slot& y = c->slots[slot2[begin + i]];
-            const bool nonempty = x.dev.rows > 0 && y.dev.rows > 0;
-            want_mfma[i] = nonempty && o.kernel != AMC_KERNEL_DOT4 && !geoms &&
-                           (!o.cross_check || y.dev.rows_pad <= mfma_max_cols);
-        }
+        const uint32_t grouped_max_rows = resolve_grouped_max_rows();
         PairDev* hp = c->h_pairs[k].p;
-        size_t row_off = 0, col_off = 0, nwork = 0, nord = 0, nimg1 = 0;
-        std::vector<uint8_t> seen1(c->slots.size(), 0);
+        size_t row_off = 0, col_off = 0, nwork = 0, nord = 0, nimg1 = 0, nimg2 = 0, seg1 = 0, seg2 = 0;
+        std::vector<uint8_t> seen1(c->slots.size(), 0), seen2(c->slots.size(), 0);
         b.grouped_resolve = !resolve_ungrouped;
         for (size_t i = 0; i < nb; ++i) {
-            const Slot& x = c->slots[slot1[begin + i]];
-            const Slot& y = c->slots[slot2[begin + i]];
-            const bool nonempty = x.dev.rows > 0 && y.dev.rows > 0;
-            if (o.kernel == AMC_KERNEL_MFMA && nonempty && !want_mfma[i]) {
+            const SlotSize x = size_of(slot1[begin + i]), y = size_of(slot2[begin + i]);
+            const bool nonempty = x.rows > 0 && y.rows > 0, mfma = want_mfma(x, y);
+            if (o.kernel == AMC_KERNEL_MFMA && nonempty && !mfma) {
                 rc = api_fail(AMC_E_INVALID,
                               "amc_match_pairs: kernel=MFMA forced but pair %zu is not eligible "
-                              "(rows_pad=%u, cols_pad=%u > %zu)", begin + i, x.dev.rows_pad,
-                              y.dev.rows_pad, mfma_max_cols);
+                              "(rows_pad=%u, cols_pad=%u > %zu)", begin + i, x.rows_pad,
+                              y.rows_pad, mfma_max_cols);
                 return false;
             }
             PairDev& pd = hp[i];
             pd.slot1 = slot1[begin + i];
             pd.slot2 = slot2[begin + i];
-            pd.mode = want_mfma[i] ? 1u : 0u;
+            pd.mode = mfma ? 1u : 0u;
             pd.pad = 0;
             pd.row_off = row_off;
             pd.col_off = col_off;
-            row_off += x.dev.rows_pad;
-            col_off += y.dev.rows_pad;
-            num_dist += (uint64_t)x.dev.rows * y.dev.rows;
+            row_off += x.rows_pad;
+            col_off += y.rows_pad;
+            b.num_dist += (uint64_t)x.rows * y.rows;
             if (!nonempty) continue;
-            if (want_mfma[i]) {
-                c->h_order[k].p[nord++] = (uint32_t)i;
+            if (mfma) {
+                ++nord;
                 if (!seen1[pd.slot1]) { seen1[pd.slot1] = 1; ++nimg1; }
-                ++n_mfma;
-                b.max_cols = std::max(b.max_cols, y.dev.rows);
-                if (std::max(x.dev.rows_pad, y.dev.rows_pad) > resolve_grouped_max_rows()) b.grouped_resolve = false;
+                if (!seen2[pd.slot2]) { seen2[pd.slot2] = 1; ++nimg2; }
+                seg1 += (x.rows + kSegRows - 1) / kSegRows;
+                seg2 += (y.rows + kSegRows - 1) / kSegRows;
+                ++b.n_mfma;
+                b.max_cols = std::max(b.max_cols, y.rows);
+                if (std::max(x.rows_pad, y.rows_pad) > grouped_max_rows) b.grouped_resolve = false;
             } else {
-                nwork += (x.dev.rows + 63) / 64;
-                if (o.cross_check) nwork += (y.dev.rows + 63) / 64;
-                if (geoms && h_guided[begin + i].grid_ok) ++n_grid; else ++n_dot4;
-            }
-        }
-        if (nord) {
-            const size_t nslots = c->slots.size();
-            std::vector<uint32_t> cnt(nslots + 1), tmp(nord);
-            auto by_slot = [&](const uint32_t* src, uint32_t* dst, bool key_is_slot2) {
-                std::fill(cnt.begin(), cnt.end(), 0u);
-                for (size_t q = 0; q < nord; ++q) ++cnt[(key_is_slot2 ? hp[src[q]].slot2 : hp[src[q]].slot1) + 1];
-                for (size_t v = 0; v < nslots; ++v) cnt[v + 1] += cnt[v];
-                for (size_t q = 0; q < nord; ++q) dst[cnt[key_is_slot2 ? hp[src[q]].slot2 : hp[src[q]].slot1]++] = src[q];
-            };
-            uint32_t* ord = c->h_order[k].p;
-            by_slot(ord, tmp.data(), false);
-            by_slot(tmp.data(), ord, true);
-        }
-        b.ngrp = b.ngrp2 = 0;
-        b.seg_cap = 0;
-        if (nord) {
-            if (!hc(c->h_grp[k].ensure(nord + 1), "pinned group cuts") ||
-                (o.cross_check && !hc(c->h_grp2[k].ensure(nord + 1), "pinned group cuts")))
-                return false;
-            size_t seg1 = 0, seg2 = 0;
-            for (size_t q = 0; q < nord; ++q) {
-                const PairDev& pq = hp[c->h_order[k].p[q]];
-                if (q == 0 || pq.slot2 != hp[c->h_order[k].p[q - 1]].slot2) c->h_grp[k].p[b.ngrp++] = (uint32_t)q;
-                seg1 += (c->slots[pq.slot1].dev.rows + kSegRows - 1) / kSegRows;
-                seg2 += (c->slots[pq.slot2].dev.rows + kSegRows - 1) / kSegRows;
-            }
-            c->h_grp[k].p[b.ngrp] = (uint32_t)nord;
-            if (o.cross_check) b.ngrp2 = nimg1;
-            b.seg_cap = std::max(seg1 + kSegsPerItem * b.ngrp, o.cross_check ? seg2 + kSegsPerItem * b.ngrp2 : 0);
-        }
+                nwork += (x.rows + 63) / 64;
+                if (o.cross_check) nwork += (y.rows + 63) / 64;
+                if (geoms && h_guided[begin + i].grid_ok) ++b.n_grid; else ++b.n_dot4;
+            }
+        }
+        b.ngrp = nimg2;
+        b.ngrp2 = o.cross_check ? nimg1 : 0;
+        b.seg_cap = nord ? std::max(seg1 + kSegsPerItem * b.ngrp, o.cross_check ? seg2 + kSegsPerItem * b.ngrp2 : 0) : 0;
         b.nwork_grid = 0;
         if (nwork) {
             if (!hc(c->h_work[k].ensure(nwork), "pinned work")) return false;
@@ -326,19 +301,21 @@
         b.row_off = row_off;
         b.nwork = nwork;
         b.nord = nord;
-        if (!defer_reverse) build_reverse_order(b);
         return true;
     };
     auto enqueue_scan = [&](Batch& b) {
-        const int k = b.set;
+        const int k = b.set, g = b.stage;
         amc_ctx::MatchScratch& S = c->ms;
         const size_t nb = b.nb, nord = b.nord, nwork = b.nwork;
+        num_dist += b.num_dist; n_mfma += b.n_mfma; n_dot4 += b.n_dot4; n_grid += b.n_grid;
+        c->last_queues = amc_ctx::LastQueues{b.begin, nb, nord, b.ngrp, b.ngrp2};
         const bool grow = S.d_pairs.cap < nb || S.d_order.cap < nb || S.d_order2.cap < nb ||
                           S.d_rowbuf.cap < b.top_rows || S.d_colbuf.cap < b.top_cols ||
                           S.d_accmask.cap < b.top_rows / 32 + 8 || S.d_pair_off.cap < nb || S.d_pair_cnt.cap < nb ||
                           S.d_matches.cap < 2 * b.cap || S.d_cand_cnt.cap < nb || S.d_candbuf.cap < b.top_cols ||
                           S.d_live.cap < nb || S.d_live_fwd.cap < nb || S.d_live_all.cap < nb || S.d_live_rev.cap < nb ||
-                          S.d_live_scan.cap < live_scratch_words(nb) ||
+                          S.d_live_scan.cap < live_scratch_words(nb) || c->d_csr.cap < nb ||
+                          S.d_queue_tmp.cap < 2 * nb || S.d_queue_tab.cap < queue_scratch_words(nb, c->slots.size()) ||
                           S.d_work.cap < nwork || (geoms && S.d_guided.cap < nb) || S.d_segs.cap < b.seg_cap ||
                           S.d_seg_base.cap < nord || S.d_grp.cap < b.ngrp + 1 || S.d_grp2.cap < b.ngrp2 + 1 ||
                           S.d_grp_segs.cap < std::max(b.ngrp, b.ngrp2) || S.d_grp_item_base.cap < std::max(b.ngrp, b.ngrp2);
@@ -352,25 +329,26 @@
             !hc(S.d_cand_cnt.ensure(nb), "cand_cnt") || !hc(S.d_candbuf.ensure(b.top_cols), "candbuf") ||
             !hc(S.d_live.ensure(nb), "live flags") || !hc(S.d_live_fwd.ensure(nb), "live list (forward)") ||
             !hc(S.d_live_all.ensure(nb), "live list") || !hc(S.d_live_rev.ensure(nb), "live list (reverse)") ||
-            !hc(S.d_live_scan.ensure(live_scratch_words(nb)), "live list scratch") ||
+            !hc(S.d_live_scan.ensure(live_scratch_words(nb)), "live list scratch") || !hc(c->d_csr.ensure(nb), "dev csr") ||
+            !hc(S.d_queue_tmp.ensure(2 * nb), "queue order scratch") ||
+            !hc(S.d_queue_tab.ensure(queue_scratch_words(nb, c->slots.size())), "queue order tables") ||
             (nwork && !hc(S.d_work.ensure(nwork), "dev work")) || (geoms && !hc(S.d_guided.ensure(nb), "dev guided")) ||
             !hc(S.d_segs.ensure(b.seg_cap), "segment descriptors") || !hc(S.d_seg_base.ensure(nord), "segment bases") ||
             !hc(S.d_grp.ensure(b.ngrp + 1), "group cuts") || !hc(S.d_grp2.ensure(b.ngrp2 + 1), "group cuts") ||
             !hc(S.d_grp_segs.ensure(std::max(b.ngrp, b.ngrp2)), "group segments") ||
             !hc(S.d_grp_item_base.ensure(std::max(b.ngrp, b.ngrp2)), "group items"))
             return false;
-        bool okq = hc(hipMemcpyAsync(S.d_pairs.p, c->h_pairs[k].p, nb * sizeof(PairDev),
+        bool okq = hc(hipMemcpyAsync(S.d_pairs.p, c->h_pairs[g].p, nb * sizeof(PairDev),
                                      hipMemcpyHostToDevice, st), "H2D pairs") &&
                    hc(memset_async(c->d_scalars, 0, 2 * sizeof(uint32_t), st), "memset cursor") &&
                    hc(memset_async(c->d_scalars + 3, 0, sizeof(uint32_t), st), "memset errcount");
         if (okq && nord)
-            okq = hc(hipMemcpyAsync(S.d_order.p, c->h_order[k].p, nord * sizeof(uint32_t),
-                                    hipMemcpyHostToDevice, st), "H2D order") &&
-                  hc(hipMemcpyAsync(S.d_grp.p, c->h_grp[k].p, (b.ngrp + 1) * sizeof(uint32_t),
-                                    hipMemcpyHostToDevice, st), "H2D group cuts") &&
+            okq = hc(launch_build_queues(S.d_pairs.p, (uint32_t)nb, (uint32_t)nord, (uint32_t)c->slots.size(), S.d_order.p,
+                                         S.d_grp.p, o.cross_check ? S.d_order2.p : nullptr, o.cross_check ? S.d_grp2.p : nullptr,
+                                         S.d_queue_tmp.p, S.d_queue_tab.p, st), "queue orders") &&
                   hc(memset_async(S.d_accmask.p, 0, (b.row_off / 32 + 8) * sizeof(uint32_t), st), "memset accmask");
         if (okq && nwork)
-            okq = hc(hipMemcpyAsync(S.d_work.p, c->h_work[k].p, nwork * sizeof(Dot4Work),
+            okq = hc(hipMemcpyAsync(S.d_work.p, c->h_work[g].p, nwork * sizeof(Dot4Work),
                                     hipMemcpyHostToDevice, st), "H2D work");
         if (okq && geoms)
             okq = hc(hipMemcpyAsync(S.d_guided.p, h_guided.data() + b.begin, nb * sizeof(GuidedDev),
@@ -440,11 +418,6 @@
                                              S.d_live_all.p, nlive + 1, st),
                     "candidate selection"))
                 return false;
-            if (!hc(hipMemcpyAsync(S.d_order2.p, c->h_order2[k].p, nord * sizeof(uint32_t),
-                                   hipMemcpyHostToDevice, st), "H2D order2") ||
-                !hc(hipMemcpyAsync(S.d_grp2.p, c->h_grp2[k].p, (b.ngrp2 + 1) * sizeof(uint32_t),
-                                   hipMemcpyHostToDevice, st), "H2D group cuts"))
-                return false;
             if (!hc(launch_compact_order(S.d_order2.p, (uint32_t)nord, (uint32_t)nb, S.d_cand_cnt.p, S.d_live_rev.p, nlive + 2,
                                          S.d_live_scan.p, st),
                     "live pairs (reverse)") ||
@@ -465,11 +438,10 @@
             return false;
         return hc(hipMemcpyAsync(c->h_bscalars[k].p, c->d_scalars, 4 * sizeof(uint32_t),
                                  hipMemcpyDeviceToHost, st), "D2H cursor") &&
-               hc(hipMemcpyAsync(c->h_pair_off[k].p, S.d_pair_off.p, nb * sizeof(uint32_t),
-                                 hipMemcpyDeviceToHost, st), "D2H pair_off") &&
                hc(hipMemcpyAsync(c->h_pair_cnt[k].p, S.d_pair_cnt.p, nb * sizeof(uint32_t),
                                  hipMemcpyDeviceToHost, st), "D2H pair_cnt") &&
-               hc(hipEventRecord(c->bev[k][3], st), "event record");
+               hc(hipEventRecord(c->bev[k][3], st), "event record") &&
+               hc(launch_pair_csr(S.d_pair_cnt.p, (uint32_t)nb, c->d_csr.p, S.d_live_scan.p, st), "pair csr");
     };
     auto collect = [&](Batch& b) {
         const int k = b.set;
@@ -485,20 +457,10 @@
             rc = api_fail(AMC_E_HIP, "amc_match_pairs: internal: %u matches exceed capacity %zu", b.total, b.cap);
             return false;
         }
-        if (!hc(c->h_csr[k].ensure(b.nb), "pinned csr")) return false;
-        uint64_t run = keep_used;
-        for (size_t i = 0; i < b.nb; ++i) {
-            c->h_csr[k].p[i] = run;
-            if (keep_off) (*keep_off)[b.begin + i] = run;
-            run += c->h_pair_cnt[k].p[i];
-            priv->offsets[b.begin + i + 1] = run;
-        }
-        if (run - keep_used != b.total) {
-            rc = api_fail(AMC_E_HIP, "amc_match_pairs: internal: pair counts (%llu) disagree with the cursor (%u)",
-                          (unsigned long long)(run - keep_used), b.total);
-            return false;
-        }
+        b.keep_base = keep_used;
         rows_collected += b.top_rows;
+        collected.rows_scanned = rows_collected;
+        collected.matches = keep_used + b.total;
         if (b.total) {
             const auto tgrow = std::chrono::steady_clock::now();
             const size_t need = 2 * (keep_used + (size_t)b.total);
@@ -538,11 +500,8 @@
             if (prof && since(tgrow) > 5.0)
                 std::fprintf(stderr, "[amc match profile] batch of %zu pairs: %.1f ms growing the result tables to %zu words\n", b.nb,
                              since(tgrow), priv->matches.cap);
-            if (!hc(c->d_csr.ensure(b.nb), "dev csr") ||
-                !hc(hipMemcpyAsync(c->d_csr.p, c->h_csr[k].p, b.nb * sizeof(uint64_t), hipMemcpyHostToDevice, st), "H2D csr"))
-                return false;
             if (!hc(launch_reorder_matches(S.d_pair_off.p, S.d_pair_cnt.p, c->d_csr.p, (uint32_t)b.nb, S.d_matches.p,
-                                           c->d_keep.p, st), "reorder launch"))
+                                           c->d_keep.p + 2 * keep_used, st), "reorder launch"))
                 return false;
             pending.dst = priv->matches.p + 2 * keep_used;
             pending.src = c->d_keep.p + 2 * keep_used;
@@ -552,6 +511,21 @@
             return true;
         }
         return hc(hipEventRecord(c->bev[k][4], st), "event record");
+    };
+    auto fill_offsets = [&](const Batch& b) {
+        const uint32_t* cnt = c->h_pair_cnt[b.set].p;
+        uint64_t run = b.keep_base;
+        for (size_t i = 0; i < b.nb; ++i) {
+            if (keep_off) (*keep_off)[b.begin + i] = run;
+            run += cnt[i];
+            priv->offsets[b.begin + i + 1] = run;
+        }
+        if (run - b.keep_base != b.total) {
+            rc = api_fail(AMC_E_HIP, "amc_match_pairs: internal: pair counts (%llu) disagree with the cursor (%u)",
+                          (unsigned long long)(run - b.keep_base), b.total);
+            return false;
+        }
+        return true;
     };
     double t_hook = 0.0;
     auto run_hook = [&](const Batch& b) {
@@ -586,24 +560,28 @@
     };
 
     if (npairs > 0) {
-        Batch cur = carve(0, 0);
+        Batch cur = carve(nullptr, 0, 0, false);
         auto tp = std::chrono::steady_clock::now();
-        bool ok = prepare(cur, true);
+        bool ok = prepare(cur);
         t_prepare += since(tp);
         tp = std::chrono::steady_clock::now();
-        ok = ok && enqueue_scan(cur);
-        if (ok) build_reverse_order(cur);
-        ok = ok && enqueue_chain(cur);
+        ok = ok && enqueue_scan(cur) && enqueue_chain(cur);
         t_enqueue += since(tp);
         Batch prev;
         bool have_prev = false;
         while (ok) {
-            Batch next;
+            Batch next, wide;
             const bool have_next = cur.end < npairs;
+            bool have_wide = false;
             if (have_next) {
                 tp = std::chrono::steady_clock::now();
-                next = carve(cur.end, cur.set ^ 1);
-                ok = prepare(next, false);
+                next = carve(&cur, cur.set ^ 1, (cur.stage + 1) % amc_ctx::kMatchStages, false);
+                ok = prepare(next);
+                if (ok && next.quarter_short && few_bytes) {
+                    wide = carve(&cur, next.set, (cur.stage + 2) % amc_ctx::kMatchStages, true);
+                    have_wide = wide.end != next.end;
+                    ok = !have_wide || prepare(wide);
+                }
                 t_prepare += since(tp);
             }
             tp = std::chrono::steady_clock::now();
@@ -611,11 +589,14 @@
             t_scatter += since(tp);
             tp = std::chrono::steady_clock::now();
             ok = ok && collect(cur);
+            if (ok && have_wide && match_plan::few_matches_left(collected, rows_total - next.rows_before, few_bytes))
+                next = wide;
             t_collect += since(tp);
             tp = std::chrono::steady_clock::now();
             if (ok && have_next) ok = enqueue_scan(next) && enqueue_chain(next);
             ok = ok && flush_copy();
             t_enqueue += since(tp);
+            ok = ok && fill_offsets(cur);
             ok = ok && run_hook(cur);
             if (!have_next) {
                 tp = std::chrono::steady_clock::now();
diff --git a/pycolmap_amd/csrc/match_common.hip b/pycolmap_amd/csrc/match_common.hip
--- a/pycolmap_amd/csrc/match_common.hip
+++ b/pycolmap_amd/csrc/match_common.hip
@@ -892,9 +892,166 @@
     return launch_compact(job, nullptr, s);
 }
 
+constexpr uint32_t kQueueSeg = 1024;
+constexpr size_t kQueueTabWords = (size_t)1 << 22;
+struct QueueJob {
+    const uint32_t* src;
+    uint32_t* dst;
+    uint32_t* tab;
+    uint32_t* grp;
+    uint32_t n, nseg, seglen, by_image2;
+};
+struct QueueShape {
+    uint32_t nseg, seglen;
+};
+static QueueShape queue_shape(size_t n, size_t nslots) {
+    const size_t fit = std::max<size_t>(1, kQueueTabWords / (nslots + 1));
+    const size_t nseg = std::max<size_t>(1, std::min(fit, (n + kQueueSeg - 1) / kQueueSeg));
+    const size_t seglen = ((n + nseg - 1) / nseg + 63) / 64 * 64;
+    return QueueShape{(uint32_t)nseg, (uint32_t)std::max<size_t>(seglen, 64)};
+}
+size_t queue_scratch_words(size_t npairs, size_t nslots) {
+    return 4 * (size_t)queue_shape(npairs, nslots).nseg * (nslots + 1);
+}
+__device__ __forceinline__ uint32_t queue_key(const PairDev* __restrict__ pairs, uint32_t pi, uint32_t by_image2, uint32_t nslots) {
+    const uint4 p = *reinterpret_cast<const uint4*>(pairs + pi);
+    return p.z ? (by_image2 ? p.y : p.x) : nslots;
+}
+__global__ __launch_bounds__(256) void queue_hist_kernel(const PairDev* __restrict__ pairs, uint32_t nslots, QueueJob j0, QueueJob j1) {
+    const bool first = blockIdx.x < j0.nseg;
+    const QueueJob j = first ? j0 : j1;
+    const uint32_t seg = first ? blockIdx.x : blockIdx.x - j0.nseg;
+    const uint32_t i0 = seg * j.seglen, i1 = min(j.n, i0 + j.seglen);
+    for (uint32_t i = i0 + threadIdx.x; i < i1; i += 256) {
+        const uint32_t key = queue_key(pairs, j.src ? j.src[i] : i, j.by_image2, nslots);
+        atomicAdd(j.tab + (size_t)key * j.nseg + seg, 1u);
+    }
+}
+__global__ __launch_bounds__(1024) void queue_scan_kernel(uint32_t nslots, QueueJob j0, QueueJob j1) {
+    __shared__ uint32_t wsum[16];
+    const QueueJob j = blockIdx.x == 0 ? j0 : j1;
+    const uint32_t tid = threadIdx.x, lane = tid & 63, wid = tid >> 6;
+    const size_t words = (size_t)(nslots + 1) * j.nseg;
+    uint32_t running = 0;
+    for (size_t base = 0; base < words; base += 4096) {
+        const size_t w = base + 4 * (size_t)tid;
+        uint32_t v[4], c = 0;
+#pragma unroll
+        for (uint32_t u = 0; u < 4; ++u) {
+            v[u] = w + u < words ? j.tab[w + u] : 0u;
+            c += v[u];
+        }
+        uint32_t inc = c;
+#pragma unroll
+        for (int m = 1; m < 64; m <<= 1) {
+            const uint32_t o = __shfl_up(inc, m);
+            if (lane >= (uint32_t)m) inc += o;
+        }
+        if (lane == 63) wsum[wid] = inc;
+        __syncthreads();
+        uint32_t wbase = 0, total = 0;
+        for (uint32_t k = 0; k < 16; ++k) {
+            if (k < wid) wbase += wsum[k];
+            total += wsum[k];
+        }
+        uint32_t run = running + wbase + inc - c;
+#pragma unroll
+        for (uint32_t u = 0; u < 4; ++u) {
+            if (w + u < words) j.tab[w + u] = run;
+            run += v[u];
+        }
+        running += total;
+        __syncthreads();
+    }
+    if (!j.grp) return;
+    running = 0;
+    for (uint32_t base = 0; base < nslots; base += 1024) {
+        const uint32_t b = base + tid;
+        uint32_t start = 0, has = 0;
+        if (b < nslots) {
+            start = j.tab[(size_t)b * j.nseg];
+            has = j.tab[(size_t)(b + 1) * j.nseg] != start ? 1u : 0u;
+        }
+        uint32_t inc = has;
+#pragma unroll
+        for (int m = 1; m < 64; m <<= 1) {
+            const uint32_t o = __shfl_up(inc, m);
+            if (lane >= (uint32_t)m) inc += o;
+        }
+        if (lane == 63) wsum[wid] = inc;
+        __syncthreads();
+        uint32_t wbase = 0, total = 0;
+        for (uint32_t k = 0; k < 16; ++k) {
+            if (k < wid) wbase += wsum[k];
+            total += wsum[k];
+        }
+        if (has) j.grp[running + wbase + inc - 1] = start;
+        running += total;
+        __syncthreads();
+    }
+    if (tid == 0) j.grp[running] = j.tab[(size_t)nslots * j.nseg];
+}
+__global__ __launch_bounds__(64) void queue_scatter_kernel(const PairDev* __restrict__ pairs, uint32_t nslots, uint32_t keybits,
+                                                           QueueJob j0, QueueJob j1) {
+    const bool first = blockIdx.x < j0.nseg;
+    const QueueJob j = first ? j0 : j1;
+    const uint32_t seg = first ? blockIdx.x : blockIdx.x - j0.nseg;
+    const uint32_t lane = threadIdx.x;
+    const uint32_t i0 = seg * j.seglen, i1 = min(j.n, i0 + j.seglen);
+    const unsigned long long below = (1ull << lane) - 1ull;
+    uint32_t pi_next = 0, key_next = 0;
+    if (i0 + lane < i1) {
+        pi_next = j.src ? j.src[i0 + lane] : i0 + lane;
+        key_next = queue_key(pairs, pi_next, j.by_image2, nslots);
+    }
+    for (uint32_t base = i0; base < i1; base += 64) {
+        const uint32_t i = base + lane;
+        const bool valid = i < i1;
+        const uint32_t pi = pi_next, key = key_next;
+        if (i + 64 < i1) {
+            pi_next = j.src ? j.src[i + 64] : i + 64;
+            key_next = queue_key(pairs, pi_next, j.by_image2, nslots);
+        }
+        unsigned long long same = __ballot(valid);
+        for (uint32_t b = 0; b < keybits; ++b) {
+            const unsigned long long one = __ballot(valid && ((key >> b) & 1u));
+            same &= ((key >> b) & 1u) ? one : ~one;
+        }
+        uint32_t old = 0;
+        const int leader = valid ? __ffsll(same) - 1 : (int)lane;
+        if (valid && (int)lane == leader) old = atomicAdd(j.tab + (size_t)key * j.nseg + seg, (uint32_t)__popcll(same));
+        old = __shfl(old, leader);
+        if (valid) j.dst[old + (uint32_t)__popcll(same & below)] = pi;
+    }
+}
+hipError_t launch_build_queues(const PairDev* pairs, uint32_t npairs, uint32_t norder, uint32_t nslots, uint32_t* order,
+                               uint32_t* grp, uint32_t* order2, uint32_t* grp2, uint32_t* tmp, uint32_t* tab, hipStream_t s) {
+    if (norder == 0) return hipSuccess;
+    const QueueShape s1 = queue_shape(npairs, nslots), s2 = queue_shape(norder, nslots);
+    const size_t t1 = (size_t)s1.nseg * (nslots + 1), t2 = (size_t)s2.nseg * (nslots + 1);
+    const bool rev = order2 != nullptr;
+    hipError_t e = memset_async(tab, 0, (2 * t1 + 2 * t2) * sizeof(uint32_t), s);
+    if (e != hipSuccess) return e;
+    uint32_t keybits = 1;
+    while ((nslots >> keybits) != 0) ++keybits;
+    const QueueJob a1{nullptr, tmp, tab, nullptr, npairs, s1.nseg, s1.seglen, 0u};
+    const QueueJob b1{nullptr, tmp + npairs, tab + t1, nullptr, npairs, s1.nseg, s1.seglen, 1u};
+    const QueueJob a2{tmp, order, tab + 2 * t1, grp, norder, s2.nseg, s2.seglen, 1u};
+    const QueueJob b2{tmp + npairs, order2, tab + 2 * t1 + t2, grp2, norder, s2.nseg, s2.seglen, 0u};
+    for (int round = 0; round < 2; ++round) {
+        const QueueJob& a = round == 0 ? a1 : a2;
+        const QueueJob& b = round == 0 ? b1 : b2;
+        const uint32_t grid = a.nseg + (rev ? b.nseg : 0u);
+        hipLaunchKernelGGL(queue_hist_kernel, dim3(grid), dim3(256), 0, s, pairs, nslots, a, rev ? b : a);
+        hipLaunchKernelGGL(queue_scan_kernel, dim3(rev ? 2 : 1), dim3(1024), 0, s, nslots, a, rev ? b : a);
+        hipLaunchKernelGGL(queue_scatter_kernel, dim3(grid), dim3(64), 0, s, pairs, nslots, keybits, a, rev ? b : a);
+    }
+    return hipGetLastError();
+}
+
 __global__ __launch_bounds__(256) void reorder_matches_kernel(const uint32_t* __restrict__ src_off,
                                                               const uint32_t* __restrict__ cnt,
-                                                              const uint64_t* __restrict__ dst_off, uint32_t npairs,
+                                                              const uint32_t* __restrict__ dst_off, uint32_t npairs,
                                                               const uint2* __restrict__ src, uint2* __restrict__ dst) {
     const uint32_t p = blockIdx.x * 4 + (threadIdx.x >> 6);
     if (p >= npairs) return;
@@ -903,11 +1060,66 @@
     uint2* d = dst + dst_off[p];
     for (uint32_t i = threadIdx.x & 63; i < n; i += 64) d[i] = s[i];
 }
-hipError_t launch_reorder_matches(const uint32_t* src_off, const uint32_t* cnt, const uint64_t* dst_off, uint32_t npairs,
+hipError_t launch_reorder_matches(const uint32_t* src_off, const uint32_t* cnt, const uint32_t* dst_off, uint32_t npairs,
                                   const uint32_t* src, uint32_t* dst, hipStream_t s) {
     if (npairs == 0) return hipSuccess;
     hipLaunchKernelGGL(reorder_matches_kernel, dim3((npairs + 3) / 4), dim3(256), 0, s, src_off, cnt, dst_off, npairs,
                        reinterpret_cast<const uint2*>(src), reinterpret_cast<uint2*>(dst));
+    return hipGetLastError();
+}
+
+__global__ __launch_bounds__(kCompactThreads) void csr_count_kernel(const uint32_t* __restrict__ cnt, uint32_t n,
+                                                                    uint32_t* __restrict__ segsum) {
+    __shared__ uint32_t wsum[4];
+    const uint32_t tid = threadIdx.x, lane = tid & 63, wid = tid >> 6;
+    const uint32_t i0 = blockIdx.x * kCompactSeg + tid * kCompactPer;
+    uint32_t c = 0;
+#pragma unroll
+    for (uint32_t u = 0; u < kCompactPer; ++u)
+        if (i0 + u < n) c += cnt[i0 + u];
+#pragma unroll
+    for (int m = 1; m < 64; m <<= 1) c += __shfl_xor(c, m);
+    if (lane == 0) wsum[wid] = c;
+    __syncthreads();
+    if (tid == 0) segsum[blockIdx.x] = wsum[0] + wsum[1] + wsum[2] + wsum[3];
+}
+__global__ __launch_bounds__(kCompactThreads) void csr_scan_kernel(const uint32_t* __restrict__ cnt, uint32_t n,
+                                                                   const uint32_t* __restrict__ segsum,
+                                                                   uint32_t* __restrict__ off) {
+    __shared__ uint32_t wsum[4], psum[4];
+    const uint32_t seg = blockIdx.x, tid = threadIdx.x, lane = tid & 63, wid = tid >> 6;
+    const uint32_t i0 = seg * kCompactSeg + tid * kCompactPer;
+    uint32_t part = 0;
+    for (uint32_t k = tid; k < seg; k += kCompactThreads) part += segsum[k];
+    uint32_t v[kCompactPer], c = 0;
+#pragma unroll
+    for (uint32_t u = 0; u < kCompactPer; ++u) {
+        v[u] = i0 + u < n ? cnt[i0 + u] : 0u;
+        c += v[u];
+    }
+    uint32_t inc = c;
+#pragma unroll
+    for (int m = 1; m < 64; m <<= 1) {
+        const uint32_t o = __shfl_up(inc, m);
+        if (lane >= (uint32_t)m) inc += o;
+        part += __shfl_xor(part, m);
+    }
+    if (lane == 63) wsum[wid] = inc;
+    if (lane == 0) psum[wid] = part;
+    __syncthreads();
+    uint32_t run = psum[0] + psum[1] + psum[2] + psum[3] + inc - c;
+    for (uint32_t k = 0; k < wid; ++k) run += wsum[k];
+#pragma unroll
+    for (uint32_t u = 0; u < kCompactPer; ++u) {
+        if (i0 + u < n) off[i0 + u] = run;
+        run += v[u];
+    }
+}
+hipError_t launch_pair_csr(const uint32_t* cnt, uint32_t npairs, uint32_t* off, uint32_t* segsum, hipStream_t s) {
+    if (npairs == 0) return hipSuccess;
+    const uint32_t nseg = compact_segments(npairs);
+    hipLaunchKernelGGL(csr_count_kernel, dim3(nseg), dim3(kCompactThreads), 0, s, cnt, npairs, segsum);
+    hipLaunchKernelGGL(csr_scan_kernel, dim3(nseg), dim3(kCompactThreads), 0, s, cnt, npairs, segsum, off);
     return hipGetLastError();
 }
 
diff --git a/pycolmap_amd/csrc/match_plan.h b/pycolmap_amd/csrc/match_plan.h
--- /dev/null
+++ b/pycolmap_amd/csrc/match_plan.h
@@ -0,0 +1,69 @@
+#pragma once
+
+#include <cstddef>
+#include <cstdint>
+
+namespace amc {
+namespace match_plan {
+
+constexpr uint64_t kExposedCopyBytes = 18800000;
+constexpr uint64_t kMatchBytes = 8;
+
+struct Limits {
+    uint64_t max_entries = 0;
+    uint64_t max_match_cap = 0;
+    uint64_t max_pairs = (uint64_t)1 << 24;
+};
+
+struct History {
+    uint64_t rows_scanned = 0;
+    uint64_t matches = 0;
+};
+
+struct PairSize {
+    uint64_t rows = 0, cols = 0;
+    uint64_t cap = 0;
+};
+
+struct Cut {
+    size_t end = 0;
+    uint64_t top_rows = 0, top_cols = 0, cap = 0;
+    bool quarter_short = false;
+};
+
+inline uint64_t predicted_match_bytes(const History& h, uint64_t rows_left) {
+    if (h.rows_scanned == 0) return UINT64_MAX;
+    const unsigned __int128 bytes = (unsigned __int128)h.matches * kMatchBytes;
+    if (bytes != 0 && rows_left > ~(unsigned __int128)0 / bytes) return UINT64_MAX;
+    const unsigned __int128 p = bytes * rows_left / h.rows_scanned;
+    return p > (unsigned __int128)UINT64_MAX ? UINT64_MAX : (uint64_t)p;
+}
+
+inline bool few_matches_left(const History& h, uint64_t rows_left, uint64_t threshold = kExposedCopyBytes) {
+    return predicted_match_bytes(h, rows_left) < threshold;
+}
+
+template <class SizeFn>
+inline Cut carve(size_t begin, size_t npairs, uint64_t rows_left, const Limits& lim, const History& hist, SizeFn size,
+                 uint64_t first_row_limit = 0, bool assume_few = false, uint64_t threshold = kExposedCopyBytes) {
+    Cut c;
+    c.end = begin;
+    uint64_t limit = lim.max_entries;
+    if (begin > 0 && rows_left <= lim.max_entries && rows_left > lim.max_entries / 4 &&
+        !assume_few && !few_matches_left(hist, rows_left, threshold)) {
+        limit = rows_left - lim.max_entries / 4;
+        c.quarter_short = true;
+    }
+    if (begin == 0 && first_row_limit) limit = first_row_limit;
+    while (c.end < npairs) {
+        const PairSize s = size(c.end);
+        if (c.end > begin && (c.top_rows + s.rows > limit || c.top_cols + s.cols > lim.max_entries ||
+                              c.cap + s.cap > lim.max_match_cap || c.end - begin >= lim.max_pairs))
+            break;
+        c.top_rows += s.rows; c.top_cols += s.cols; c.cap += s.cap; ++c.end;
+    }
+    return c;
+}
+
+}
+}
```

Measured after the change: 14620 billion distances/s, median of 4. 1.0% higher.
